# NVIDIA-Merlin/distributed-embeddings

Hardware: NVIDIA H100
Metric: DLRM global samples/sec (device-timed, max over ranks) (higher is better)
Workload: dtype bf16

## Files before the change

distributed_embeddings_b200/models/dlrm_fast.py:

```python
from __future__ import annotations

import os
from typing import Optional

import torch
from torch import nn

from ..ops import _native
from ..parallel.comm import CommContext
from ..parallel.fused import FusedEngine
from ..utils import nvtx
from ..utils.lr_schedule import LearningRateScheduler
from ..utils.metrics import BinnedAUC, auc_from_histogram
from .dense_optimizer import FlatDenseOptimizer, dense_optimizer_config
from .dlrm import DLRM

FUSED_UPDATE_MIN_ROWS = 20000


def _pad8(n: int) -> int:
  return (n + 7) // 8 * 8


def _fused_dgrad(L) -> bool:
  return L.in_f == L.in_pad and L.in_f <= 2048 and L.out_f % 8 == 0


def _dgrad_block_n(L) -> int:
  return 128 if L.out_f <= 256 else 0


class _Layer:

  def __init__(self, lin: nn.Linear, relu: bool):
    self.lin = lin
    self.relu = relu
    self.out_f, self.in_f = lin.weight.shape
    self.in_pad = _pad8(self.in_f)
    self.w_off = self.b_off = 0
    self.w_numel = self.out_f * self.in_pad
    self.b_numel = _pad8(self.out_f) if lin.bias is not None else 0


class DLRMTrainStep:

  def __init__(self, model: DLRM, lr: float = 24.0, embedding_optimizer: str = "sgd",
               scheduler: Optional[LearningRateScheduler] = None, use_cuda_graph: bool = True,
               embedding_optimizer_kwargs: Optional[dict] = None, overlap: bool = True,
               gemm: str = "cublas", eval_thresholds: int = 8000, dense_optimizer: str = "sgd",
               dense_optimizer_kwargs: Optional[dict] = None, fused_table_update: bool = True,
               fused_update_min_rows: int = FUSED_UPDATE_MIN_ROWS):
    if gemm not in ("cublas", "fused_dgrad", "tcgen05", "tcgen05_pair"):
      raise ValueError("gemm must be cublas | fused_dgrad | tcgen05 | tcgen05_pair")
    self.gemm = gemm
    self.dcn = getattr(model, "interaction", "dot") == "dcnv2"
    hots = getattr(model, "multi_hot_sizes", None)
    if self.dcn and gemm != "cublas":
      raise ValueError("the dcnv2 interaction runs its GEMMs on cuBLASLt: use gemm='cublas'")
    if not self.dcn and hots is not None and any(h != 1 for h in hots):
      raise ValueError("multi-hot features need the dcnv2 interaction in DLRMTrainStep")
    self.fused_table_update = bool(fused_table_update)
    self.fused_update_min_rows = int(fused_update_min_rows)
    self.dense_cfg = dense_optimizer_config(dense_optimizer, dense_optimizer_kwargs)
    self.model = model
    self.emb = model.embedding
    if self.emb.backend != "fused":
      raise ValueError("DLRMTrainStep needs the fused embedding back end")
    self.dev = self.emb.device
    self.ops = _native.require()
    self.world = self.emb.world_size
    self.ctx = CommContext.for_group(self.emb.group, self.dev)
    self.scheduler = scheduler
    self.use_cuda_graph = use_cuda_graph
    self.overlap = overlap
    self.emb.set_optimizer(embedding_optimizer, lr=lr, **(embedding_optimizer_kwargs or {}))
    if self.emb._engine is None:
      self.emb._engine = FusedEngine(self.emb)
    self.engine: FusedEngine = self.emb._engine
    self.n_emb = len(model.table_sizes)
    self.dim = model.embedding_dim
    self.hots = list(hots) if hots is not None else [1] * self.n_emb
    if self.dcn:
      st = self.emb.strategy
      if self.emb.dp_input and any(self.hots[i] != 1 for i in st.input_groups[2]):
        raise NotImplementedError("the dcnv2 step does not support multi-hot row-sliced inputs")
      if self.dim % 8 or any(l.V.out_features % 8 for l in model.cross_layers):
        raise ValueError("the dcnv2 step needs an embedding width and a cross rank that are "
                         "multiples of 8")
    sp_env = os.environ.get("DE_B200_STREAM_PUSH", "auto")
    self._stream_push = self.world > 1 and (sp_env == "1" or (sp_env == "auto" and self.world >= 4))
    self._push_stream = torch.cuda.Stream(device=self.dev) if self._stream_push else None
    self._push_ready = torch.cuda.Event() if self._stream_push else None

    lins_b = [m for m in model.bottom_mlp.net if isinstance(m, nn.Linear)]
    lins_t = [m for m in model.top_mlp.net if isinstance(m, nn.Linear)]
    self.bottom = [_Layer(l, True) for l in lins_b]
    self.top = [_Layer(l, True) for l in lins_t[:-1]]
    self.head = _Layer(lins_t[-1], False)
    if self.head.out_f != 1:
      raise ValueError("the top MLP must end in a single logit")
    self.cross = [(_Layer(c.V, False), _Layer(c.W, False)) for c in model.cross_layers] \
        if self.dcn else []
    layers = self.bottom + [L for pair in self.cross for L in pair] + self.top + [self.head]
    self._dp_slots = []
    pos = 0
    if len(self.emb.dp_layers):
      if embedding_optimizer.lower() != self.dense_cfg["kind"]:
        if embedding_optimizer.lower().startswith("rowwise_"):
          raise ValueError(
              f"replicated tables in the fast step are updated by the dense optimizer kernel, "
              f"which has no row-wise form: embedding_optimizer={embedding_optimizer!r} needs "
              f"data_parallel_threshold=None (no replicated tables)")
        if embedding_optimizer.lower() == "ftrl":
          raise ValueError(
              "replicated tables in the fast step are updated by the dense optimizer kernel, "
              "which has no FTRL: a dense FTRL step would set every row the step does not touch "
              "to the closed form of its z.  embedding_optimizer='ftrl' needs "
              "data_parallel_threshold=None (no replicated tables)")
        raise ValueError("replicated tables in the fast step are updated by the dense optimizer "
                         "kernel: use the same embedding_optimizer and dense_optimizer ('sgd', "
                         "'adagrad' or 'adam') or data_parallel_threshold=None")
      for layer in self.emb.dp_layers:
        w = layer.embeddings
        self._dp_slots.append((pos, tuple(w.shape)))
        pos += _pad8(w.numel())
    for L in layers:
      L.w_off = pos
      pos += L.w_numel
      L.b_off = pos
      pos += L.b_numel
    self.n_flat = pos
    dev = self.dev
    self.p32 = torch.zeros(pos, dtype=torch.float32, device=dev)
    self.p16 = torch.zeros(pos, dtype=torch.bfloat16, device=dev)
    if self.world > 1:
      self.gsym = self.ctx.alloc_multicast(pos * 4, "dense_grads") or \
          self.ctx.alloc(pos * 4, "dense_grads")
      self.allreduce_kind = "nvls_multimem" if getattr(self.gsym, "mc_ptr", 0) else "p2p"
      self.g32 = self.gsym.view(torch.float32, (pos,))
    else:
      self.gsym = None
      self.allreduce_kind = "none"
      self.g32 = torch.zeros(pos, dtype=torch.float32, device=dev)
    with torch.no_grad():
      dp_targets = []
      for layer, (off, shape) in zip(self.emb.dp_layers, self._dp_slots):
        n = shape[0] * shape[1]
        view = self.p32[off:off + n].view(shape)
        view.copy_(layer.embeddings.data)
        layer.embeddings.data = view
        dp_targets.append(self.g32[off:off + n].view(shape))
      if self._dp_slots:
        self.engine.set_dp_grad_targets(dp_targets)
        self.engine._tables_dirty = True
        self.engine._key = None
      for L in layers:
        wv = self.p32[L.w_off:L.w_off + L.w_numel].view(L.out_f, L.in_pad)
        wv[:, :L.in_f].copy_(L.lin.weight)
        L.lin.weight.data = wv[:, :L.in_f]
        if L.lin.bias is not None:
          bv = self.p32[L.b_off:L.b_off + L.out_f]
          bv.copy_(L.lin.bias)
          L.lin.bias.data = bv
        L.w16 = self.p16[L.w_off:L.w_off + L.w_numel].view(L.out_f, L.in_pad)
        L.b16 = self.p16[L.b_off:L.b_off + L.out_f]
        L.gw = self.g32[L.w_off:L.w_off + L.w_numel].view(L.out_f, L.in_pad)
        L.gb = self.g32[L.b_off:L.b_off + L.b_numel]
        L.w16T = torch.empty(L.in_pad, L.out_f, dtype=torch.bfloat16, device=dev)
      self.p16.copy_(self.p32)
      self._refresh_transposes()
    self.dense_opt = FlatDenseOptimizer(self.dense_cfg, self.p32)
    self.lr_t = torch.full((1,), float(lr), dtype=torch.float32, device=dev)
    self.engine.share_lr(self.lr_t)
    self.lr = float(lr)
    self.loss = torch.zeros(1, dtype=torch.float32, device=dev)
    self._batch = None
    self._graph = None
    self._side = torch.cuda.Stream(device=dev) if overlap else None
    self._wgrad_overlap = os.environ.get("DE_B200_WGRAD_STREAM", "auto")
    self._wstream = torch.cuda.Stream(device=dev) if overlap else None
    ar_env = os.environ.get("DE_B200_AR_OVERLAP", "auto")
    ar_on = ar_env == "1" or (ar_env == "auto" and self.world >= 4)
    self._ar_stream = torch.cuda.Stream(device=dev) if (overlap and self.world > 1 and ar_on) \
        else None
    self.eval_auc = BinnedAUC(eval_thresholds, device=dev)
    self._eval_loss = torch.zeros(1, dtype=torch.float64, device=dev)
    self._eval_count = torch.zeros(1, dtype=torch.int64, device=dev)
    self._eval_graph = None

  def _refresh_transposes(self):
    for L in self.bottom[1:] + self.top[1:]:
      if _fused_dgrad(L):
        L.w16T.copy_(L.w16.t())

  def _linear_fwd(self, L, x):
    if self.gemm in ("tcgen05", "tcgen05_pair"):
      pair = self.gemm == "tcgen05_pair" and L.out_f >= 256
      self.ops.gemm_tn_bias_act(x, L.w16, L.b16, L.y, True, 512 if pair else 0)
    else:
      torch._addmm_activation(L.b16, x, L.w16.t(), out=L.y)
    return L.y

  def _wgrad(self, L, x):
    use = self._wstream is not None and (
        self._wgrad_overlap == "1" or
        (self._wgrad_overlap == "auto" and (self._batch or 0) >= 49152))
    if not use:
      torch.mm(L.dy.t(), x, out_dtype=torch.float32, out=L.gw)
      return
    self._w_used = True
    self._wstream.wait_stream(torch.cuda.current_stream())
    with torch.cuda.stream(self._wstream):
      torch.mm(L.dy.t(), x, out_dtype=torch.float32, out=L.gw)

  def _dgrad_relu(self, L, x_below, dx, gb_below):
    if _fused_dgrad(L):
      self.ops.gemm_dgrad_relu_bias(L.dy, L.w16T, x_below, dx, gb_below, _dgrad_block_n(L))
    else:
      torch.mm(L.dy, L.w16, out=dx)
      self.ops.relu_bwd_bias(dx, x_below, gb_below)

  def _alloc(self, b: int):
    dev, bf = self.dev, torch.bfloat16
    if self.dcn:
      self._alloc_dcn(b)
    else:
      if self._stream_push:
        self.engine.enable_streamed_push(max(1024, -(-b // 16)))
      self.engine.prepare(b, [1] * self.n_emb, ids64=False)
      self.cat_stage = self.engine.in_flat[:self.n_emb * b].view(self.n_emb, b)
    self.num_in = torch.zeros(b, self.bottom[0].in_f, dtype=torch.float32, device=dev)
    self.lab_in = torch.zeros(b, dtype=torch.float32, device=dev)
    self.x0 = torch.zeros(b, self.bottom[0].in_pad, dtype=bf, device=dev)
    for L in self.bottom + self.top:
      L.y = torch.empty(b, L.out_f, dtype=bf, device=dev)
      L.dy = torch.empty(b, L.out_f, dtype=bf, device=dev)
    if not self.dcn:
      self.z = torch.zeros(b, self.top[0].in_pad, dtype=bf, device=dev)
      self.dz = torch.empty(b, self.top[0].in_pad, dtype=bf, device=dev)
    self._batch = b
    self._graph = None
    self._eval_graph = None
    self._n_valid = torch.zeros(1, dtype=torch.int64, device=dev)
    self._probs = torch.zeros(b, dtype=torch.float32, device=dev)
    self._stage = [(torch.zeros_like(self.cat_stage), torch.zeros_like(self.num_in),
                    torch.zeros_like(self.lab_in)) for _ in range(2)]
    self._slot_dev = torch.zeros(1, dtype=torch.int32, device=dev)
    self._slot_host = torch.tensor([[0], [1]], dtype=torch.int32).pin_memory()
    self._h2d_done = [torch.cuda.Event(), torch.cuda.Event()]
    self._consumed = [torch.cuda.Event(), torch.cuda.Event()]
    self._prefetched = 0
    self._consumed_n = 0
    self._use_stage = False

  def _alloc_dcn(self, b: int):
    dev, bf = self.dev, torch.bfloat16
    eng = self.engine
    D = self.model.cross_dim
    eng.set_out_row_stride(D)
    eng.prepare(b, self.hots, ids64=False)
    if eng.out_needs_reduce:
      raise NotImplementedError("the dcnv2 step does not support multi-hot row-sliced inputs")
    self.cat_stage = eng.in_flat[:sum(self.hots) * b]
    self.emb_cols = eng.total_width
    L = len(self.cross)
    self.xs = [eng.out_full] + [torch.empty(b, D, dtype=bf, device=dev) for _ in range(L)]
    self.ss = [torch.empty(b, D, dtype=bf, device=dev) for _ in range(L)]
    self.us = [torch.empty(b, V.out_f, dtype=bf, device=dev) for V, _ in self.cross]
    self.dX = [torch.empty(b, D, dtype=bf, device=dev) for _ in range(L + 1)]
    self.g = torch.empty(b, D, dtype=bf, device=dev)
    self.du = torch.empty(b, max(V.out_f for V, _ in self.cross), dtype=bf, device=dev)

  def _select_stage(self):
    a, b_ = self._stage
    self.ops.select_copy([a[0], a[1], a[2]], [b_[0], b_[1], b_[2]],
                         [self.cat_stage, self.num_in, self.lab_in], self._slot_dev)

  def _forward(self, train: bool = True):
    ops = self.ops
    eng = self.engine
    if self._side is not None:
      self._side.wait_stream(torch.cuda.current_stream())
      with torch.cuda.stream(self._side):
        eng.launch_forward(train)
    ops.cast_pad(self.num_in, self.x0)
    x = self.x0
    for L in self.bottom:
      x = self._linear_fwd(L, x)
    if self._side is not None:
      torch.cuda.current_stream().wait_stream(self._side)
    else:
      eng.launch_forward(train)
    if eng.out_needs_reduce:
      eng.wait_output()
      ops.interact_fwd(x, eng.out, self.n_emb, self.z, [])
    else:
      ops.interact_fwd(x, eng.out, self.n_emb, self.z, eng.sync_out_wait())
    x = self.z
    for L in self.top:
      x = self._linear_fwd(L, x)

  def _forward_dcn(self, train: bool = True):
    ops, eng = self.ops, self.engine
    if self._side is not None:
      self._side.wait_stream(torch.cuda.current_stream())
      with torch.cuda.stream(self._side):
        eng.launch_forward(train)
    ops.cast_pad(self.num_in, self.x0)
    x = self.x0
    for L in self.bottom:
      x = self._linear_fwd(L, x)
    x0 = self.xs[0]
    ops.copy_cast_2d(x, x0.data_ptr() + self.emb_cols * x0.element_size(), x0.stride(0), 1, 1.0)
    if self._side is not None:
      torch.cuda.current_stream().wait_stream(self._side)
    else:
      eng.launch_forward(train)
    eng.wait_output()
    x = x0
    for l, (V, W) in enumerate(self.cross):
      u, s_ = self.us[l], self.ss[l]
      torch.mm(x, V.w16.t(), out=u)
      torch.addmm(W.b16, u, W.w16.t(), out=s_)
      ops.cross_fwd(x0, s_, x, self.xs[l + 1])
      x = self.xs[l + 1]
    for L in self.top:
      x = self._linear_fwd(L, x)

  def _backward_dcn(self):
    ops, eng = self.ops, self.engine
    b = self._batch
    last = self.top[-1]
    self.loss.zero_()
    H = self.head
    ops.head_loss(last.y, H.w16.view(-1), H.b16, self.lab_in, 1.0 / b, last.dy,
                  H.gw.view(-1), H.gb, last.gb, self.loss, None)
    nL = len(self.cross)
    for i in range(len(self.top) - 1, -1, -1):
      L = self.top[i]
      x = self.top[i - 1].y if i > 0 else self.xs[nL]
      self._wgrad(L, x)
      if i > 0:
        self._dgrad_relu(L, x, self.top[i - 1].dy, self.top[i - 1].gb)
      else:
        torch.mm(L.dy, L.w16, out=self.dX[nL])
    self._allreduce_top_early()
    x0 = self.xs[0]
    for l in range(nL - 1, -1, -1):
      V, W = self.cross[l]
      dy = self.dX[l + 1]
      du = self.du[:, :V.out_f]
      ops.cross_bwd(dy, x0, self.g, W.gb)
      torch.mm(self.g.t(), self.us[l], out_dtype=torch.float32, out=W.gw)
      torch.mm(self.g, W.w16, out=du)
      torch.mm(du.t(), self.xs[l], out_dtype=torch.float32, out=V.gw)
      torch.addmm(dy, du, V.w16, out=self.dX[l])
    hb = self.bottom[-1]
    ops.cross_dx0(self.dX[0], self.dX[1:], self.ss, self.g, hb.dy)
    if eng.routes_all is not None:
      ops.push_grad(eng.routes_all, len(eng.routes_all_np), self.g[:, :self.emb_cols], eng.act,
                    1.0, eng.sync_grad_signal())
    self._backward_tail(None, False)

  def _allreduce_top_early(self):
    if self._ar_stream is not None:
      ar = self._ar_stream
      ar.wait_stream(torch.cuda.current_stream())
      if getattr(self, "_w_used", False):
        ar.wait_stream(self._wstream)
      off = self.top[0].w_off
      with torch.cuda.stream(ar):
        self.ctx.allreduce_(self.gsym, self.n_flat - off, torch.float32, scale=1.0 / self.world,
                            byte_offset=off * 4, max_blocks=32)

  def _backward(self):
    ops, eng = self.ops, self.engine
    b = self._batch
    last = self.top[-1]
    self.loss.zero_()
    H = self.head
    ops.head_loss(last.y, H.w16.view(-1), H.b16, self.lab_in, 1.0 / b, last.dy,
                  H.gw.view(-1), H.gb, last.gb, self.loss, None)
    for i in range(len(self.top) - 1, -1, -1):
      L = self.top[i]
      x = self.top[i - 1].y if i > 0 else self.z
      dx = self.top[i - 1].dy if i > 0 else self.dz
      self._wgrad(L, x)
      if i > 0:
        self._dgrad_relu(L, x, dx, self.top[i - 1].gb)
      else:
        torch.mm(L.dy, L.w16, out=dx)
    self._allreduce_top_early()
    hb = self.bottom[-1]
    pushed = eng.streamed_push
    applied = None
    if pushed:
      eng.push_counters.zero_()
      self._push_ready.record(torch.cuda.current_stream())
      ops.interact_bwd(hb.y, eng.out, self.n_emb, self.dz, hb.dy, 0, 0, 1.0, eng.routes_stage,
                       len(eng.routes_stage_np), [], eng.push_counters, eng.push_chunk_rows)
      self._push_stream.wait_event(self._push_ready)
      with torch.cuda.stream(self._push_stream):
        eng.launch_streamed_push()
    else:
      applied = eng.producer_update(self.dim, self.fused_update_min_rows) \
          if self.fused_table_update else None
      ops.interact_bwd(hb.y, eng.out, self.n_emb, self.dz, hb.dy, 0, 0, 1.0, eng.routes_all,
                       len(eng.routes_all_np), eng.sync_grad_signal(), None, 0,
                       *(applied.interact_args() if applied else ()))
    self._backward_tail(applied, pushed)

  def _backward_tail(self, applied, pushed: bool):
    ops, eng = self.ops, self.engine
    hb = self.bottom[-1]
    if self._side is not None:
      self._side.wait_stream(torch.cuda.current_stream())
      if pushed:
        self._side.wait_stream(self._push_stream)
      with torch.cuda.stream(self._side):
        eng.backward_inplace(applied)
    else:
      if pushed:
        torch.cuda.current_stream().wait_stream(self._push_stream)
      eng.backward_inplace(applied)
    ops.relu_bwd_bias(hb.dy, hb.y, hb.gb)
    for i in range(len(self.bottom) - 1, -1, -1):
      L = self.bottom[i]
      x = self.bottom[i - 1].y if i > 0 else self.x0
      self._wgrad(L, x)
      if i > 0:
        self._dgrad_relu(L, x, self.bottom[i - 1].dy, self.bottom[i - 1].gb)
    if self._dp_slots and self._side is not None:
      torch.cuda.current_stream().wait_stream(self._side)
    if getattr(self, "_w_used", False):
      torch.cuda.current_stream().wait_stream(self._wstream)
      self._w_used = False
    if self.world > 1:
      if self._ar_stream is not None:
        ar = self._ar_stream
        ar.wait_stream(torch.cuda.current_stream())
        with torch.cuda.stream(ar):
          self.ctx.allreduce_(self.gsym, self.top[0].w_off, torch.float32, scale=1.0 / self.world)
        torch.cuda.current_stream().wait_stream(ar)
      else:
        self.ctx.allreduce_(self.gsym, self.n_flat, torch.float32, scale=1.0 / self.world)
    self.dense_opt.apply(ops, self.p16, self.g32, self.lr_t)
    self._refresh_transposes()
    if self._side is not None:
      torch.cuda.current_stream().wait_stream(self._side)

  def _step_impl(self):
    with nvtx.range("dlrm_forward"):
      if self._use_stage:
        self._select_stage()
      self._forward_dcn() if self.dcn else self._forward()
    with nvtx.range("dlrm_backward_update"):
      self._backward_dcn() if self.dcn else self._backward()

  def set_lr(self, lr: float):
    self.lr = float(lr)
    self.lr_t.fill_(self.lr)
    if self.emb._fused_optimizer is not None:
      self.emb._fused_optimizer["lr"] = self.lr

  def load_batch(self, numerical, categorical, labels):
    b = int(numerical.shape[0])
    if b != self._batch:
      self._alloc(b)
    self.num_in.copy_(numerical, non_blocking=True)
    self.lab_in.copy_(labels.reshape(-1), non_blocking=True)
    if isinstance(categorical, (list, tuple)):
      for v, c in zip(self.engine.in_views, categorical):
        v.copy_(c.reshape(v.shape), non_blocking=True)
    elif self.dcn:
      self.cat_stage.copy_(categorical.reshape(-1), non_blocking=True)
    else:
      self.cat_stage.copy_(categorical, non_blocking=True)

  def prefetch(self, numerical, categorical, labels):
    b = int(numerical.shape[0])
    if b != self._batch:
      self._alloc(b)
    if not self._use_stage:
      self._use_stage = True
      self._graph = None
      self._copy_stream = torch.cuda.Stream(device=self.dev)
    slot = self._prefetched & 1
    cs = self._copy_stream
    if self._prefetched >= 2:
      cs.wait_event(self._consumed[slot])
    with torch.cuda.stream(cs):
      st = self._stage[slot]
      st[0].copy_(categorical.reshape(-1) if self.dcn else categorical, non_blocking=True)
      st[1].copy_(numerical, non_blocking=True)
      st[2].copy_(labels.reshape(-1), non_blocking=True)
      self._h2d_done[slot].record(cs)
    self._prefetched += 1

  def run_prefetched(self) -> torch.Tensor:
    assert self._consumed_n < self._prefetched, "call prefetch() first"
    slot = self._consumed_n & 1
    main = torch.cuda.current_stream()
    main.wait_event(self._h2d_done[slot])
    self._slot_dev.copy_(self._slot_host[slot], non_blocking=True)
    loss = self.run()
    self._consumed[slot].record(main)
    self._consumed_n += 1
    return loss

  def run(self) -> torch.Tensor:
    if self.scheduler is not None:
      self.set_lr(self.scheduler.step())
    if not self.use_cuda_graph:
      self._step_impl()
      return self.loss
    if self._graph is None:
      self.lr_t.zero_()
      self.engine.dry_updates(True)
      dense_snap = self.dense_opt.snapshot()
      s = torch.cuda.Stream(device=self.dev)
      s.wait_stream(torch.cuda.current_stream())
      with torch.cuda.stream(s):
        for _ in range(2):
          self._step_impl()
      torch.cuda.current_stream().wait_stream(s)
      torch.cuda.synchronize()
      self.engine.dry_updates(False)
      self.dense_opt.restore(dense_snap)
      g = torch.cuda.CUDAGraph()
      with torch.cuda.graph(g):
        self._step_impl()
      self._graph = g
      self.set_lr(self.lr)
    self._graph.replay()
    return self.loss

  def step(self, numerical, categorical, labels) -> torch.Tensor:
    self.load_batch(numerical, categorical, labels)
    return self.run()

  def dense_optimizer_state(self) -> dict:
    return self.dense_opt.state_dict(self.model)

  def load_dense_optimizer_state(self, state: dict):
    self.dense_opt.load_state_dict(self.model, state)

  def _eval_impl(self):
    with nvtx.range("dlrm_eval"):
      self._forward_dcn(False) if self.dcn else self._forward(False)
      H = self.head
      self.ops.head_eval(self.top[-1].y, H.w16.view(-1), H.b16, self.lab_in, self._n_valid,
                         self._probs, self.eval_auc.hist, self._eval_loss, self._eval_count)

  def _eval_ready(self):
    if self._batch is None:
      raise RuntimeError("evaluation runs in chunks of the training batch: load or run a "
                         "training batch first")
    if self.engine.out_needs_reduce:
      raise NotImplementedError("evaluation does not support multi-hot row-sliced inputs")
    if not self.use_cuda_graph or self._eval_graph is not None:
      return
    self._n_valid.zero_()
    s = torch.cuda.Stream(device=self.dev)
    s.wait_stream(torch.cuda.current_stream())
    with torch.cuda.stream(s):
      self._eval_impl()
    torch.cuda.current_stream().wait_stream(s)
    torch.cuda.synchronize()
    g = torch.cuda.CUDAGraph()
    with torch.cuda.graph(g):
      self._eval_impl()
    self._eval_graph = g

  def _eval_chunks(self, numerical, categorical, labels, out=None):
    n = int(numerical.shape[0])
    if n < 1:
      raise ValueError("evaluation needs at least one sample")
    self._eval_ready()
    b = self._batch
    lab = labels.reshape(-1) if labels is not None else None
    if self.dcn:
      cats = None
    elif isinstance(categorical, (list, tuple)):
      cats = [c.reshape(-1) for c in categorical]
    else:
      cats = None
    for s in range(0, n, b):
      m = min(b, n - s)
      self.num_in[:m].copy_(numerical[s:s + m], non_blocking=True)
      if self.dcn:
        for v, c in zip(self.engine.in_views, categorical):
          v[:m].copy_(c[s:s + m].reshape(m, -1), non_blocking=True)
          if m < b:
            v[m:].zero_()
        if m < b:
          self.num_in[m:].zero_()
      elif cats is None:
        self.cat_stage[:, :m].copy_(categorical[:, s:s + m], non_blocking=True)
      else:
        for f, c in enumerate(cats):
          self.cat_stage[f, :m].copy_(c[s:s + m], non_blocking=True)
      if m < b and not self.dcn:
        self.num_in[m:].zero_()
        self.cat_stage[:, m:].zero_()
      if lab is not None:
        self.lab_in[:m].copy_(lab[s:s + m], non_blocking=True)
      self._n_valid.fill_(m if lab is not None else 0)
      if self.use_cuda_graph:
        self._eval_graph.replay()
      else:
        self._eval_impl()
      if out is not None:
        out[s:s + m].copy_(self._probs[:m])

  def evaluate(self, numerical, categorical, labels):
    self._eval_chunks(numerical, categorical, labels)

  def predict(self, numerical, categorical) -> torch.Tensor:
    out = torch.empty(int(numerical.shape[0]), dtype=torch.float32, device=self.dev)
    self._eval_chunks(numerical, categorical, None, out)
    return out

  def eval_metrics(self, reset: bool = True) -> dict:
    hist = self.eval_auc.hist.view(-1)
    packed = torch.cat([hist.double(), self._eval_loss, self._eval_count.double()])
    if self.world > 1:
      import torch.distributed as dist
      dist.all_reduce(packed, group=self.emb.group)
    packed = packed.cpu()
    nb = hist.numel()
    res = auc_from_histogram(packed[:nb].round().long().view(2, -1))
    loss, count = float(packed[nb]), int(round(float(packed[nb + 1])))
    if reset:
      self.eval_auc.reset()
      self._eval_loss.zero_()
      self._eval_count.zero_()
    return {"auc": res.auc, "tie_bound": res.tie_bound,
            "log_loss": loss / count if count else float("nan"), "samples": count}
```

distributed_embeddings_b200/ops/csrc/bindings.cpp:

```cpp
#include <ATen/cuda/CUDAContext.h>
#include <c10/cuda/CUDAGuard.h>
#include <c10/cuda/CUDAStream.h>
#include <cuda_runtime.h>
#include <torch/library.h>
#include <torch/torch.h>

#include <cstdlib>
#include <cstring>
#include <mutex>
#include <string>
#include <unordered_map>
#include <vector>

#include "de_b200.h"

namespace {

using at::Tensor;

#define DE_CUDA_CHECK(expr)                                                              \
  do {                                                                                   \
    cudaError_t _e = (expr);                                                             \
    TORCH_CHECK(_e == cudaSuccess, "CUDA error in " #expr ": ", cudaGetErrorString(_e)); \
  } while (0)

cudaStream_t cur_stream() { return at::cuda::getCurrentCUDAStream().stream(); }

int sm_count() {
  static int cached = -1;
  if (cached < 0) cached = at::cuda::getCurrentDeviceProperties()->multiProcessorCount;
  return cached;
}

de::PeerPtrs to_peers(at::IntArrayRef ptrs) {
  TORCH_CHECK(ptrs.size() <= de::kMaxPeers, "at most ", de::kMaxPeers, " peers are supported");
  de::PeerPtrs p;
  std::memset(&p, 0, sizeof(p));
  for (size_t i = 0; i < ptrs.size(); ++i) p.p[i] = reinterpret_cast<void*>(ptrs[i]);
  return p;
}

void check_launch() {
  cudaError_t e = cudaGetLastError();
  TORCH_CHECK(e == cudaSuccess, "kernel launch failed: ", cudaGetErrorString(e));
}

struct SyncCtx {
  de::PeerPtrs flags;
  uint32_t* state;
  int* error_flag;
  unsigned long long timeout;
  int rank, world;
};
std::vector<SyncCtx>& sync_ctxs() {
  static std::vector<SyncCtx> v;
  return v;
}
std::mutex& sync_mutex() {
  static std::mutex m;
  return m;
}

int64_t sync_ctx_create(at::IntArrayRef flag_ptrs, Tensor state, int64_t rank, int64_t world,
                        int64_t timeout_cycles, int64_t error_ptr) {
  TORCH_CHECK(state.is_cuda() && state.scalar_type() == at::kInt && state.is_contiguous() &&
                  state.numel() >= de::kSyncStateWords,
              "sync state must be an int32 CUDA tensor of >= ", de::kSyncStateWords, " words");
  SyncCtx c;
  c.flags = to_peers(flag_ptrs);
  c.state = reinterpret_cast<uint32_t*>(state.data_ptr<int>());
  c.error_flag = reinterpret_cast<int*>(error_ptr);
  c.timeout = static_cast<unsigned long long>(timeout_cycles);
  c.rank = static_cast<int>(rank);
  c.world = static_cast<int>(world);
  std::lock_guard<std::mutex> lock(sync_mutex());
  sync_ctxs().push_back(c);
  return static_cast<int64_t>(sync_ctxs().size()) - 1;
}

de::SyncArgs to_sync(at::IntArrayRef spec) {
  de::SyncArgs a = de::no_sync();
  if (spec.size() == 0) return a;
  TORCH_CHECK(spec.size() == 5, "sync spec = {handle, wait_ch, wait_abs_ch, signal_ch, slot}");
  SyncCtx c;
  {
    std::lock_guard<std::mutex> lock(sync_mutex());
    TORCH_CHECK(spec[0] >= 0 && spec[0] < static_cast<int64_t>(sync_ctxs().size()),
                "unknown sync context");
    c = sync_ctxs()[spec[0]];
  }
  for (int i = 1; i <= 3; ++i)
    TORCH_CHECK(spec[i] >= -1 && spec[i] < de::kSyncChannels, "sync channel out of range");
  TORCH_CHECK(spec[4] >= 0 && spec[4] < 2 * de::kSyncChannels, "sync counter slot out of range");
  a.flags = c.flags;
  a.state = c.state;
  a.error_flag = c.error_flag;
  a.timeout = c.timeout;
  a.rank = c.rank;
  a.world = c.world;
  a.wait_ch = static_cast<int32_t>(spec[1]);
  a.wait_abs_ch = static_cast<int32_t>(spec[2]);
  a.signal_ch = static_cast<int32_t>(spec[3]);
  a.counter_slot = static_cast<int32_t>(spec[4]);
  return a;
}

int dtype_code(at::ScalarType t) {
  if (t == at::kFloat) return 0;
  if (t == at::kBFloat16) return 1;
  if (t == at::kHalf) return 2;
  TORCH_CHECK(false, "activations / gradients must be fp32, bf16 or fp16");
  return -1;
}

void sync_only(at::IntArrayRef sync) {
  de::launch_sync_only(to_sync(sync), cur_stream());
  check_launch();
}

std::vector<int64_t> struct_sizes() {
  return {static_cast<int64_t>(sizeof(de::InputDesc)), static_cast<int64_t>(sizeof(de::TableDesc)),
          static_cast<int64_t>(de::kMaxPeers), static_cast<int64_t>(sizeof(de::GradRoute)),
          static_cast<int64_t>(de::kSyncStateWords),
          static_cast<int64_t>(sizeof(de::CacheRemap))};
}

void lookup_fwd(const Tensor& descs, int64_t n_inputs, int64_t batch, int64_t src_batch,
                int64_t dst_batch, int64_t dst_stride, at::IntArrayRef src_ptrs,
                at::IntArrayRef dst_ptrs, int64_t rot, bool ids64, int64_t act_dtype, bool vec4,
                at::IntArrayRef sync, int64_t tile_samples, int64_t table_dtype, bool vec8) {
  TORCH_CHECK(descs.is_cuda(), "descs must live on the GPU");
  TORCH_CHECK(table_dtype >= 0 && table_dtype <= 2, "table_dtype: 0 fp32, 1 bf16, 2 fp16");
  c10::cuda::CUDAGuard guard(descs.device());
  de::launch_lookup_fwd(reinterpret_cast<const de::InputDesc*>(descs.data_ptr()),
                        static_cast<int>(n_inputs), batch, src_batch, dst_batch, dst_stride,
                        to_peers(src_ptrs), to_peers(dst_ptrs), static_cast<int>(rot), ids64,
                        static_cast<int>(act_dtype), vec4, sm_count(), cur_stream(),
                        to_sync(sync), static_cast<int>(tile_samples),
                        static_cast<int>(table_dtype), vec8);
  check_launch();
}

void scatter_add_bwd(const Tensor& descs, int64_t n_inputs, int64_t batch, int64_t src_batch,
                     int64_t grad_batch, int64_t grad_stride, at::IntArrayRef src_ptrs,
                     at::IntArrayRef grad_ptrs, int64_t rot, double scale, int64_t scale_ptr,
                     bool ids64, int64_t act_dtype, bool vec4, bool vec8, at::IntArrayRef sync,
                     bool staged) {
  TORCH_CHECK(descs.is_cuda(), "descs must live on the GPU");
  c10::cuda::CUDAGuard guard(descs.device());
  de::launch_scatter_add_bwd(reinterpret_cast<const de::InputDesc*>(descs.data_ptr()),
                             static_cast<int>(n_inputs), batch, src_batch, grad_batch, grad_stride,
                             to_peers(src_ptrs), to_peers(grad_ptrs), static_cast<int>(rot),
                             static_cast<float>(scale), reinterpret_cast<const float*>(scale_ptr),
                             ids64, static_cast<int>(act_dtype), vec4, sm_count(), cur_stream(),
                             vec8, to_sync(sync), staged);
  check_launch();
}

int bit_length(int64_t v) {
  int b = 0;
  while (v > 0) {
    ++b;
    v >>= 1;
  }
  return b < 1 ? 1 : b;
}

bool use_own_sort() {
  static const bool own = [] {
    const char* v = std::getenv("DE_B200_SORT");
    return !(v != nullptr && std::string(v) == "cub");
  }();
  return own;
}

std::tuple<Tensor, Tensor> radix_sort_pairs(const Tensor& keys, const Tensor& items,
                                            int64_t end_bit) {
  TORCH_CHECK(keys.is_cuda() && keys.scalar_type() == at::kLong && keys.is_contiguous());
  TORCH_CHECK(items.is_cuda() && items.scalar_type() == at::kInt && items.is_contiguous() &&
              items.numel() == keys.numel());
  c10::cuda::CUDAGuard guard(keys.device());
  const int64_t n = keys.numel();
  TORCH_CHECK(n < (int64_t(1) << 31), "own radix sort: too many items");
  Tensor ka = keys.clone(), ia = items.clone();
  Tensor kb = at::empty_like(ka), ib = at::empty_like(ia);
  if (n == 0) return {ka, ia};
  Tensor temp = at::empty({static_cast<int64_t>(de::radix_sort_temp_bytes(n))},
                          at::TensorOptions().device(keys.device()).dtype(at::kByte));
  int where = de::radix_sort_pairs(temp.data_ptr(), ka.data_ptr<int64_t>(),
                                   reinterpret_cast<uint32_t*>(ia.data_ptr<int>()),
                                   kb.data_ptr<int64_t>(),
                                   reinterpret_cast<uint32_t*>(ib.data_ptr<int>()), n,
                                   static_cast<int>(end_bit), cur_stream());
  check_launch();
  if (where == 0) return {ka, ia};
  return {kb, ib};
}

std::tuple<Tensor, Tensor> radix_sort_pairs32(const Tensor& keys, const Tensor& items,
                                              int64_t end_bit) {
  TORCH_CHECK(keys.is_cuda() && keys.scalar_type() == at::kInt && keys.is_contiguous());
  TORCH_CHECK(items.is_cuda() && items.scalar_type() == at::kInt && items.is_contiguous() &&
              items.numel() == keys.numel());
  c10::cuda::CUDAGuard guard(keys.device());
  const int64_t n = keys.numel();
  TORCH_CHECK(n < (int64_t(1) << 31), "own radix sort: too many items");
  Tensor ka = keys.clone(), ia = items.clone();
  Tensor kb = at::empty_like(ka), ib = at::empty_like(ia);
  Tensor out = at::empty({n}, keys.options().dtype(at::kLong));
  if (n == 0) return {out, ia};
  Tensor temp = at::empty({static_cast<int64_t>(de::radix_sort_temp_bytes(n))},
                          at::TensorOptions().device(keys.device()).dtype(at::kByte));
  int where = de::radix_sort_pairs32(
      temp.data_ptr(), reinterpret_cast<uint32_t*>(ka.data_ptr<int>()),
      reinterpret_cast<uint32_t*>(ia.data_ptr<int>()),
      reinterpret_cast<uint32_t*>(kb.data_ptr<int>()),
      reinterpret_cast<uint32_t*>(ib.data_ptr<int>()), out.data_ptr<int64_t>(), n,
      static_cast<int>(end_bit), cur_stream());
  check_launch();
  return {out, where == 0 ? ia : ib};
}

std::tuple<Tensor, Tensor> head_segments(const Tensor& sorted_keys) {
  TORCH_CHECK(sorted_keys.is_cuda() && sorted_keys.scalar_type() == at::kLong &&
              sorted_keys.is_contiguous());
  c10::cuda::CUDAGuard guard(sorted_keys.device());
  const int64_t n = sorted_keys.numel();
  auto i64 = at::TensorOptions().device(sorted_keys.device()).dtype(at::kLong);
  Tensor seg_start = at::empty({n + 1}, i64);
  Tensor n_unique = at::zeros({1}, i64);
  if (n == 0) return {seg_start, n_unique};
  Tensor temp = at::empty({static_cast<int64_t>(de::head_segments_temp_bytes(n))},
                          at::TensorOptions().device(sorted_keys.device()).dtype(at::kByte));
  de::head_segments(temp.data_ptr(), sorted_keys.data_ptr<int64_t>(), n,
                    seg_start.data_ptr<int64_t>(), n_unique.data_ptr<int64_t>(), cur_stream());
  check_launch();
  return {seg_start, n_unique};
}

std::tuple<Tensor, Tensor, Tensor, Tensor> sort_items(const Tensor& descs, const Tensor& tables,
                                                      int64_t n_tables, int64_t n_inputs,
                                                      int64_t batch, int64_t src_batch,
                                                      at::IntArrayRef src_ptrs, bool ids64,
                                                      int64_t n_items, int64_t total_rows,
                                                      bool prefill_sentinel) {
  TORCH_CHECK(descs.is_cuda() && tables.is_cuda());
  TORCH_CHECK(n_inputs * batch < (int64_t(1) << 32),
              "sorted update: n_inputs * batch = ", n_inputs * batch, " does not fit 32-bit items");
  c10::cuda::CUDAGuard guard(descs.device());
  auto stream = cur_stream();
  auto i64 = at::TensorOptions().device(descs.device()).dtype(at::kLong);
  auto i32 = at::TensorOptions().device(descs.device()).dtype(at::kInt);
  Tensor keys = prefill_sentinel ? at::full({n_items}, total_rows, i64) : at::empty({n_items}, i64);
  Tensor keys_sorted = at::empty({n_items}, i64);
  Tensor items = at::empty({n_items}, i32), items_sorted = at::empty({n_items}, i32);
  Tensor seg_start = at::empty({n_items + 1}, i64);
  Tensor n_unique = at::zeros({1}, i64);
  if (n_items == 0) return {keys_sorted, items_sorted, seg_start, n_unique};
  if (use_own_sort() && total_rows < (int64_t(1) << 32) - 1) {
    TORCH_CHECK(n_items < (int64_t(1) << 31), "own radix sort: too many items");
    Tensor k32a = prefill_sentinel
                      ? at::full({n_items}, static_cast<int64_t>(static_cast<int32_t>(
                                                static_cast<uint32_t>(total_rows))), i32)
                      : at::empty({n_items}, i32);
    Tensor k32b = at::empty({n_items}, i32);
    de::launch_build_keys(reinterpret_cast<const de::InputDesc*>(descs.data_ptr()),
                          reinterpret_cast<const de::TableDesc*>(tables.data_ptr()),
                          static_cast<int>(n_tables), static_cast<int>(n_inputs), batch,
                          src_batch, to_peers(src_ptrs), ids64, k32a.data_ptr(),
                          reinterpret_cast<uint32_t*>(items.data_ptr<int>()), sm_count(), stream,
                          true);
    check_launch();
    size_t sort_bytes = de::radix_sort_temp_bytes(n_items);
    size_t head_bytes = de::head_segments_temp_bytes(n_items);
    Tensor temp = at::empty({static_cast<int64_t>(std::max(sort_bytes, head_bytes))},
                            at::TensorOptions().device(descs.device()).dtype(at::kByte));
    int where = de::radix_sort_pairs32(
        temp.data_ptr(), reinterpret_cast<uint32_t*>(k32a.data_ptr<int>()),
        reinterpret_cast<uint32_t*>(items.data_ptr<int>()),
        reinterpret_cast<uint32_t*>(k32b.data_ptr<int>()),
        reinterpret_cast<uint32_t*>(items_sorted.data_ptr<int>()),
        keys_sorted.data_ptr<int64_t>(), n_items, bit_length(total_rows), stream);
    if (where == 0) std::swap(items, items_sorted);
    de::head_segments(temp.data_ptr(), keys_sorted.data_ptr<int64_t>(), n_items,
                      seg_start.data_ptr<int64_t>(), n_unique.data_ptr<int64_t>(), stream);
    check_launch();
    return {keys_sorted, items_sorted, seg_start, n_unique};
  }
  de::launch_build_keys(reinterpret_cast<const de::InputDesc*>(descs.data_ptr()),
                        reinterpret_cast<const de::TableDesc*>(tables.data_ptr()),
                        static_cast<int>(n_tables), static_cast<int>(n_inputs), batch, src_batch,
                        to_peers(src_ptrs), ids64, keys.data_ptr<int64_t>(),
                        reinterpret_cast<uint32_t*>(items.data_ptr<int>()), sm_count(), stream);
  check_launch();
  if (use_own_sort()) {
    TORCH_CHECK(n_items < (int64_t(1) << 31), "own radix sort: too many items");
    size_t sort_bytes = de::radix_sort_temp_bytes(n_items);
    size_t head_bytes = de::head_segments_temp_bytes(n_items);
    Tensor temp = at::empty({static_cast<int64_t>(std::max(sort_bytes, head_bytes))},
                            at::TensorOptions().device(descs.device()).dtype(at::kByte));
    int where = de::radix_sort_pairs(temp.data_ptr(), keys.data_ptr<int64_t>(),
                                     reinterpret_cast<uint32_t*>(items.data_ptr<int>()),
                                     keys_sorted.data_ptr<int64_t>(),
                                     reinterpret_cast<uint32_t*>(items_sorted.data_ptr<int>()),
                                     n_items, bit_length(total_rows), stream);
    if (where == 0) {
      std::swap(keys, keys_sorted);
      std::swap(items, items_sorted);
    }
    de::head_segments(temp.data_ptr(), keys_sorted.data_ptr<int64_t>(), n_items,
                      seg_start.data_ptr<int64_t>(), n_unique.data_ptr<int64_t>(), stream);
    check_launch();
    return {keys_sorted, items_sorted, seg_start, n_unique};
  }
  size_t sort_bytes = de::sort_pairs_temp_bytes(n_items);
  size_t uniq_bytes = de::unique_temp_bytes(n_items);
  Tensor temp = at::empty({static_cast<int64_t>(std::max(sort_bytes, uniq_bytes)) + 16},
                          at::TensorOptions().device(descs.device()).dtype(at::kByte));
  de::sort_pairs(temp.data_ptr(), sort_bytes, keys.data_ptr<int64_t>(),
                 keys_sorted.data_ptr<int64_t>(),
                 reinterpret_cast<const uint32_t*>(items.data_ptr<int>()),
                 reinterpret_cast<uint32_t*>(items_sorted.data_ptr<int>()), n_items,
                 bit_length(total_rows), stream);
  de::unique_segments(temp.data_ptr(), uniq_bytes, keys_sorted.data_ptr<int64_t>(), n_items,
                      seg_start.data_ptr<int64_t>(), n_unique.data_ptr<int64_t>(), stream);
  check_launch();
  return {keys_sorted, items_sorted, seg_start, n_unique};
}

void segment_update(const Tensor& descs, const Tensor& tables, int64_t n_tables, int64_t batch,
                    int64_t grad_batch, int64_t grad_stride, at::IntArrayRef grad_ptrs,
                    const Tensor& sorted_keys, const Tensor& sorted_items, const Tensor& seg_start,
                    const Tensor& n_unique, int64_t opt_kind, double lr, double eps, double beta1,
                    double beta2, double bias1, double bias2, double grad_scale,
                    double weight_decay, int64_t lr_ptr, const c10::optional<Tensor>& emit_keys,
                    const c10::optional<Tensor>& emit_rows, int64_t max_width, int64_t act_dtype,
                    bool vec4, const c10::optional<Tensor>& scratch, int64_t step_ptr,
                    int64_t table_dtype, int64_t state_dtype, double lr_power = -0.5,
                    double l1 = 0.0, double l2 = 0.0, double l2_shrinkage = 0.0,
                    double ftrl_beta = 0.0) {
  c10::cuda::CUDAGuard guard(descs.device());
  TORCH_CHECK(table_dtype >= 0 && table_dtype <= 2, "table_dtype: 0 fp32, 1 bf16, 2 fp16");
  TORCH_CHECK(state_dtype == 0 || state_dtype == 1, "state_dtype: 0 fp32, 1 bf16");
  de::OptimizerArgs opt;
  opt.kind = static_cast<int32_t>(opt_kind);
  opt.lr = static_cast<float>(lr);
  opt.eps = static_cast<float>(eps);
  opt.beta1 = static_cast<float>(beta1);
  opt.beta2 = static_cast<float>(beta2);
  opt.bias1 = static_cast<float>(bias1);
  opt.bias2 = static_cast<float>(bias2);
  opt.grad_scale = static_cast<float>(grad_scale);
  opt.weight_decay = static_cast<float>(weight_decay);
  opt.lr_ptr = reinterpret_cast<const float*>(lr_ptr);
  opt.step_ptr = reinterpret_cast<const float*>(step_ptr);
  opt.lr_power = static_cast<float>(lr_power);
  opt.l1 = static_cast<float>(l1);
  opt.l2 = static_cast<float>(l2);
  opt.l2_shrinkage = static_cast<float>(l2_shrinkage);
  opt.ftrl_beta = static_cast<float>(ftrl_beta);
  if (opt.kind == de::kOptEmit) TORCH_CHECK(emit_keys.has_value() && emit_rows.has_value());
  if (scratch.has_value() && vec4 && max_width <= 128 && opt.kind != de::kOptEmit) {
    const int64_t n_items = sorted_keys.numel();
    const int64_t sw = (max_width + 3) / 4 * 4;
    TORCH_CHECK(scratch->scalar_type() == at::kFloat && scratch->is_contiguous() &&
                    scratch->numel() >= ((n_items + 31) / 32) * sw,
                "scratch too small for the balanced update");
    bool ok = de::launch_balanced_update(
        reinterpret_cast<const de::InputDesc*>(descs.data_ptr()),
        reinterpret_cast<const de::TableDesc*>(tables.data_ptr()), static_cast<int>(n_tables),
        batch, grad_batch, grad_stride, to_peers(grad_ptrs), sorted_keys.data_ptr<int64_t>(),
        reinterpret_cast<const uint32_t*>(sorted_items.data_ptr<int>()), n_items,
        seg_start.data_ptr<int64_t>(), n_unique.data_ptr<int64_t>(), opt,
        scratch->data_ptr<float>(), static_cast<int>(sw), static_cast<int>(max_width),
        static_cast<int>(act_dtype), sm_count(), cur_stream(), static_cast<int>(table_dtype),
        static_cast<int>(state_dtype));
    TORCH_CHECK(ok, "balanced update launch failed");
    check_launch();
    return;
  }
  de::launch_segment_update(
      reinterpret_cast<const de::InputDesc*>(descs.data_ptr()),
      reinterpret_cast<const de::TableDesc*>(tables.data_ptr()), static_cast<int>(n_tables), batch,
      grad_batch, grad_stride, to_peers(grad_ptrs), sorted_keys.data_ptr<int64_t>(),
      reinterpret_cast<const uint32_t*>(sorted_items.data_ptr<int>()),
      seg_start.data_ptr<int64_t>(), n_unique.data_ptr<int64_t>(), sorted_keys.numel(), opt,
      emit_keys.has_value() ? emit_keys->data_ptr<int64_t>() : nullptr,
      emit_rows.has_value() ? emit_rows->data_ptr<float>() : nullptr, static_cast<int>(max_width),
      static_cast<int>(act_dtype), vec4, sm_count(), cur_stream(), static_cast<int>(table_dtype),
      static_cast<int>(state_dtype));
  check_launch();
}

Tensor upload_bytes(const void* host, size_t bytes, const at::Device& dev) {
  Tensor t = at::empty({static_cast<int64_t>(bytes)},
                       at::TensorOptions().device(dev).dtype(at::kByte));
  DE_CUDA_CHECK(cudaMemcpyAsync(t.data_ptr(), host, bytes, cudaMemcpyHostToDevice, cur_stream()));
  return t;
}

de::InputDesc single_desc(const void* table, const Tensor& values,
                          const c10::optional<Tensor>& offsets, int64_t hotness, int64_t rows,
                          int64_t width, int64_t combiner) {
  de::InputDesc d;
  std::memset(&d, 0, sizeof(d));
  d.table = table;
  d.ids = values.data_ptr();
  d.offsets = offsets.has_value() ? offsets->data_ptr<int64_t>() : nullptr;
  d.sub_rows = rows;
  d.width = static_cast<int32_t>(width);
  d.hotness = offsets.has_value() ? 0 : static_cast<int32_t>(hotness);
  d.combiner = static_cast<int32_t>(combiner);
  return d;
}

void check_ids(const Tensor& values, const c10::optional<Tensor>& offsets) {
  TORCH_CHECK(values.is_cuda() && values.is_contiguous(), "ids must be a contiguous CUDA tensor");
  TORCH_CHECK(values.scalar_type() == at::kInt || values.scalar_type() == at::kLong,
              "ids must be int32 or int64");
  if (offsets.has_value())
    TORCH_CHECK(offsets->is_cuda() && offsets->scalar_type() == at::kLong &&
                    offsets->is_contiguous(),
                "row_splits must be a contiguous int64 CUDA tensor");
}

Tensor embedding_lookup_fwd(const Tensor& param, const Tensor& values,
                            const c10::optional<Tensor>& offsets, int64_t hotness, int64_t batch,
                            int64_t combiner, bool out_bf16) {
  const auto pt = param.scalar_type();
  TORCH_CHECK(param.is_cuda() && param.dim() == 2 &&
                  (pt == at::kFloat || pt == at::kBFloat16 || pt == at::kHalf) &&
                  param.is_contiguous(),
              "param must be a contiguous fp32, bf16 or fp16 [rows, width] CUDA tensor");
  check_ids(values, offsets);
  c10::cuda::CUDAGuard guard(param.device());
  const int64_t width = param.size(1);
  const int tdt = dtype_code(pt);
  Tensor out = at::empty({batch, width}, param.options().dtype(out_bf16 ? at::kBFloat16 : pt));
  if (batch == 0) return out;
  de::InputDesc d = single_desc(param.data_ptr(), values, offsets, hotness, param.size(0), width,
                                combiner);
  Tensor dd = upload_bytes(&d, sizeof(d), param.device());
  de::PeerPtrs src, dst;
  std::memset(&src, 0, sizeof(src));
  std::memset(&dst, 0, sizeof(dst));
  dst.p[0] = out.data_ptr();
  const int64_t avg_hot = std::max<int64_t>(1, values.numel() / std::max<int64_t>(batch, 1));
  int64_t lanes_per_row = 1;
  while (lanes_per_row < (width + 3) / 4 && lanes_per_row < 32) lanes_per_row *= 2;
  const int64_t ts = std::max<int64_t>(32 / lanes_per_row, std::min<int64_t>(32, 64 / avg_hot));
  const uintptr_t base = reinterpret_cast<uintptr_t>(param.data_ptr());
  const bool vec4 = width % 4 == 0 && base % (4 * param.element_size()) == 0;
  de::launch_lookup_fwd(reinterpret_cast<const de::InputDesc*>(dd.data_ptr()), 1, batch, batch,
                        batch, width, src, dst, 0, values.scalar_type() == at::kLong,
                        out_bf16 ? 1 : tdt, vec4, sm_count(), cur_stream(), de::no_sync(),
                        static_cast<int>(std::max<int64_t>(1, ts)), tdt,
                        width % 8 == 0 && base % 16 == 0);
  check_launch();
  return out;
}

void embedding_scatter_add(Tensor dst, const Tensor& values, const c10::optional<Tensor>& offsets,
                           int64_t hotness, int64_t batch, int64_t combiner, const Tensor& grad,
                           double scale) {
  TORCH_CHECK(dst.is_cuda() && dst.dim() == 2 && dst.scalar_type() == at::kFloat &&
              dst.is_contiguous());
  TORCH_CHECK(grad.is_cuda() && grad.dim() == 2 && grad.stride(1) == 1);
  check_ids(values, offsets);
  if (batch == 0) return;
  c10::cuda::CUDAGuard guard(dst.device());
  const int64_t width = dst.size(1);
  de::InputDesc d = single_desc(dst.data_ptr(), values, offsets, hotness, dst.size(0), width,
                                combiner);
  Tensor dd = upload_bytes(&d, sizeof(d), dst.device());
  de::PeerPtrs src, gp;
  std::memset(&src, 0, sizeof(src));
  std::memset(&gp, 0, sizeof(gp));
  gp.p[0] = grad.data_ptr();
  const int gdt = dtype_code(grad.scalar_type());
  const int64_t gstride = grad.stride(0);
  const bool vec4 = (width % 4 == 0) && (gstride % 4 == 0) &&
                    (reinterpret_cast<uintptr_t>(grad.data_ptr()) % 16 == 0) &&
                    (reinterpret_cast<uintptr_t>(dst.data_ptr()) % 16 == 0);
  de::launch_scatter_add_bwd(reinterpret_cast<const de::InputDesc*>(dd.data_ptr()), 1, batch,
                             batch, batch, gstride, src, gp, 0, static_cast<float>(scale), nullptr,
                             values.scalar_type() == at::kLong, gdt, vec4, sm_count(),
                             cur_stream(), false, de::no_sync());
  check_launch();
}

std::tuple<Tensor, Tensor> embedding_lookup_grad(const Tensor& values,
                                                 const c10::optional<Tensor>& offsets,
                                                 int64_t hotness, int64_t batch, int64_t combiner,
                                                 const Tensor& grad, int64_t num_rows) {
  TORCH_CHECK(grad.is_cuda() && grad.dim() == 2 && grad.stride(1) == 1);
  check_ids(values, offsets);
  c10::cuda::CUDAGuard guard(grad.device());
  const int64_t width = grad.size(1);
  const int64_t n_items = values.numel();
  auto f32 = grad.options().dtype(at::kFloat);
  auto i64 = grad.options().dtype(at::kLong);
  if (n_items == 0) return {at::empty({0}, i64), at::empty({0, width}, f32)};
  de::InputDesc d = single_desc(nullptr, values, offsets, hotness, num_rows, width, combiner);
  de::TableDesc t;
  std::memset(&t, 0, sizeof(t));
  t.rows = num_rows;
  t.width = static_cast<int32_t>(width);
  Tensor dd = upload_bytes(&d, sizeof(d), grad.device());
  Tensor td = upload_bytes(&t, sizeof(t), grad.device());
  auto sorted = sort_items(dd, td, 1, 1, batch, batch, {}, values.scalar_type() == at::kLong,
                           n_items, num_rows, false);
  Tensor emit_keys = at::empty({n_items}, i64);
  Tensor emit_rows = at::empty({n_items, width}, f32);
  const int gdt = dtype_code(grad.scalar_type());
  const int64_t gstride = grad.stride(0);
  const bool vec4 = (width % 4 == 0) && (gstride % 4 == 0) &&
                    (reinterpret_cast<uintptr_t>(grad.data_ptr()) % 16 == 0);
  std::vector<int64_t> gp = {reinterpret_cast<int64_t>(grad.data_ptr())};
  segment_update(dd, td, 1, batch, batch, gstride, gp, std::get<0>(sorted), std::get<1>(sorted),
                 std::get<2>(sorted), std::get<3>(sorted), de::kOptEmit, 0, 0, 0, 0, 1, 1, 1.0, 0, 0,
                 emit_keys, emit_rows, width, gdt, vec4, c10::nullopt, 0, 0, 0);
  int64_t n_unique = std::get<3>(sorted).item<int64_t>();
  if (n_unique > 0) {
    int64_t last = emit_keys.narrow(0, n_unique - 1, 1).item<int64_t>();
    if (last >= num_rows) --n_unique;
  }
  return {emit_keys.narrow(0, 0, n_unique), emit_rows.narrow(0, 0, n_unique)};
}

Tensor row_to_split(const Tensor& indices, int64_t num_rows) {
  TORCH_CHECK(indices.is_cuda() && indices.dim() == 2 && indices.size(1) == 2 &&
                  indices.scalar_type() == at::kLong && indices.is_contiguous(),
              "indices must be a contiguous int64 [nnz, 2] CUDA tensor");
  c10::cuda::CUDAGuard guard(indices.device());
  Tensor splits = at::empty({num_rows + 1}, indices.options());
  de::launch_row_to_split(indices.data_ptr<int64_t>(), indices.size(0), num_rows,
                          splits.data_ptr<int64_t>(), cur_stream());
  check_launch();
  return splits;
}

void hash_init(Tensor table) {
  TORCH_CHECK(table.is_cuda() && table.scalar_type() == at::kLong && table.is_contiguous());
  c10::cuda::CUDAGuard guard(table.device());
  de::launch_hash_init(table.data_ptr<int64_t>(), table.numel() / 2, cur_stream());
  check_launch();
}

Tensor integer_lookup(Tensor table, Tensor count, Tensor next_index, const Tensor& keys,
                      int64_t capacity) {
  TORCH_CHECK(table.is_cuda() && count.is_cuda() && next_index.is_cuda() && keys.is_cuda());
  TORCH_CHECK(table.scalar_type() == at::kLong && keys.scalar_type() == at::kLong &&
              next_index.scalar_type() == at::kLong && count.scalar_type() == at::kInt);
  c10::cuda::CUDAGuard guard(table.device());
  Tensor k = keys.contiguous();
  Tensor out = at::empty_like(k);
  de::launch_integer_lookup(table.data_ptr<int64_t>(), table.numel() / 2,
                            reinterpret_cast<uint32_t*>(count.data_ptr<int>()),
                            next_index.data_ptr<int64_t>(), k.data_ptr<int64_t>(), k.numel(),
                            capacity, out.data_ptr<int64_t>(), cur_stream());
  check_launch();
  return out;
}

void barrier(at::IntArrayRef flag_ptrs, Tensor epoch, int64_t rank, int64_t world, int64_t channel,
             int64_t timeout_cycles, int64_t error_ptr) {
  c10::cuda::CUDAGuard guard(epoch.device());
  de::launch_barrier(to_peers(flag_ptrs), reinterpret_cast<uint32_t*>(epoch.data_ptr<int>()),
                     static_cast<int>(rank), static_cast<int>(world), static_cast<int>(channel),
                     static_cast<unsigned long long>(timeout_cycles),
                     reinterpret_cast<int*>(error_ptr), cur_stream());
  check_launch();
}

void allreduce(at::IntArrayRef buf_ptrs, at::IntArrayRef flag_ptrs, Tensor epoch, int64_t rank,
               int64_t world, int64_t n_elems, double scale, bool bf16, int64_t channel,
               int64_t timeout_cycles, int64_t error_ptr, int64_t mc_ptr, int64_t max_blocks) {
  c10::cuda::CUDAGuard guard(epoch.device());
  if (mc_ptr != 0) {
    de::launch_allreduce_multimem(reinterpret_cast<void*>(mc_ptr), to_peers(flag_ptrs),
                                  reinterpret_cast<uint32_t*>(epoch.data_ptr<int>()),
                                  static_cast<int>(rank), static_cast<int>(world), n_elems,
                                  static_cast<float>(scale), bf16, static_cast<int>(channel),
                                  static_cast<unsigned long long>(timeout_cycles),
                                  reinterpret_cast<int*>(error_ptr), sm_count(), cur_stream(),
                         static_cast<int>(max_blocks));
  } else {
    de::launch_allreduce(to_peers(buf_ptrs), to_peers(flag_ptrs),
                         reinterpret_cast<uint32_t*>(epoch.data_ptr<int>()),
                         static_cast<int>(rank), static_cast<int>(world), n_elems,
                         static_cast<float>(scale), bf16, static_cast<int>(channel),
                         static_cast<unsigned long long>(timeout_cycles),
                         reinterpret_cast<int*>(error_ptr), sm_count(), cur_stream(),
                         static_cast<int>(max_blocks));
  }
  check_launch();
}

void p2p_store_bench(const Tensor& src, int64_t dst_ptr, int64_t n_rows, int64_t row_bytes,
                     int64_t vec_bytes, int64_t dst_stride, int64_t unroll, int64_t blocks,
                     int64_t threads) {
  TORCH_CHECK(src.is_cuda() && src.is_contiguous() &&
              src.numel() * src.element_size() >= n_rows * row_bytes);
  TORCH_CHECK(row_bytes % vec_bytes == 0 && (vec_bytes == 4 || vec_bytes == 8 || vec_bytes == 16));
  TORCH_CHECK((row_bytes / vec_bytes >= 32 && (row_bytes / vec_bytes) % 32 == 0) ||
              32 % (row_bytes / vec_bytes) == 0);
  TORCH_CHECK(unroll >= 1 && unroll <= 8 && threads % 32 == 0 && threads <= 1024);
  c10::cuda::CUDAGuard guard(src.device());
  de::launch_p2p_store_bench(src.data_ptr(), reinterpret_cast<void*>(dst_ptr), n_rows,
                             static_cast<int>(row_bytes), static_cast<int>(vec_bytes), dst_stride,
                             static_cast<int>(unroll), static_cast<int>(blocks),
                             static_cast<int>(threads), cur_stream());
  check_launch();
}

void push_segments(const Tensor& segs, const Tensor& src, at::IntArrayRef dst_ptrs,
                   int64_t max_seg_elems, at::IntArrayRef sync) {
  TORCH_CHECK(segs.is_cuda() && segs.scalar_type() == at::kLong && segs.is_contiguous() &&
              segs.dim() == 2 && segs.size(1) == 4);
  TORCH_CHECK(src.is_cuda() && src.is_contiguous() &&
              (src.element_size() == 4 || src.element_size() == 8));
  c10::cuda::CUDAGuard guard(src.device());
  de::launch_push_segments(segs.data_ptr<int64_t>(), static_cast<int>(segs.size(0)),
                           src.data_ptr(), to_peers(dst_ptrs),
                           static_cast<int>(src.element_size()), max_seg_elems, sm_count(),
                           cur_stream(), to_sync(sync));
  check_launch();
}

void push_grad(const Tensor& routes, int64_t n_routes, const Tensor& src, int64_t dst_dtype,
               double scale, at::IntArrayRef sync) {
  TORCH_CHECK(routes.is_cuda() && routes.scalar_type() == at::kByte &&
              routes.numel() >= n_routes * static_cast<int64_t>(sizeof(de::GradRoute)));
  TORCH_CHECK(src.is_cuda() && src.dim() == 2 && src.stride(1) == 1);
  c10::cuda::CUDAGuard guard(src.device());
  de::launch_push_grad(reinterpret_cast<const de::GradRoute*>(routes.data_ptr()),
                       static_cast<int>(n_routes), src.data_ptr(), src.stride(0),
                       dtype_code(src.scalar_type()), static_cast<int>(dst_dtype), src.size(0),
                       static_cast<float>(scale), sm_count(), cur_stream(), to_sync(sync));
  check_launch();
}

void stream_push(at::IntArrayRef src_ptrs, at::IntArrayRef dst_ptrs, at::IntArrayRef row_bytes,
                 const Tensor& counters, int64_t chunk_rows, int64_t rows, int64_t blocks,
                 at::IntArrayRef sync) {
  TORCH_CHECK(src_ptrs.size() == dst_ptrs.size() && src_ptrs.size() == row_bytes.size() &&
              src_ptrs.size() <= de::kMaxPeers);
  TORCH_CHECK(counters.is_cuda() && counters.scalar_type() == at::kInt && chunk_rows > 0 &&
              counters.numel() >= (rows + chunk_rows - 1) / chunk_rows);
  de::PushPlan plan;
  std::memset(&plan, 0, sizeof(plan));
  plan.n = static_cast<int32_t>(src_ptrs.size());
  for (size_t i = 0; i < src_ptrs.size(); ++i) {
    TORCH_CHECK(row_bytes[i] % 16 == 0 && src_ptrs[i] % 16 == 0 && dst_ptrs[i] % 16 == 0,
                "streamed push needs 16-byte aligned rows");
    plan.src[i] = reinterpret_cast<const void*>(src_ptrs[i]);
    plan.dst[i] = reinterpret_cast<void*>(dst_ptrs[i]);
    plan.row_bytes[i] = row_bytes[i];
  }
  c10::cuda::CUDAGuard guard(counters.device());
  de::SyncArgs sa = to_sync(sync);
  de::launch_stream_push(plan, reinterpret_cast<const uint32_t*>(counters.data_ptr<int>()),
                         static_cast<int>(chunk_rows), rows, sa.timeout, sa.error_flag,
                         static_cast<int>(blocks), cur_stream(), sa);
  check_launch();
}

void rowslice_reduce(const Tensor& partial, int64_t out_ptr, int64_t out_stride,
                     int64_t out_dtype, const Tensor& cols) {
  TORCH_CHECK(partial.is_cuda() && partial.dim() == 3 && partial.scalar_type() == at::kFloat &&
              partial.is_contiguous());
  TORCH_CHECK(cols.is_cuda() && cols.scalar_type() == at::kInt && cols.is_contiguous() &&
              cols.dim() == 2 && cols.size(1) == 3);
  c10::cuda::CUDAGuard guard(partial.device());
  de::launch_rowslice_reduce(partial.data_ptr<float>(), static_cast<int>(partial.size(0)),
                             partial.size(1), partial.size(2), reinterpret_cast<void*>(out_ptr),
                             out_stride, static_cast<int>(out_dtype), cols.data_ptr<int>(),
                             static_cast<int>(cols.size(0)), cur_stream());
  check_launch();
}

void gather_segments(const Tensor& segs, at::IntArrayRef src_ptrs, Tensor dst,
                     int64_t max_seg_elems) {
  TORCH_CHECK(segs.is_cuda() && segs.scalar_type() == at::kLong && segs.is_contiguous());
  TORCH_CHECK(dst.is_cuda() && dst.is_contiguous());
  c10::cuda::CUDAGuard guard(dst.device());
  de::launch_gather_segments(segs.data_ptr<int64_t>(), static_cast<int>(segs.size(0)),
                             to_peers(src_ptrs), dst.data_ptr(),
                             static_cast<int>(dst.element_size()), max_seg_elems, cur_stream());
  check_launch();
}

void gather_ragged(const Tensor& segs, at::IntArrayRef val_ptrs, at::IntArrayRef split_ptrs,
                   Tensor dst_vals, Tensor goff, int64_t b, int64_t max_cap) {
  TORCH_CHECK(segs.is_cuda() && segs.scalar_type() == at::kLong && segs.is_contiguous());
  TORCH_CHECK(goff.is_cuda() && goff.scalar_type() == at::kLong && dst_vals.is_cuda());
  c10::cuda::CUDAGuard guard(dst_vals.device());
  de::launch_gather_ragged(segs.data_ptr<int64_t>(), static_cast<int>(segs.size(0)),
                           to_peers(val_ptrs), to_peers(split_ptrs), dst_vals.data_ptr(),
                           goff.data_ptr<int64_t>(), b, static_cast<int>(val_ptrs.size()),
                           static_cast<int>(dst_vals.element_size()), max_cap, cur_stream());
  check_launch();
}

void select_copy(at::TensorList src0, at::TensorList src1, at::TensorList dst,
                 const Tensor& slot_flag) {
  TORCH_CHECK(src0.size() == dst.size() && src1.size() == dst.size() && dst.size() <= 4);
  TORCH_CHECK(slot_flag.is_cuda() && slot_flag.scalar_type() == at::kInt);
  const void* s0[4];
  const void* s1[4];
  void* d[4];
  int64_t nb[4];
  for (size_t i = 0; i < dst.size(); ++i) {
    TORCH_CHECK(src0[i].is_contiguous() && src1[i].is_contiguous() && dst[i].is_contiguous());
    nb[i] = dst[i].numel() * dst[i].element_size();
    TORCH_CHECK(src0[i].numel() * src0[i].element_size() == nb[i] &&
                src1[i].numel() * src1[i].element_size() == nb[i] && nb[i] % 16 == 0,
                "select_copy segments must match and be multiples of 16 bytes");
    s0[i] = src0[i].data_ptr();
    s1[i] = src1[i].data_ptr();
    d[i] = dst[i].data_ptr();
  }
  c10::cuda::CUDAGuard guard(slot_flag.device());
  de::launch_select_copy(s0, s1, d, nb, static_cast<int>(dst.size()), slot_flag.data_ptr<int>(),
                         sm_count(), cur_stream());
  check_launch();
}

void copy_cast_2d(const Tensor& src, int64_t dst_ptr, int64_t dst_stride, int64_t dst_dtype,
                  double scale) {
  TORCH_CHECK(src.is_cuda() && src.dim() == 2 && src.stride(1) == 1);
  c10::cuda::CUDAGuard guard(src.device());
  de::launch_copy_cast_2d(src.data_ptr(), src.stride(0), reinterpret_cast<void*>(dst_ptr),
                          dst_stride, src.size(0), src.size(1), dtype_code(src.scalar_type()),
                          static_cast<int>(dst_dtype), static_cast<float>(scale), cur_stream());
  check_launch();
}

void check_bf16_2d(const Tensor& t, const char* name) {
  TORCH_CHECK(t.is_cuda() && t.dim() == 2 && t.scalar_type() == at::kBFloat16 && t.stride(1) == 1,
              name, " must be a 2-D bf16 CUDA tensor with unit inner stride");
}

void check_row_alignment(const Tensor& t, int64_t bytes, const char* name) {
  TORCH_CHECK((t.stride(0) * 2) % bytes == 0 &&
                  reinterpret_cast<uintptr_t>(t.data_ptr()) % static_cast<uintptr_t>(bytes) == 0,
              name, bytes == 16 ? " rows must start on 16-byte boundaries"
                                : " rows must start on 4-byte boundaries");
}

void interact_fwd(const Tensor& bottom, const Tensor& emb, int64_t n_emb, Tensor z,
                  at::IntArrayRef sync) {
  check_bf16_2d(bottom, "bottom");
  check_bf16_2d(emb, "emb");
  check_bf16_2d(z, "z");
  c10::cuda::CUDAGuard guard(bottom.device());
  const int64_t dim = bottom.size(1);
  TORCH_CHECK(emb.size(1) == n_emb * dim, "emb must be [batch, n_emb * dim]");
  TORCH_CHECK(emb.size(0) >= bottom.size(0) && z.size(0) >= bottom.size(0),
              "emb and z need a row per row of bottom");
  check_row_alignment(bottom, 16, "bottom");
  check_row_alignment(emb, 16, "emb");
  const int64_t need = (n_emb + 1) * n_emb / 2 + dim;
  TORCH_CHECK(z.size(1) >= need, "z is too narrow");
  bool ok = de::launch_interact_fwd(bottom.data_ptr(), bottom.stride(0), emb.data_ptr(),
                                    emb.stride(0), static_cast<int>(n_emb), static_cast<int>(dim),
                                    z.data_ptr(), z.stride(0), static_cast<int>(z.size(1)),
                                    bottom.size(0), sm_count(), cur_stream(), to_sync(sync));
  TORCH_CHECK(ok, "unsupported interaction shape (n_emb <= 31, dim in {16,32,64,128})");
  check_launch();
}

void interact_bwd(const Tensor& bottom, const Tensor& emb, int64_t n_emb, const Tensor& dz,
                  Tensor dbottom, int64_t demb_ptr, int64_t demb_stride, double emb_grad_scale,
                  const c10::optional<Tensor>& routes, int64_t n_routes, at::IntArrayRef sync,
                  const c10::optional<Tensor>& done_counters, int64_t chunk_rows,
                  const c10::optional<Tensor>& apply_descs, double apply_scale,
                  int64_t apply_scale_ptr, bool apply_ids64) {
  de::InteractApply apply{};
  if (apply_descs.has_value()) {
    const Tensor& a = *apply_descs;
    TORCH_CHECK(!a.is_cuda() && a.scalar_type() == at::kByte && a.is_contiguous(),
                "apply_descs must be a contiguous uint8 CPU tensor of InputDesc records");
    TORCH_CHECK(a.numel() == n_emb * static_cast<int64_t>(sizeof(de::InputDesc)),
                "apply_descs needs one InputDesc per embedding row");
    TORCH_CHECK(n_emb <= de::kMaxInteractApply, "apply_descs: at most 31 embedding rows");
    TORCH_CHECK(apply_scale_ptr % 4 == 0, "apply_scale_ptr must be 4-byte aligned");
    TORCH_CHECK(!done_counters.has_value(), "apply_descs cannot be combined with done_counters");
    const auto* d = reinterpret_cast<const de::InputDesc*>(a.data_ptr());
    for (int64_t f = 0; f < n_emb; ++f) {
      if (d[f].table == nullptr) continue;
      TORCH_CHECK(d[f].width == 128 && bottom.size(1) == 128,
                  "apply_descs: applied tables must be 128 wide, like the interaction");
      TORCH_CHECK(d[f].hotness == 1 && d[f].offsets == nullptr && d[f].ids != nullptr,
                  "apply_descs: applied inputs must be one-hot with direct ids");
      TORCH_CHECK(reinterpret_cast<uintptr_t>(d[f].table) % 16 == 0,
                  "apply_descs: tables must be 16-byte aligned");
      TORCH_CHECK(reinterpret_cast<uintptr_t>(d[f].ids) % (apply_ids64 ? 8 : 4) == 0,
                  "apply_descs: ids must be aligned to their element size");
      TORCH_CHECK(d[f].row_base >= 0 && d[f].sub_rows >= 0,
                  "apply_descs: row_base and sub_rows must not be negative");
      apply.table[f] = static_cast<float*>(const_cast<void*>(d[f].table));
      apply.ids[f] = d[f].ids;
      apply.row_base[f] = d[f].row_base;
      apply.sub_rows[f] = d[f].sub_rows;
      apply.id_shift[f] = d[f].id_shift;
      apply.mask |= 1u << f;
    }
    apply.scale = static_cast<float>(apply_scale);
    apply.scale_ptr = reinterpret_cast<const float*>(apply_scale_ptr);
    apply.ids64 = apply_ids64 ? 1 : 0;
  }
  check_bf16_2d(bottom, "bottom");
  check_bf16_2d(emb, "emb");
  check_bf16_2d(dz, "dz");
  check_bf16_2d(dbottom, "dbottom");
  if (routes.has_value()) {
    TORCH_CHECK(routes->is_cuda() && routes->scalar_type() == at::kByte &&
                routes->numel() >= n_routes * static_cast<int64_t>(sizeof(de::GradRoute)));
  } else {
    TORCH_CHECK(demb_ptr != 0, "interact_bwd needs an embedding-gradient buffer or routes");
  }
  const int64_t dim = bottom.size(1);
  const int64_t batch = bottom.size(0);
  TORCH_CHECK(emb.size(1) == n_emb * dim, "emb must be [batch, n_emb * dim]");
  TORCH_CHECK((n_emb + 1) * n_emb / 2 + dim <= dz.size(1), "dz is too narrow");
  TORCH_CHECK(dbottom.size(1) == dim, "dbottom must be [batch, dim]");
  TORCH_CHECK(emb.size(0) >= batch && dz.size(0) >= batch && dbottom.size(0) >= batch,
              "emb, dz and dbottom need a row per row of bottom");
  check_row_alignment(bottom, 16, "bottom");
  check_row_alignment(emb, 16, "emb");
  check_row_alignment(dbottom, 4, "dbottom");
  if (!routes.has_value())
    TORCH_CHECK(demb_stride % 2 == 0 && demb_ptr % 4 == 0,
                "embedding-gradient rows must start on 4-byte boundaries");
  if (done_counters.has_value()) {
    TORCH_CHECK(done_counters->is_cuda() && done_counters->scalar_type() == at::kInt &&
                    done_counters->is_contiguous(),
                "done_counters must be a contiguous int32 CUDA tensor");
    TORCH_CHECK(chunk_rows > 0, "chunk_rows must be positive with done_counters");
    TORCH_CHECK(done_counters->numel() >= (batch + chunk_rows - 1) / chunk_rows,
                "done_counters needs one counter per chunk of chunk_rows samples");
  }
  c10::cuda::CUDAGuard guard(bottom.device());
  bool ok = de::launch_interact_bwd(bottom.data_ptr(), bottom.stride(0), emb.data_ptr(),
                                    emb.stride(0), static_cast<int>(n_emb), static_cast<int>(dim),
                                    dz.data_ptr(), dz.stride(0), dbottom.data_ptr(),
                                    dbottom.stride(0), reinterpret_cast<void*>(demb_ptr),
                                    demb_stride, static_cast<float>(emb_grad_scale),
                                    bottom.size(0), sm_count(), cur_stream(),
                                    routes.has_value()
                                        ? reinterpret_cast<const de::GradRoute*>(routes->data_ptr())
                                        : nullptr,
                                    static_cast<int>(n_routes), to_sync(sync),
                                    done_counters.has_value()
                                        ? reinterpret_cast<uint32_t*>(done_counters->data_ptr<int>())
                                        : nullptr,
                                    static_cast<int>(chunk_rows),
                                    apply.mask != 0 ? &apply : nullptr);
  TORCH_CHECK(ok, "unsupported interaction shape (n_emb <= 31, dim in {32,64,128}; routed / "
                  "signalling launches need dim in {64,128} and 16-byte aligned rows)");
  check_launch();
}

void avgpool_fwd(const Tensor& x, int64_t n, Tensor out, int64_t stride) {
  check_bf16_2d(x, "x");
  check_bf16_2d(out, "out");
  const int64_t out_len = (n + stride - 1) / stride;
  TORCH_CHECK(x.size(1) >= n && out.size(1) >= out_len && out.size(0) == x.size(0));
  const int64_t pad = std::max<int64_t>(0, (out_len - 1) * stride + stride - n);
  c10::cuda::CUDAGuard guard(x.device());
  de::launch_avgpool_fwd(x.data_ptr(), x.stride(0), static_cast<int>(n), out.data_ptr(),
                         out.stride(0), static_cast<int>(out_len), static_cast<int>(stride),
                         static_cast<int>(pad / 2), x.size(0), cur_stream());
  check_launch();
}

void avgpool_bwd(const Tensor& dout, Tensor dx, int64_t n, int64_t stride) {
  check_bf16_2d(dout, "dout");
  check_bf16_2d(dx, "dx");
  const int64_t out_len = (n + stride - 1) / stride;
  TORCH_CHECK(dx.size(1) >= n && dout.size(1) >= out_len && dout.size(0) == dx.size(0));
  const int64_t pad = std::max<int64_t>(0, (out_len - 1) * stride + stride - n);
  c10::cuda::CUDAGuard guard(dx.device());
  de::launch_avgpool_bwd(dout.data_ptr(), dout.stride(0), static_cast<int>(out_len),
                         dx.data_ptr(), dx.stride(0), static_cast<int>(n),
                         static_cast<int>(stride), static_cast<int>(pad / 2), dx.size(0),
                         cur_stream());
  check_launch();
}

void relu_bwd_bias(Tensor dy, const Tensor& y, Tensor db) {
  check_bf16_2d(dy, "dy");
  check_bf16_2d(y, "y");
  TORCH_CHECK(dy.is_contiguous() && y.is_contiguous() && dy.size(1) % 8 == 0);
  TORCH_CHECK(y.sizes() == dy.sizes(), "y must have the shape of dy");
  TORCH_CHECK(dy.size(1) >= 8 && dy.size(1) <= 2048, "relu_bwd_bias supports 8..2048 columns");
  TORCH_CHECK(db.is_cuda() && db.scalar_type() == at::kFloat && db.numel() >= dy.size(1));
  c10::cuda::CUDAGuard guard(dy.device());
  de::launch_relu_bwd_bias(dy.data_ptr(), y.data_ptr(), db.data_ptr<float>(), dy.size(0),
                           static_cast<int>(dy.size(1)), cur_stream());
  check_launch();
}

void check_cross(const Tensor& t, const Tensor& ref, int64_t cols, const char* name) {
  TORCH_CHECK(t.is_cuda() && t.device() == ref.device(), name, " must be on the device of x0");
  TORCH_CHECK(t.dim() == 2 && t.scalar_type() == at::kBFloat16, name, " must be a 2-D bf16 tensor");
  TORCH_CHECK(t.is_contiguous(), name, " must be contiguous");
  TORCH_CHECK(t.size(0) == ref.size(0) && t.size(1) == cols, name, " has the wrong shape");
  TORCH_CHECK(cols % 8 == 0 && cols > 0, name, " must have a positive multiple of 8 columns");
  TORCH_CHECK((reinterpret_cast<uintptr_t>(t.data_ptr()) & 15) == 0, name,
              " must be 16-byte aligned");
}

void cross_fwd(const Tensor& x0, const Tensor& s, const Tensor& xl, Tensor out) {
  TORCH_CHECK(x0.dim() == 2, "x0 must be a 2-D bf16 tensor");
  const int64_t d = x0.size(1);
  check_cross(x0, x0, d, "x0");
  check_cross(s, x0, d, "s");
  check_cross(xl, x0, d, "xl");
  check_cross(out, x0, d, "out");
  c10::cuda::CUDAGuard guard(x0.device());
  de::launch_cross_fwd(x0.data_ptr(), s.data_ptr(), xl.data_ptr(), out.data_ptr(), x0.numel(),
                       sm_count(), cur_stream());
  check_launch();
}

void cross_bwd(const Tensor& dy, const Tensor& x0, Tensor g, Tensor db) {
  TORCH_CHECK(x0.dim() == 2, "x0 must be a 2-D bf16 tensor");
  const int64_t d = x0.size(1);
  check_cross(x0, x0, d, "x0");
  check_cross(dy, x0, d, "dy");
  check_cross(g, x0, d, "g");
  TORCH_CHECK(db.device() == x0.device() && db.scalar_type() == at::kFloat && db.is_contiguous(),
              "db must be a contiguous fp32 tensor on the device of x0");
  TORCH_CHECK(db.numel() == d, "db must hold one element per column");
  c10::cuda::CUDAGuard guard(x0.device());
  de::launch_cross_bwd(dy.data_ptr(), x0.data_ptr(), g.data_ptr(), db.data_ptr<float>(),
                       x0.size(0), static_cast<int>(d), cur_stream());
  check_launch();
}

void cross_dx0(const Tensor& d_chain, at::TensorList dy, at::TensorList s, Tensor dx0,
               Tensor d_bottom) {
  TORCH_CHECK(d_chain.dim() == 2, "d_chain must be a 2-D bf16 tensor");
  const int64_t d = d_chain.size(1);
  check_cross(d_chain, d_chain, d, "d_chain");
  check_cross(dx0, d_chain, d, "dx0");
  TORCH_CHECK(dy.size() == s.size(), "dy and s must have the same length");
  TORCH_CHECK(!dy.empty() && dy.size() <= static_cast<size_t>(de::kMaxCrossLayers),
              "cross_dx0 takes 1 to 8 layers");
  TORCH_CHECK(d_bottom.dim() == 2 && d_bottom.size(1) <= d,
              "d_bottom must be 2-D with at most the columns of d_chain");
  check_cross(d_bottom, d_chain, d_bottom.size(1), "d_bottom");
  de::CrossTerms terms{};
  for (size_t l = 0; l < dy.size(); ++l) {
    check_cross(dy[l], d_chain, d, "dy");
    check_cross(s[l], d_chain, d, "s");
    terms.dy[l] = dy[l].data_ptr();
    terms.s[l] = s[l].data_ptr();
  }
  terms.n = static_cast<int>(dy.size());
  c10::cuda::CUDAGuard guard(d_chain.device());
  de::launch_cross_dx0(d_chain.data_ptr(), terms, dx0.data_ptr(), d_bottom.data_ptr(),
                       d_chain.size(0), static_cast<int>(d),
                       static_cast<int>(d - d_bottom.size(1)), cur_stream());
  check_launch();
}

void head_loss(const Tensor& x, const Tensor& w, const Tensor& bias, const Tensor& labels,
               double inv_batch, Tensor dx, Tensor dw, Tensor db, Tensor dbias_prev,
               Tensor loss_sum, const c10::optional<Tensor>& logits) {
  check_bf16_2d(x, "x");
  TORCH_CHECK(x.is_contiguous() && dx.is_contiguous());
  TORCH_CHECK(w.scalar_type() == at::kBFloat16 && bias.scalar_type() == at::kBFloat16);
  TORCH_CHECK(labels.scalar_type() == at::kFloat && labels.is_contiguous());
  const int64_t batch = x.size(0), k = x.size(1);
  auto f32 = [](const Tensor& t, int64_t n, const char* name) {
    TORCH_CHECK(t.is_cuda() && t.scalar_type() == at::kFloat && t.is_contiguous() &&
                    t.numel() >= n,
                name, " must be a contiguous fp32 CUDA tensor with enough elements");
  };
  TORCH_CHECK(w.is_cuda() && w.is_contiguous() && w.numel() == k, "w must hold K elements");
  TORCH_CHECK(bias.is_cuda() && bias.numel() >= 1, "bias must hold one element");
  TORCH_CHECK(labels.is_cuda() && labels.numel() == batch, "labels must hold one value per row");
  TORCH_CHECK(dx.is_cuda() && dx.scalar_type() == at::kBFloat16 && dx.sizes() == x.sizes(),
              "dx must be a bf16 tensor of the shape of x");
  f32(dw, k, "dw");
  f32(db, 1, "db");
  f32(dbias_prev, k, "dbias_prev");
  f32(loss_sum, 1, "loss_sum");
  if (logits.has_value()) f32(*logits, batch, "logits");
  c10::cuda::CUDAGuard guard(x.device());
  bool ok = de::launch_head_loss(x.data_ptr(), static_cast<int>(x.size(1)), w.data_ptr(),
                                 bias.data_ptr(), labels.data_ptr<float>(), x.size(0),
                                 static_cast<float>(inv_batch), dx.data_ptr(),
                                 dw.data_ptr<float>(), db.data_ptr<float>(),
                                 dbias_prev.data_ptr<float>(), loss_sum.data_ptr<float>(),
                                 logits.has_value() ? logits->data_ptr<float>() : nullptr,
                                 sm_count(), cur_stream());
  TORCH_CHECK(ok, "head_loss supports K in {64,128,256,512,1024}");
  check_launch();
}

void head_eval(const Tensor& x, const Tensor& w, const Tensor& bias, const Tensor& labels,
               const Tensor& n_valid, Tensor probs, Tensor hist, Tensor loss_sum, Tensor count) {
  check_bf16_2d(x, "x");
  TORCH_CHECK(x.is_contiguous(), "x must be contiguous");
  const int64_t batch = x.size(0), k = x.size(1);
  TORCH_CHECK(k == 64 || k == 128 || k == 256 || k == 512 || k == 1024,
              "head_eval supports K in {64,128,256,512,1024}");
  const auto dev = x.device();
  auto on_dev = [&](const Tensor& t, at::ScalarType dt, const char* name, const char* what) {
    TORCH_CHECK(t.device() == dev && t.scalar_type() == dt && t.is_contiguous(), name, what);
  };
  on_dev(w, at::kBFloat16, "w", " must be a contiguous bf16 tensor on the device of x");
  TORCH_CHECK(w.numel() == k, "w must hold K elements");
  on_dev(bias, at::kBFloat16, "bias", " must be a contiguous bf16 tensor on the device of x");
  TORCH_CHECK(bias.numel() >= 1, "bias must hold one element");
  on_dev(labels, at::kFloat, "labels", " must be a contiguous fp32 tensor on the device of x");
  TORCH_CHECK(labels.numel() == batch, "labels must hold one value per row");
  on_dev(n_valid, at::kLong, "n_valid", " must be an int64 tensor on the device of x");
  TORCH_CHECK(n_valid.numel() == 1, "n_valid must be one int64 word");
  on_dev(probs, at::kFloat, "probs", " must be a contiguous fp32 tensor on the device of x");
  TORCH_CHECK(probs.numel() == batch, "probs must hold one value per row");
  on_dev(hist, at::kLong, "hist", " must be a contiguous int64 tensor on the device of x");
  TORCH_CHECK(hist.dim() == 2 && hist.size(0) == 2 && hist.size(1) >= 1 &&
                  hist.size(1) <= (int64_t{1} << 24),
              "hist must be [2, T - 1] with 2 <= T <= 2^24 + 1");
  on_dev(loss_sum, at::kDouble, "loss_sum", " must be an fp64 tensor on the device of x");
  TORCH_CHECK(loss_sum.numel() == 1, "loss_sum must hold one element");
  on_dev(count, at::kLong, "count", " must be an int64 tensor on the device of x");
  TORCH_CHECK(count.numel() == 1, "count must hold one element");
  c10::cuda::CUDAGuard guard(dev);
  bool ok = de::launch_head_eval(x.data_ptr(), static_cast<int>(k), w.data_ptr(), bias.data_ptr(),
                                 labels.data_ptr<float>(), batch, n_valid.data_ptr<int64_t>(),
                                 probs.data_ptr<float>(), hist.data_ptr<int64_t>(),
                                 static_cast<int>(hist.size(1)), loss_sum.data_ptr<double>(),
                                 count.data_ptr<int64_t>(), sm_count(), cur_stream());
  TORCH_CHECK(ok, "head_eval supports K in {64,128,256,512,1024}");
  check_launch();
}

void dense_sgd(Tensor p32, Tensor p16, Tensor g32, const Tensor& lr, double grad_scale) {
  TORCH_CHECK(p32.is_cuda() && p32.scalar_type() == at::kFloat && g32.scalar_type() == at::kFloat &&
              p16.scalar_type() == at::kBFloat16 && lr.scalar_type() == at::kFloat);
  TORCH_CHECK(p32.numel() % 4 == 0 && p32.numel() == g32.numel() && p32.numel() == p16.numel());
  c10::cuda::CUDAGuard guard(p32.device());
  de::launch_sgd_update(p32.data_ptr<float>(), p16.data_ptr(), g32.data_ptr<float>(),
                        lr.data_ptr<float>(), static_cast<float>(grad_scale), p32.numel(),
                        sm_count(), cur_stream());
  check_launch();
}

void check_dense_opt(const Tensor& p32, const Tensor& p16, const Tensor& g32,
                     const std::vector<std::pair<const Tensor*, const char*>>& state,
                     const Tensor& lr, const Tensor* step) {
  TORCH_CHECK(p32.is_cuda(), "p32 must be a CUDA tensor");
  const auto dev = p32.device();
  const int64_t n = p32.numel();
  TORCH_CHECK(n % 4 == 0, "the flat buffers must hold a multiple of 4 elements");
  auto flat = [&](const Tensor& t, at::ScalarType dt, const char* name, const char* what) {
    TORCH_CHECK(t.device() == dev && t.scalar_type() == dt, name, what);
    TORCH_CHECK(t.is_contiguous(), name, " must be contiguous");
    TORCH_CHECK(t.numel() == n, name, " must have as many elements as p32");
    TORCH_CHECK((reinterpret_cast<uintptr_t>(t.data_ptr()) & 15) == 0, name,
                " must be 16-byte aligned");
  };
  flat(p32, at::kFloat, "p32", " must be an fp32 tensor");
  flat(p16, at::kBFloat16, "p16", " must be a bf16 tensor on the device of p32");
  flat(g32, at::kFloat, "g32", " must be an fp32 tensor on the device of p32");
  for (const auto& s : state)
    flat(*s.first, at::kFloat, s.second, " must be an fp32 tensor on the device of p32");
  auto word = [&](const Tensor& t, const char* name) {
    TORCH_CHECK(t.device() == dev && t.scalar_type() == at::kFloat && t.numel() == 1, name,
                " must be a one-element fp32 tensor on the device of p32");
  };
  word(lr, "lr");
  if (step != nullptr) word(*step, "step");
}

void dense_adagrad(Tensor p32, Tensor p16, Tensor g32, Tensor acc, const Tensor& lr, double eps) {
  check_dense_opt(p32, p16, g32, {{&acc, "acc"}}, lr, nullptr);
  c10::cuda::CUDAGuard guard(p32.device());
  de::launch_dense_opt(de::kOptAdagrad, p32.data_ptr<float>(), p16.data_ptr(),
                       g32.data_ptr<float>(), acc.data_ptr<float>(), nullptr,
                       lr.data_ptr<float>(), nullptr, 0.f, 0.f, static_cast<float>(eps),
                       p32.numel(), sm_count(), cur_stream());
  check_launch();
}

void dense_adam(Tensor p32, Tensor p16, Tensor g32, Tensor m, Tensor v, const Tensor& lr,
                const Tensor& step, double beta1, double beta2, double eps) {
  check_dense_opt(p32, p16, g32, {{&m, "m"}, {&v, "v"}}, lr, &step);
  c10::cuda::CUDAGuard guard(p32.device());
  de::launch_dense_opt(de::kOptAdam, p32.data_ptr<float>(), p16.data_ptr(),
                       g32.data_ptr<float>(), m.data_ptr<float>(), v.data_ptr<float>(),
                       lr.data_ptr<float>(), step.data_ptr<float>(), static_cast<float>(beta1),
                       static_cast<float>(beta2), static_cast<float>(eps), p32.numel(),
                       sm_count(), cur_stream());
  check_launch();
}

void cast_pad(const Tensor& src, Tensor dst) {
  TORCH_CHECK(src.is_cuda() && src.scalar_type() == at::kFloat && src.is_contiguous());
  TORCH_CHECK(dst.scalar_type() == at::kBFloat16 && dst.is_contiguous() &&
              dst.size(0) == src.size(0) && dst.size(1) >= src.size(1));
  c10::cuda::CUDAGuard guard(src.device());
  de::launch_cast_pad(src.data_ptr<float>(), static_cast<int>(src.size(1)), dst.data_ptr(),
                      static_cast<int>(dst.size(1)), src.size(0), cur_stream());
  check_launch();
}

void gemm_tn_bias_act(const Tensor& a, const Tensor& b, const c10::optional<Tensor>& bias,
                      Tensor out, bool relu, int64_t block_n) {
  check_bf16_2d(a, "a");
  check_bf16_2d(b, "b");
  check_bf16_2d(out, "out");
  TORCH_CHECK(a.size(1) == b.size(1) && out.size(0) == a.size(0) && out.size(1) == b.size(0),
              "shape mismatch");
  if (bias.has_value())
    TORCH_CHECK(bias->is_cuda() && bias->scalar_type() == at::kBFloat16 && bias->is_contiguous() &&
                bias->numel() == b.size(0));
  c10::cuda::CUDAGuard guard(a.device());
  bool ok = de::launch_gemm_tn_bias_act(
      a.data_ptr(), a.stride(0), b.data_ptr(), b.stride(0),
      bias.has_value() ? bias->data_ptr() : nullptr, out.data_ptr(), out.stride(0),
      static_cast<int>(a.size(0)), static_cast<int>(b.size(0)), static_cast<int>(a.size(1)), relu,
      static_cast<int>(block_n), sm_count(), cur_stream());
  TORCH_CHECK(ok, "gemm_tn_bias_act: unsupported shape/alignment or launch failure");
  check_launch();
}

void gemm_dgrad_relu_bias(const Tensor& dy, const Tensor& wt, const Tensor& act, Tensor dx,
                          Tensor colsum, int64_t block_n) {
  check_bf16_2d(dy, "dy");
  check_bf16_2d(wt, "wt");
  check_bf16_2d(act, "act");
  check_bf16_2d(dx, "dx");
  TORCH_CHECK(dy.size(1) == wt.size(1) && dx.size(0) == dy.size(0) && dx.size(1) == wt.size(0) &&
              act.size(0) == dx.size(0) && act.size(1) == dx.size(1), "shape mismatch");
  TORCH_CHECK(colsum.is_cuda() && colsum.scalar_type() == at::kFloat &&
              colsum.numel() >= dx.size(1));
  c10::cuda::CUDAGuard guard(dy.device());
  bool ok = de::launch_gemm_tn_fused(
      dy.data_ptr(), dy.stride(0), wt.data_ptr(), wt.stride(0), nullptr, dx.data_ptr(),
      dx.stride(0), static_cast<int>(dy.size(0)), static_cast<int>(wt.size(0)),
      static_cast<int>(dy.size(1)), 2, act.data_ptr(), act.stride(0), colsum.data_ptr<float>(),
      static_cast<int>(block_n), sm_count(), cur_stream());
  TORCH_CHECK(ok, "gemm_dgrad_relu_bias: unsupported shape/alignment or launch failure");
  check_launch();
}

Tensor symm_alloc(int64_t nbytes, int64_t device_index) {
  c10::cuda::CUDAGuard guard(static_cast<c10::DeviceIndex>(device_index));
  void* ptr = nullptr;
  const size_t padded = (static_cast<size_t>(nbytes) + 255) & ~static_cast<size_t>(255);
  DE_CUDA_CHECK(cudaMalloc(&ptr, padded));
  DE_CUDA_CHECK(cudaMemset(ptr, 0, padded));
  DE_CUDA_CHECK(cudaDeviceSynchronize());
  auto deleter = [](void* p) { cudaFree(p); };
  return at::from_blob(ptr, {static_cast<int64_t>(padded)}, deleter,
                       at::TensorOptions()
                           .device(at::Device(at::kCUDA, static_cast<c10::DeviceIndex>(device_index)))
                           .dtype(at::kByte));
}

Tensor ipc_get_handle(const Tensor& buf) {
  TORCH_CHECK(buf.is_cuda());
  cudaIpcMemHandle_t h;
  DE_CUDA_CHECK(cudaIpcGetMemHandle(&h, buf.data_ptr()));
  Tensor out = at::empty({static_cast<int64_t>(sizeof(h))}, at::TensorOptions().dtype(at::kByte));
  std::memcpy(out.data_ptr(), &h, sizeof(h));
  return out;
}

int64_t ipc_open(const Tensor& handle, int64_t device_index) {
  TORCH_CHECK(!handle.is_cuda() && handle.numel() == sizeof(cudaIpcMemHandle_t));
  c10::cuda::CUDAGuard guard(static_cast<c10::DeviceIndex>(device_index));
  cudaIpcMemHandle_t h;
  std::memcpy(&h, handle.data_ptr(), sizeof(h));
  void* ptr = nullptr;
  DE_CUDA_CHECK(cudaIpcOpenMemHandle(&ptr, h, cudaIpcMemLazyEnablePeerAccess));
  return reinterpret_cast<int64_t>(ptr);
}

void ipc_close(int64_t ptr, int64_t device_index) {
  c10::cuda::CUDAGuard guard(static_cast<c10::DeviceIndex>(device_index));
  cudaIpcCloseMemHandle(reinterpret_cast<void*>(ptr));
}

de::CacheTable to_cache(at::TensorList cache, at::IntArrayRef host, int64_t n_sets,
                        int64_t n_spill, int64_t rows) {
  TORCH_CHECK(cache.size() == 8, "offload cache: 8 tensors expected");
  TORCH_CHECK(host.size() == 3, "offload cache: 3 host pointers expected");
  TORCH_CHECK(n_sets >= 1 && n_sets < (int64_t(1) << 31) && n_spill >= 0 && rows >= 1 &&
                  rows < (int64_t(1) << 32) - 1,
              "offload cache: bad geometry (n_sets ", n_sets, ", n_spill ", n_spill, ", rows ",
              rows, ")");
  const int64_t slots = n_sets * 32 + n_spill;
  const Tensor& w = cache[0];
  TORCH_CHECK(w.is_cuda() && w.scalar_type() == at::kFloat && w.is_contiguous() && w.dim() == 2 &&
                  w.size(0) == slots && w.size(1) >= 1 && w.data_ptr() != nullptr,
              "offload cache: weight must be a contiguous fp32 CUDA tensor [", slots, ", width]");
  TORCH_CHECK(w.size(1) % 4 != 0 || (reinterpret_cast<uintptr_t>(w.data_ptr()) % 16 == 0 &&
                                     host[0] % 16 == 0),
              "offload cache: rows of width % 4 == 0 must be 16-byte aligned");
  TORCH_CHECK(host[0] != 0, "offload cache: host table pointer is null");
  de::CacheTable T{};
  T.weight = w.data_ptr<float>();
  T.host_weight = reinterpret_cast<float*>(host[0]);
  T.width = static_cast<int32_t>(w.size(1));
  float** cs[2] = {&T.state0, &T.state1};
  float** hs[2] = {&T.host_state0, &T.host_state1};
  int32_t* sw[2] = {&T.state0_width, &T.state1_width};
  for (int k = 0; k < 2; ++k) {
    const Tensor& s = cache[1 + k];
    if (s.numel() == 0) {
      TORCH_CHECK(host[1 + k] == 0, "offload cache: host state without a cache state");
      continue;
    }
    TORCH_CHECK(s.is_cuda() && s.scalar_type() == at::kFloat && s.is_contiguous() &&
                    s.size(0) == slots && (s.dim() == 1 || (s.dim() == 2 && s.size(1) == w.size(1))),
                "offload cache: state must be fp32 CUDA [slots] or [slots, width]");
    TORCH_CHECK(host[1 + k] != 0 && host[1 + k] % 16 == 0 &&
                    reinterpret_cast<uintptr_t>(s.data_ptr()) % 16 == 0,
                "offload cache: host state pointer is null or misaligned");
    *cs[k] = s.data_ptr<float>();
    *hs[k] = reinterpret_cast<float*>(host[1 + k]);
    *sw[k] = static_cast<int32_t>(s.dim() == 1 ? 1 : s.size(1));
  }
  auto check_i = [&](const Tensor& t, at::ScalarType ty, int64_t n, const char* what) {
    TORCH_CHECK(t.is_cuda() && t.scalar_type() == ty && t.is_contiguous() && t.numel() == n &&
                    t.device() == w.device(),
                "offload cache: ", what, " must be a contiguous CUDA tensor of ", n, " elements");
  };
  check_i(cache[3], at::kLong, slots, "tags (int64)");
  check_i(cache[4], at::kInt, n_sets * 32, "ticks (int32)");
  check_i(cache[5], at::kInt, slots, "dirty (int32)");
  check_i(cache[6], at::kInt, 1, "tick_word (int32)");
  check_i(cache[7], at::kLong, 4, "stats (int64)");
  T.tags = cache[3].data_ptr<int64_t>();
  T.ticks = cache[4].data_ptr<int32_t>();
  T.dirty = cache[5].data_ptr<int32_t>();
  T.tick_word = cache[6].data_ptr<int32_t>();
  T.stats = cache[7].data_ptr<int64_t>();
  T.n_sets = n_sets;
  T.n_spill = n_spill;
  T.rows = rows;
  return T;
}

void offload_cache_pass(at::TensorList cache, at::IntArrayRef host, int64_t n_sets,
                        int64_t n_spill, int64_t rows, const Tensor& descs, const Tensor& tables,
                        int64_t n_inputs, int64_t batch, bool ids64, int64_t n_items,
                        bool prefill_sentinel, const Tensor& remap, int64_t n_remap,
                        int64_t max_remap_n, int64_t out_ptr, bool train) {
  de::CacheTable T = to_cache(cache, host, n_sets, n_spill, rows);
  TORCH_CHECK(n_items == n_spill && n_items >= 1,
              "offload cache: the spill region must hold every id of the step (", n_items,
              " ids, ", n_spill, " spill slots)");
  TORCH_CHECK(n_items < (int64_t(1) << 31), "offload cache: too many ids per step");
  TORCH_CHECK(descs.is_cuda() && tables.is_cuda() && remap.is_cuda() &&
                  descs.device() == cache[0].device() && remap.device() == cache[0].device(),
              "offload cache: descriptors must live on the cache's GPU");
  TORCH_CHECK(descs.numel() == n_inputs * static_cast<int64_t>(sizeof(de::InputDesc)) &&
                  tables.numel() == static_cast<int64_t>(sizeof(de::TableDesc)) &&
                  remap.numel() == n_remap * static_cast<int64_t>(sizeof(de::CacheRemap)) &&
                  n_inputs >= 1 && n_remap >= 1 && max_remap_n >= 0,
              "offload cache: descriptor array sizes do not match their counts");
  TORCH_CHECK(out_ptr != 0 && out_ptr % (ids64 ? 8 : 4) == 0, "offload cache: bad slot-id buffer");
  TORCH_CHECK(n_sets * 32 + n_spill < (ids64 ? (int64_t(1) << 62) : (int64_t(1) << 31)),
              "offload cache: slot ids do not fit the id type");
  c10::cuda::CUDAGuard guard(cache[0].device());
  auto stream = cur_stream();
  auto dev = cache[0].device();
  auto i64 = at::TensorOptions().device(dev).dtype(at::kLong);
  auto i32 = at::TensorOptions().device(dev).dtype(at::kInt);
  de::launch_cache_spill_writeback(T, sm_count(), stream);
  check_launch();
  auto sorted = sort_items(descs, tables, 1, n_inputs, batch, batch, {}, ids64, n_items, rows,
                           prefill_sentinel);
  const Tensor& keys = std::get<0>(sorted);
  const Tensor& seg_start = std::get<2>(sorted);
  const Tensor& n_unique = std::get<3>(sorted);
  Tensor uniq = at::empty({n_items}, i64), slot_of = at::empty({n_items}, i64);
  Tensor move = at::empty({n_items}, i64);
  Tensor set_a = at::empty({n_items}, i32), item_a = at::empty({n_items}, i32);
  Tensor set_b = at::empty({n_items}, i32), item_b = at::empty({n_items}, i32);
  Tensor set_sorted = at::empty({n_items}, i64);
  Tensor seg = at::empty({n_items + 1}, i64), n_seg = at::zeros({1}, i64);
  const size_t temp_bytes =
      std::max(de::radix_sort_temp_bytes(n_items), de::head_segments_temp_bytes(n_items));
  Tensor temp = at::empty({static_cast<int64_t>(temp_bytes)},
                          at::TensorOptions().device(dev).dtype(at::kByte));
  de::launch_cache_probe(T, keys.data_ptr<int64_t>(), seg_start.data_ptr<int64_t>(),
                         n_unique.data_ptr<int64_t>(), n_items, train, uniq.data_ptr<int64_t>(),
                         reinterpret_cast<uint32_t*>(set_a.data_ptr<int>()),
                         reinterpret_cast<uint32_t*>(item_a.data_ptr<int>()),
                         slot_of.data_ptr<int64_t>(), move.data_ptr<int64_t>(), sm_count(), stream);
  check_launch();
  int where = de::radix_sort_pairs32(
      temp.data_ptr(), reinterpret_cast<uint32_t*>(set_a.data_ptr<int>()),
      reinterpret_cast<uint32_t*>(item_a.data_ptr<int>()),
      reinterpret_cast<uint32_t*>(set_b.data_ptr<int>()),
      reinterpret_cast<uint32_t*>(item_b.data_ptr<int>()), set_sorted.data_ptr<int64_t>(), n_items,
      bit_length(n_sets), stream);
  const Tensor& u_sorted = where == 0 ? item_a : item_b;
  de::head_segments(temp.data_ptr(), set_sorted.data_ptr<int64_t>(), n_items,
                    seg.data_ptr<int64_t>(), n_seg.data_ptr<int64_t>(), stream);
  check_launch();
  de::launch_cache_assign(T, set_sorted.data_ptr<int64_t>(),
                          reinterpret_cast<const uint32_t*>(u_sorted.data_ptr<int>()),
                          seg.data_ptr<int64_t>(), n_seg.data_ptr<int64_t>(), n_items, train,
                          uniq.data_ptr<int64_t>(), slot_of.data_ptr<int64_t>(),
                          move.data_ptr<int64_t>(), sm_count(), stream);
  check_launch();
  de::launch_cache_fill(T, n_unique.data_ptr<int64_t>(), n_items, uniq.data_ptr<int64_t>(),
                        slot_of.data_ptr<int64_t>(), move.data_ptr<int64_t>(), sm_count(), stream);
  check_launch();
  de::launch_cache_remap(reinterpret_cast<const de::CacheRemap*>(remap.data_ptr()),
                         static_cast<int>(n_remap), max_remap_n, uniq.data_ptr<int64_t>(),
                         n_unique.data_ptr<int64_t>(), slot_of.data_ptr<int64_t>(), rows, ids64,
                         reinterpret_cast<void*>(out_ptr), sm_count(), stream);
  check_launch();
}

void offload_cache_flush(at::TensorList cache, at::IntArrayRef host, int64_t n_sets,
                         int64_t n_spill, int64_t rows) {
  de::CacheTable T = to_cache(cache, host, n_sets, n_spill, rows);
  c10::cuda::CUDAGuard guard(cache[0].device());
  de::launch_cache_flush(T, sm_count(), cur_stream());
  check_launch();
}

int64_t host_device_pointer(const Tensor& host) {
  TORCH_CHECK(!host.is_cuda());
  void* dptr = nullptr;
  DE_CUDA_CHECK(cudaHostGetDevicePointer(&dptr, host.data_ptr(), 0));
  return reinterpret_cast<int64_t>(dptr);
}

}

TORCH_LIBRARY(de_b200, m) {
  m.def("struct_sizes() -> int[]", &struct_sizes);
  m.def(
      "sync_ctx_create(int[] flag_ptrs, Tensor state, int rank, int world, int timeout_cycles, "
      "int error_ptr) -> int",
      &sync_ctx_create);
  m.def("sync_only(int[] sync) -> ()", &sync_only);
  m.def(
      "lookup_fwd(Tensor descs, int n_inputs, int batch, int src_batch, int dst_batch, "
      "int dst_stride, int[] src_ptrs, int[] dst_ptrs, int rot, bool ids64, int act_dtype, "
      "bool vec4, int[] sync, int tile_samples, int table_dtype=0, bool vec8=False) -> ()",
      &lookup_fwd);
  m.def(
      "scatter_add_bwd(Tensor descs, int n_inputs, int batch, int src_batch, int grad_batch, "
      "int grad_stride, int[] src_ptrs, int[] grad_ptrs, int rot, float scale, int scale_ptr, bool ids64, "
      "int act_dtype, bool vec4, bool vec8, int[] sync, bool staged) -> ()",
      &scatter_add_bwd);
  m.def(
      "sort_items(Tensor descs, Tensor tables, int n_tables, int n_inputs, int batch, "
      "int src_batch, int[] src_ptrs, bool ids64, int n_items, int total_rows, "
      "bool prefill_sentinel) -> "
      "(Tensor, Tensor, Tensor, Tensor)",
      &sort_items);
  m.def("radix_sort_pairs(Tensor keys, Tensor items, int end_bit) -> (Tensor, Tensor)",
        &radix_sort_pairs);
  m.def("radix_sort_pairs32(Tensor keys, Tensor items, int end_bit) -> (Tensor, Tensor)",
        &radix_sort_pairs32);
  m.def("head_segments(Tensor sorted_keys) -> (Tensor, Tensor)", &head_segments);
  m.def(
      "segment_update(Tensor descs, Tensor tables, int n_tables, int batch, int grad_batch, "
      "int grad_stride, int[] grad_ptrs, Tensor sorted_keys, Tensor sorted_items, "
      "Tensor seg_start, Tensor n_unique, int opt_kind, float lr, float eps, float beta1, "
      "float beta2, float bias1, float bias2, float grad_scale, float weight_decay, int lr_ptr, "
      "Tensor? emit_keys, Tensor? emit_rows, int max_width, int act_dtype, bool vec4, "
      "Tensor? scratch, int step_ptr, int table_dtype=0, int state_dtype=0, "
      "float lr_power=-0.5, float l1=0., float l2=0., float l2_shrinkage=0., "
      "float ftrl_beta=0.) -> ()",
      &segment_update);
  m.def(
      "embedding_lookup_fwd(Tensor param, Tensor values, Tensor? offsets, int hotness, int batch, "
      "int combiner, bool out_bf16) -> Tensor",
      &embedding_lookup_fwd);
  m.def(
      "embedding_scatter_add(Tensor(a!) dst, Tensor values, Tensor? offsets, int hotness, "
      "int batch, int combiner, Tensor grad, float scale) -> ()",
      &embedding_scatter_add);
  m.def(
      "embedding_lookup_grad(Tensor values, Tensor? offsets, int hotness, int batch, int combiner, "
      "Tensor grad, int num_rows) -> (Tensor, Tensor)",
      &embedding_lookup_grad);
  m.def("row_to_split(Tensor indices, int num_rows) -> Tensor", &row_to_split);
  m.def("hash_init(Tensor(a!) table) -> ()", &hash_init);
  m.def(
      "integer_lookup(Tensor(a!) table, Tensor(b!) count, Tensor(c!) next_index, Tensor keys, "
      "int capacity) -> Tensor",
      &integer_lookup);
  m.def(
      "barrier(int[] flag_ptrs, Tensor(a!) epoch, int rank, int world, int channel, "
      "int timeout_cycles, int error_ptr) -> ()",
      &barrier);
  m.def(
      "allreduce(int[] buf_ptrs, int[] flag_ptrs, Tensor(a!) epoch, int rank, int world, "
      "int n_elems, float scale, bool bf16, int channel, int timeout_cycles, "
      "int error_ptr, int mc_ptr, int max_blocks) -> ()",
      &allreduce);
  m.def("gather_segments(Tensor segs, int[] src_ptrs, Tensor(a!) dst, int max_seg_elems) -> ()",
        &gather_segments);
  m.def(
      "p2p_store_bench(Tensor src, int dst_ptr, int n_rows, int row_bytes, int vec_bytes, "
      "int dst_stride, int unroll, int blocks, int threads) -> ()",
      &p2p_store_bench);
  m.def(
      "push_segments(Tensor segs, Tensor src, int[] dst_ptrs, int max_seg_elems, int[] sync) -> ()",
      &push_segments);
  m.def(
      "push_grad(Tensor routes, int n_routes, Tensor src, int dst_dtype, float scale, int[] sync) "
      "-> ()",
      &push_grad);
  m.def(
      "stream_push(int[] src_ptrs, int[] dst_ptrs, int[] row_bytes, Tensor counters, "
      "int chunk_rows, int rows, int blocks, int[] sync) -> ()",
      &stream_push);
  m.def(
      "rowslice_reduce(Tensor partial, int out_ptr, int out_stride, int out_dtype, Tensor cols) "
      "-> ()",
      &rowslice_reduce);
  m.def(
      "gather_ragged(Tensor segs, int[] val_ptrs, int[] split_ptrs, Tensor(a!) dst_vals, "
      "Tensor(b!) goff, int b, int max_cap) -> ()",
      &gather_ragged);
  m.def("select_copy(Tensor[] src0, Tensor[] src1, Tensor(a!)[] dst, Tensor slot_flag) -> ()",
        &select_copy);
  m.def("copy_cast_2d(Tensor src, int dst_ptr, int dst_stride, int dst_dtype, float scale) -> ()",
        &copy_cast_2d);
  m.def("interact_fwd(Tensor bottom, Tensor emb, int n_emb, Tensor(a!) z, int[] sync) -> ()",
        &interact_fwd);
  m.def(
      "interact_bwd(Tensor bottom, Tensor emb, int n_emb, Tensor dz, Tensor(a!) dbottom, "
      "int demb_ptr, int demb_stride, float emb_grad_scale, Tensor? routes, int n_routes, "
      "int[] sync, Tensor? done_counters, int chunk_rows, Tensor? apply_descs=None, "
      "float apply_scale=0.0, int apply_scale_ptr=0, bool apply_ids64=False) -> ()",
      &interact_bwd);
  m.def("avgpool_fwd(Tensor x, int n, Tensor(a!) out, int stride) -> ()", &avgpool_fwd);
  m.def("avgpool_bwd(Tensor dout, Tensor(a!) dx, int n, int stride) -> ()", &avgpool_bwd);
  m.def("relu_bwd_bias(Tensor(a!) dy, Tensor y, Tensor(b!) db) -> ()", &relu_bwd_bias);
  m.def("cross_fwd(Tensor x0, Tensor s, Tensor xl, Tensor(a!) out) -> ()", &cross_fwd);
  m.def("cross_bwd(Tensor dy, Tensor x0, Tensor(a!) g, Tensor(b!) db) -> ()", &cross_bwd);
  m.def(
      "cross_dx0(Tensor d_chain, Tensor[] dy, Tensor[] s, Tensor(a!) dx0, Tensor(b!) d_bottom) "
      "-> ()",
      &cross_dx0);
  m.def(
      "head_loss(Tensor x, Tensor w, Tensor bias, Tensor labels, float inv_batch, Tensor(a!) dx, "
      "Tensor(b!) dw, Tensor(c!) db, Tensor(d!) dbias_prev, Tensor(e!) loss_sum, Tensor? logits) "
      "-> ()",
      &head_loss);
  m.def(
      "head_eval(Tensor x, Tensor w, Tensor bias, Tensor labels, Tensor n_valid, Tensor(a!) probs, "
      "Tensor(b!) hist, Tensor(c!) loss_sum, Tensor(d!) count) -> ()",
      &head_eval);
  m.def(
      "dense_sgd(Tensor(a!) p32, Tensor(b!) p16, Tensor(c!) g32, Tensor lr, float grad_scale) "
      "-> ()",
      &dense_sgd);
  m.def(
      "dense_adagrad(Tensor(a!) p32, Tensor(b!) p16, Tensor(c!) g32, Tensor(d!) acc, Tensor lr, "
      "float eps) -> ()",
      &dense_adagrad);
  m.def(
      "dense_adam(Tensor(a!) p32, Tensor(b!) p16, Tensor(c!) g32, Tensor(d!) m, Tensor(e!) v, "
      "Tensor lr, Tensor step, float beta1, float beta2, float eps) -> ()",
      &dense_adam);
  m.def("cast_pad(Tensor src, Tensor(a!) dst) -> ()", &cast_pad);
  m.def(
      "gemm_tn_bias_act(Tensor a, Tensor b, Tensor? bias, Tensor(a!) out, bool relu, int block_n) "
      "-> ()",
      &gemm_tn_bias_act);
  m.def(
      "gemm_dgrad_relu_bias(Tensor dy, Tensor wt, Tensor act, Tensor(a!) dx, Tensor(b!) colsum, "
      "int block_n) -> ()",
      &gemm_dgrad_relu_bias);
  m.def("symm_alloc(int nbytes, int device_index) -> Tensor", &symm_alloc);
  m.def("ipc_get_handle(Tensor buf) -> Tensor", &ipc_get_handle);
  m.def("ipc_open(Tensor handle, int device_index) -> int", &ipc_open);
  m.def("ipc_close(int ptr, int device_index) -> ()", &ipc_close);
  m.def("host_device_pointer(Tensor host) -> int", &host_device_pointer);
  m.def(
      "offload_cache_pass(Tensor[] cache, int[] host, int n_sets, int n_spill, int rows, "
      "Tensor descs, Tensor tables, int n_inputs, int batch, bool ids64, int n_items, "
      "bool prefill_sentinel, Tensor remap, int n_remap, int max_remap_n, int out_ptr, "
      "bool train) -> ()",
      &offload_cache_pass);
  m.def("offload_cache_flush(Tensor[] cache, int[] host, int n_sets, int n_spill, int rows) -> ()",
        &offload_cache_flush);
}
```

distributed_embeddings_b200/ops/csrc/de_b200.h:

```cpp
#pragma once
#include <cuda_runtime.h>
#include <stdint.h>

namespace de {

constexpr int kMaxPeers = 16;
constexpr int kGridCapSms = 132;

struct alignas(16) InputDesc {
  const void* table;
  const void* ids;
  const int64_t* offsets;
  int64_t ids_off;
  int64_t id_shift;
  int64_t sub_rows;
  int64_t row_base;
  int32_t width;
  int32_t hotness;
  int32_t dst_col;
  int32_t combiner;
  int32_t local_table;
  int32_t flags;
  int64_t item_off;
};

struct PeerPtrs {
  void* p[kMaxPeers];
};

constexpr int kSyncChannels = 16;
constexpr int kSyncStateWords = 64;
struct SyncArgs {
  PeerPtrs flags;
  uint32_t* state;
  int* error_flag;
  unsigned long long timeout;
  int32_t rank, world;
  int32_t wait_ch;
  int32_t wait_abs_ch;
  int32_t signal_ch;
  int32_t counter_slot;
};
inline SyncArgs no_sync() {
  SyncArgs s{};
  s.state = nullptr;
  s.wait_ch = s.wait_abs_ch = s.signal_ch = -1;
  return s;
}

struct alignas(16) GradRoute {
  void* dst;
  int64_t dst_stride;
  int32_t src_col;
  int32_t width;
  int32_t dst_col;
  int32_t pad;
};

enum OptimizerKind : int32_t {
  kOptSGD = 0,
  kOptAdagrad = 1,
  kOptRowwiseAdagrad = 2,
  kOptAdam = 3,
  kOptEmit = 4,
  kOptRowwiseAdam = 5,
  kOptFtrl = 6,
};

struct alignas(16) TableDesc {
  void* weight;
  void* state0;
  void* state1;
  int64_t rows;
  int64_t key_base;
  int32_t width;
  int32_t pad;
};

struct OptimizerArgs {
  int32_t kind;
  float lr;
  float eps;
  float beta1, beta2;
  float bias1, bias2;
  float grad_scale;
  float weight_decay;
  const float* lr_ptr;
  const float* step_ptr;
  float lr_power;
  float l1, l2;
  float l2_shrinkage;
  float ftrl_beta;
};

void launch_lookup_fwd(const InputDesc* descs, int n_inputs, int64_t batch, int64_t src_batch,
                       int64_t dst_batch, int64_t dst_stride, const PeerPtrs& src,
                       const PeerPtrs& dst, int rot, bool ids64, int act_dtype, bool vec4,
                       int sm_count, cudaStream_t stream, const SyncArgs& sync,
                       int tile_samples = 32, int table_dtype = 0, bool vec8 = false);

void launch_scatter_add_bwd(const InputDesc* descs, int n_inputs, int64_t batch, int64_t src_batch,
                            int64_t grad_batch, int64_t grad_stride, const PeerPtrs& src,
                            const PeerPtrs& grad, int rot, float scale, const float* scale_ptr,
                            bool ids64, int act_dtype, bool vec4, int sm_count,
                            cudaStream_t stream, bool vec8, const SyncArgs& sync,
                            bool staged = false);

void launch_build_keys(const InputDesc* descs, const TableDesc* tables, int n_tables, int n_inputs,
                       int64_t batch, int64_t src_batch, const PeerPtrs& src, bool ids64, void* keys,
                       uint32_t* items, int sm_count, cudaStream_t stream, bool keys32 = false);
size_t sort_pairs_temp_bytes(int64_t n);
void sort_pairs(void* temp, size_t temp_bytes, const int64_t* keys_in, int64_t* keys_out,
                const uint32_t* items_in, uint32_t* items_out, int64_t n, int end_bit,
                cudaStream_t stream);
size_t unique_temp_bytes(int64_t n);
void unique_segments(void* temp, size_t temp_bytes, const int64_t* sorted_keys, int64_t n,
                     int64_t* seg_start, int64_t* n_unique, cudaStream_t stream);
size_t radix_sort_temp_bytes(int64_t n);
int radix_sort_pairs(void* temp, int64_t* keys_a, uint32_t* items_a, int64_t* keys_b,
                     uint32_t* items_b, int64_t n, int end_bit, cudaStream_t stream);
int radix_sort_pairs32(void* temp, uint32_t* keys_a, uint32_t* items_a, uint32_t* keys_b,
                       uint32_t* items_b, int64_t* keys_out64, int64_t n, int end_bit,
                       cudaStream_t stream);
size_t head_segments_temp_bytes(int64_t n);
void head_segments(void* temp, const int64_t* sorted_keys, int64_t n, int64_t* seg_start,
                   int64_t* n_unique, cudaStream_t stream);
void launch_segment_update(const InputDesc* descs, const TableDesc* tables, int n_tables,
                           int64_t batch, int64_t grad_batch, int64_t grad_stride,
                           const PeerPtrs& grad, const int64_t* sorted_keys,
                           const uint32_t* sorted_items, const int64_t* seg_start,
                           const int64_t* n_unique, int64_t n_items, const OptimizerArgs& opt,
                           int64_t* emit_keys, float* emit_rows, int max_width, int act_dtype,
                           bool vec4, int sm_count, cudaStream_t stream, int table_dtype = 0,
                           int state_dtype = 0);

bool launch_balanced_update(const InputDesc* descs, const TableDesc* tables, int n_tables,
                            int64_t batch, int64_t grad_batch, int64_t grad_stride,
                            const PeerPtrs& grad, const int64_t* sorted_keys,
                            const uint32_t* sorted_items, int64_t n_items,
                            const int64_t* seg_start, const int64_t* n_unique,
                            const OptimizerArgs& opt, float* scratch, int scratch_width,
                            int max_width, int act_dtype, int sm_count, cudaStream_t stream,
                            int table_dtype = 0, int state_dtype = 0);

struct CacheTable {
  float* weight;
  float* state0;
  float* state1;
  float* host_weight;
  float* host_state0;
  float* host_state1;
  int64_t* tags;
  int32_t* ticks;
  int32_t* dirty;
  int32_t* tick_word;
  int64_t* stats;
  int64_t n_sets;
  int64_t n_spill;
  int64_t rows;
  int32_t width;
  int32_t state0_width;
  int32_t state1_width;
  int32_t pad;
};
struct alignas(16) CacheRemap {
  const void* ids;
  int64_t n;
  int64_t id_shift;
  int64_t sub_rows;
  int64_t row_base;
  int64_t out_off;
};
void launch_cache_spill_writeback(const CacheTable& T, int sm_count, cudaStream_t stream);
void launch_cache_probe(const CacheTable& T, const int64_t* sorted_keys, const int64_t* seg_start,
                        const int64_t* n_unique, int64_t cap, bool train, int64_t* uniq,
                        uint32_t* miss_set, uint32_t* miss_item, int64_t* slot_of, int64_t* move,
                        int sm_count, cudaStream_t stream);
void launch_cache_assign(const CacheTable& T, const int64_t* set_sorted, const uint32_t* u_sorted,
                         const int64_t* seg, const int64_t* n_seg, int64_t cap, bool train,
                         const int64_t* uniq, int64_t* slot_of, int64_t* move, int sm_count,
                         cudaStream_t stream);
void launch_cache_fill(const CacheTable& T, const int64_t* n_unique, int64_t cap,
                       const int64_t* uniq, const int64_t* slot_of, const int64_t* move,
                       int sm_count, cudaStream_t stream);
void launch_cache_remap(const CacheRemap* inputs, int n_inputs, int64_t max_n,
                        const int64_t* uniq, const int64_t* n_unique, const int64_t* slot_of,
                        int64_t rows, bool ids64, void* out, int sm_count, cudaStream_t stream);
void launch_cache_flush(const CacheTable& T, int sm_count, cudaStream_t stream);

void launch_row_to_split(const int64_t* coo_indices, int64_t nnz, int64_t num_rows,
                         int64_t* row_splits, cudaStream_t stream);
void launch_hash_init(int64_t* table, int64_t n_slots, cudaStream_t stream);
void launch_integer_lookup(int64_t* table, int64_t n_slots, uint32_t* counts, int64_t* next_index,
                           const int64_t* keys, int64_t n, int64_t capacity, int64_t* out,
                           cudaStream_t stream);

void launch_barrier(const PeerPtrs& flags, uint32_t* epoch, int rank, int world, int channel,
                    unsigned long long timeout_cycles, int* error_flag, cudaStream_t stream);
void launch_allreduce(const PeerPtrs& bufs, const PeerPtrs& flags, uint32_t* epoch, int rank,
                      int world, int64_t n_elems, float scale, bool bf16, int channel,
                      unsigned long long timeout_cycles, int* error_flag, int sm_count,
                      cudaStream_t stream, int max_blocks = 0);
void launch_allreduce_multimem(void* mc_ptr, const PeerPtrs& flags, uint32_t* epoch, int rank,
                               int world, int64_t n_elems, float scale, bool bf16, int channel,
                               unsigned long long timeout_cycles, int* error_flag, int sm_count,
                               cudaStream_t stream, int max_blocks = 0);
void launch_p2p_store_bench(const void* src, void* dst, int64_t n_rows, int row_bytes,
                            int vec_bytes, int64_t dst_stride, int unroll, int blocks, int threads,
                            cudaStream_t stream);
void launch_sync_only(const SyncArgs& sync, cudaStream_t stream);
void launch_push_segments(const int64_t* segs, int n_seg, const void* src, const PeerPtrs& dst,
                          int elem_bytes, int64_t max_seg_elems, int sm_count,
                          cudaStream_t stream, const SyncArgs& sync);
void launch_push_grad(const GradRoute* routes, int n_routes, const void* src, int64_t src_stride,
                      int src_dtype, int dst_dtype, int64_t rows, float scale, int sm_count,
                      cudaStream_t stream, const SyncArgs& sync);
struct PushPlan {
  const void* src[kMaxPeers];
  void* dst[kMaxPeers];
  int64_t row_bytes[kMaxPeers];
  int32_t n;
};
void launch_stream_push(const PushPlan& plan, const uint32_t* counters, int chunk_rows,
                        int64_t rows, unsigned long long timeout, int* error_flag, int blocks,
                        cudaStream_t stream, const SyncArgs& sync);
void launch_rowslice_reduce(const float* partial, int world, int64_t rows, int64_t part_stride,
                            void* out, int64_t out_stride, int out_dtype, const int32_t* cols,
                            int n_cols, cudaStream_t stream);
void launch_gather_segments(const int64_t* segs, int n_seg, const PeerPtrs& src, void* dst,
                            int elem_bytes, int64_t max_seg_elems, cudaStream_t stream);
void launch_gather_ragged(const int64_t* segs, int n_seg, const PeerPtrs& src_vals,
                          const PeerPtrs& src_splits, void* dst_vals, int64_t* goff, int64_t b,
                          int world, int elem_bytes, int64_t max_cap, cudaStream_t stream);
void launch_select_copy(const void* const* src0, const void* const* src1, void* const* dst,
                        const int64_t* nbytes, int count, const int* slot_flag, int sm_count,
                        cudaStream_t stream);
void launch_copy_cast_2d(const void* src, int64_t src_stride, void* dst, int64_t dst_stride,
                         int64_t rows, int64_t cols, int src_dtype, int dst_dtype, float scale,
                         cudaStream_t stream);

bool launch_interact_fwd(const void* bottom, int64_t bottom_stride, const void* emb,
                         int64_t emb_stride, int n_emb, int dim, void* z, int64_t z_stride,
                         int z_width, int64_t batch, int sm_count, cudaStream_t stream,
                         const SyncArgs& sync);
constexpr int kMaxInteractApply = 31;
struct InteractApply {
  float* table[kMaxInteractApply];
  const void* ids[kMaxInteractApply];
  int64_t row_base[kMaxInteractApply];
  int64_t sub_rows[kMaxInteractApply];
  int64_t id_shift[kMaxInteractApply];
  const float* scale_ptr;
  float scale;
  uint32_t mask;
  int32_t ids64;
};

bool launch_interact_bwd(const void* bottom, int64_t bottom_stride, const void* emb,
                         int64_t emb_stride, int n_emb, int dim, const void* dz,
                         int64_t dz_stride, void* dbottom, int64_t dbottom_stride, void* demb,
                         int64_t demb_stride, float emb_grad_scale, int64_t batch, int sm_count,
                         cudaStream_t stream, const GradRoute* routes, int n_routes,
                         const SyncArgs& sync, uint32_t* done_counters = nullptr,
                         int chunk_rows = 0, const InteractApply* apply = nullptr);
void launch_avgpool_fwd(const void* x, int64_t x_stride, int n, void* out, int64_t out_stride,
                        int out_len, int stride, int left, int64_t rows, cudaStream_t stream);
void launch_avgpool_bwd(const void* dout, int64_t dout_stride, int out_len, void* dx,
                        int64_t dx_stride, int n, int stride, int left, int64_t rows,
                        cudaStream_t stream);
void launch_relu_bwd_bias(void* dy, const void* y, float* db, int64_t rows, int cols,
                          cudaStream_t stream);
constexpr int kMaxCrossLayers = 8;
struct CrossTerms {
  const void* dy[kMaxCrossLayers];
  const void* s[kMaxCrossLayers];
  int n;
};
void launch_cross_fwd(const void* x0, const void* s, const void* xl, void* out, int64_t n,
                      int sm_count, cudaStream_t stream);
void launch_cross_bwd(const void* dy, const void* x0, void* g, float* db, int64_t rows, int cols,
                      cudaStream_t stream);
void launch_cross_dx0(const void* d_chain, const CrossTerms& terms, void* dx0, void* d_bottom,
                      int64_t rows, int cols, int emb_cols, cudaStream_t stream);
bool launch_head_loss(const void* x, int K, const void* w, const void* bias, const float* labels,
                      int64_t batch, float inv_batch, void* dx, float* dw, float* db,
                      float* dbias_prev, float* loss_sum, float* logits_out, int sm_count,
                      cudaStream_t stream);
bool launch_head_eval(const void* x, int K, const void* w, const void* bias, const float* labels,
                      int64_t batch, const int64_t* n_valid, float* probs, int64_t* hist, int nb,
                      double* loss_sum, int64_t* count, int sm_count, cudaStream_t stream);
void launch_sgd_update(float* p32, void* p16, float* g32, const float* lr_ptr, float grad_scale,
                       int64_t n, int sm_count, cudaStream_t stream);
bool launch_dense_opt(int kind, float* p32, void* p16, float* g32, float* s0, float* s1,
                      const float* lr_ptr, const float* step_ptr, float beta1, float beta2,
                      float eps, int64_t n, int sm_count, cudaStream_t stream);
void launch_cast_pad(const float* src, int src_cols, void* dst, int dst_cols, int64_t rows,
                     cudaStream_t stream);

bool launch_gemm_tn_fused(const void* A, int64_t lda, const void* B, int64_t ldb, const void* bias,
                          void* C, int64_t ldc, int M, int N, int K, int epi, const void* act,
                          int64_t ldact, float* colsum, int block_n, int sm_count,
                          cudaStream_t stream);
bool launch_gemm_tn_bias_act(const void* A, int64_t lda, const void* B, int64_t ldb,
                             const void* bias, void* C, int64_t ldc, int M, int N, int K,
                             bool relu, int block_n, int sm_count, cudaStream_t stream);

}
```

distributed_embeddings_b200/ops/csrc/gemm_wgmma.cu:

```cuda
#include <cuda.h>
#include <cuda_bf16.h>
#include <cuda_runtime.h>
#include <stdint.h>

#include <atomic>
#include <mutex>

#include "de_b200.h"

namespace de {

namespace {

using bf16 = __nv_bfloat16;

constexpr int BLOCK_M = 128;
constexpr int BLOCK_K = 64;
constexpr int WGMMA_N = 128;
constexpr int WGMMA_K = 16;
constexpr int kGemmThreads = 384;
constexpr int kMaxColsum = 2048;

__device__ __forceinline__ uint32_t smem_addr(const void* p) {
  return static_cast<uint32_t>(__cvta_generic_to_shared(p));
}
__device__ __forceinline__ void mbar_init(uint64_t* bar, uint32_t count) {
  asm volatile("mbarrier.init.shared::cta.b64 [%0], %1;" ::"r"(smem_addr(bar)), "r"(count));
}
__device__ __forceinline__ void mbar_expect_tx(uint64_t* bar, uint32_t bytes) {
  asm volatile("mbarrier.arrive.expect_tx.shared::cta.b64 _, [%0], %1;" ::"r"(smem_addr(bar)),
               "r"(bytes)
               : "memory");
}
__device__ __forceinline__ void mbar_arrive(uint64_t* bar) {
  asm volatile("mbarrier.arrive.shared::cta.b64 _, [%0];" ::"r"(smem_addr(bar)) : "memory");
}
__device__ __forceinline__ void mbar_wait(uint64_t* bar, uint32_t parity) {
  uint32_t done;
  do {
    asm volatile(
        "{\n"
        ".reg .pred p;\n"
        "mbarrier.try_wait.parity.shared::cta.b64 p, [%1], %2;\n"
        "selp.u32 %0, 1, 0, p;\n"
        "}\n"
        : "=r"(done)
        : "r"(smem_addr(bar)), "r"(parity)
        : "memory");
  } while (!done);
}
__device__ __forceinline__ void mbar_wait_cluster(uint64_t* bar, uint32_t parity) {
  uint32_t done;
  do {
    asm volatile(
        "{\n"
        ".reg .pred p;\n"
        "mbarrier.try_wait.parity.acquire.cluster.shared::cta.b64 p, [%1], %2;\n"
        "selp.u32 %0, 1, 0, p;\n"
        "}\n"
        : "=r"(done)
        : "r"(smem_addr(bar)), "r"(parity)
        : "memory");
  } while (!done);
}
__device__ __forceinline__ void fence_barrier_init() {
  asm volatile("fence.mbarrier_init.release.cluster;" ::: "memory");
}
__device__ __forceinline__ void fence_proxy_async() {
  asm volatile("fence.proxy.async.shared::cta;" ::: "memory");
}
__device__ __forceinline__ void tma_load_2d(void* smem_dst, const CUtensorMap* map, uint64_t* bar,
                                            int c0, int c1) {
  asm volatile(
      "cp.async.bulk.tensor.2d.shared::cluster.global.mbarrier::complete_tx::bytes [%0], [%1, "
      "{%3, %4}], [%2];" ::"r"(smem_addr(smem_dst)),
      "l"(map), "r"(smem_addr(bar)), "r"(c0), "r"(c1)
      : "memory");
}
__device__ __forceinline__ void tma_load_2d_multicast(void* smem_dst, const CUtensorMap* map,
                                                      uint64_t* bar, int c0, int c1,
                                                      uint16_t cta_mask) {
  asm volatile(
      "cp.async.bulk.tensor.2d.shared::cluster.global.mbarrier::complete_tx::bytes.multicast::"
      "cluster [%0], [%1, {%3, %4}], [%2], %5;" ::"r"(smem_addr(smem_dst)),
      "l"(map), "r"(smem_addr(bar)), "r"(c0), "r"(c1), "h"(cta_mask)
      : "memory");
}
__device__ __forceinline__ void tma_prefetch_desc(const CUtensorMap* map) {
  asm volatile("prefetch.tensormap [%0];" ::"l"(map) : "memory");
}
__device__ __forceinline__ void cp_async_16(void* smem_dst, const void* src, uint32_t src_bytes) {
  asm volatile("cp.async.cg.shared.global [%0], [%1], 16, %2;" ::"r"(smem_addr(smem_dst)),
               "l"(src), "r"(src_bytes)
               : "memory");
}
__device__ __forceinline__ void cp_async_commit() {
  asm volatile("cp.async.commit_group;" ::: "memory");
}
__device__ __forceinline__ void cp_async_wait_all() {
  asm volatile("cp.async.wait_group 0;" ::: "memory");
}
__device__ __forceinline__ uint32_t lds_b32(uint32_t a) {
  uint32_t v;
  asm volatile("ld.shared.b32 %0, [%1];" : "=r"(v) : "r"(a) : "memory");
  return v;
}
__device__ __forceinline__ void sts_b32(uint32_t a, uint32_t v) {
  asm volatile("st.shared.b32 [%0], %1;" ::"r"(a), "r"(v) : "memory");
}
__device__ __forceinline__ uint4 lds_b128(uint32_t a) {
  uint4 v;
  asm volatile("ld.shared.v4.b32 {%0, %1, %2, %3}, [%4];"
               : "=r"(v.x), "=r"(v.y), "=r"(v.z), "=r"(v.w)
               : "r"(a)
               : "memory");
  return v;
}
__device__ __forceinline__ void red_add_f32(float* gmem, float v) {
  asm volatile("red.global.add.f32 [%0], %1;" ::"l"(gmem), "f"(v) : "memory");
}
__device__ __forceinline__ void warpgroup_bar_sync(int cw) {
  asm volatile("bar.sync %0, 128;" ::"r"(2 + cw) : "memory");
}

__device__ __forceinline__ void wgmma_fence() {
  asm volatile("wgmma.fence.sync.aligned;" ::: "memory");
}
__device__ __forceinline__ void wgmma_commit() {
  asm volatile("wgmma.commit_group.sync.aligned;" ::: "memory");
}
template <int N>
__device__ __forceinline__ void wgmma_wait() {
  asm volatile("wgmma.wait_group.sync.aligned %0;" ::"n"(N) : "memory");
}
__device__ __forceinline__ void wgmma_m64n128k16(float (&d)[64], uint64_t desc_a, uint64_t desc_b,
                                                 uint32_t accumulate) {
  asm volatile(
      "{\n"
      ".reg .pred p;\n"
      "setp.ne.b32 p, %66, 0;\n"
      "wgmma.mma_async.sync.aligned.m64n128k16.f32.bf16.bf16 "
      "{%0,%1,%2,%3,%4,%5,%6,%7,%8,%9,%10,%11,%12,%13,%14,%15,%16,%17,%18,%19,%20,%21,%22,%23,%24,"
      "%25,%26,%27,%28,%29,%30,%31,%32,%33,%34,%35,%36,%37,%38,%39,%40,%41,%42,%43,%44,%45,%46,%47,"
      "%48,%49,%50,%51,%52,%53,%54,%55,%56,%57,%58,%59,%60,%61,%62,%63}, "
      "%64, %65, p, 1, 1, 0, 0;\n"
      "}\n"
      : "+f"(d[0]), "+f"(d[1]), "+f"(d[2]), "+f"(d[3]), "+f"(d[4]), "+f"(d[5]), "+f"(d[6]),
        "+f"(d[7]), "+f"(d[8]), "+f"(d[9]), "+f"(d[10]), "+f"(d[11]), "+f"(d[12]), "+f"(d[13]),
        "+f"(d[14]), "+f"(d[15]), "+f"(d[16]), "+f"(d[17]), "+f"(d[18]), "+f"(d[19]), "+f"(d[20]),
        "+f"(d[21]), "+f"(d[22]), "+f"(d[23]), "+f"(d[24]), "+f"(d[25]), "+f"(d[26]), "+f"(d[27]),
        "+f"(d[28]), "+f"(d[29]), "+f"(d[30]), "+f"(d[31]), "+f"(d[32]), "+f"(d[33]), "+f"(d[34]),
        "+f"(d[35]), "+f"(d[36]), "+f"(d[37]), "+f"(d[38]), "+f"(d[39]), "+f"(d[40]), "+f"(d[41]),
        "+f"(d[42]), "+f"(d[43]), "+f"(d[44]), "+f"(d[45]), "+f"(d[46]), "+f"(d[47]), "+f"(d[48]),
        "+f"(d[49]), "+f"(d[50]), "+f"(d[51]), "+f"(d[52]), "+f"(d[53]), "+f"(d[54]), "+f"(d[55]),
        "+f"(d[56]), "+f"(d[57]), "+f"(d[58]), "+f"(d[59]), "+f"(d[60]), "+f"(d[61]), "+f"(d[62]),
        "+f"(d[63])
      : "l"(desc_a), "l"(desc_b), "r"(accumulate)
      : "memory");
}

__device__ __forceinline__ uint64_t make_sw128_kmajor_desc(uint32_t smem_byte_addr) {
  uint64_t d = 0;
  d |= static_cast<uint64_t>((smem_byte_addr & 0x3FFFF) >> 4);
  d |= static_cast<uint64_t>(1) << 16;
  d |= static_cast<uint64_t>(1024 >> 4) << 32;
  d |= static_cast<uint64_t>(1) << 62;
  return d;
}

template <int BLOCK_N, int STAGES, int EPI = 0>
struct SmemLayout {
  static constexpr int kABytes = BLOCK_M * BLOCK_K * 2;
  static constexpr int kBBytes = BLOCK_N * BLOCK_K * 2;
  static constexpr int kStageBytes = kABytes + kBBytes;
  static constexpr int kActRowBytes = BLOCK_N * 2 + 16;
  static constexpr int kActWgBytes = 64 * kActRowBytes;
  static constexpr int kActOffset = STAGES * kStageBytes;
  static constexpr int kColsumOffset = kActOffset + (EPI == 2 ? 2 * kActWgBytes : 0);
  static constexpr int kBarOffset = kColsumOffset + kMaxColsum * 4;
  static_assert(8 * BLOCK_N <= kMaxColsum, "per-warp column sums exceed their region");
  static constexpr int kNumBars = 2 * STAGES;
  static constexpr int kTileOffset = kBarOffset + kNumBars * 8;
  static constexpr int kTotal = kTileOffset + STAGES * 4;
};

constexpr int kSchedSlots = 256;
__device__ unsigned int g_tile_sched[kSchedSlots][2];

template <int BLOCK_N, int STAGES, int EPI, bool CLUSTER>
__device__ __forceinline__ void consumer_tile(uint8_t* smem, uint64_t* full_bar, uint64_t* empty_bar,
                                              int& stage, uint32_t& phase, int m0, int n0,
                                              int num_kb, int cw, const bf16* __restrict__ bias,
                                              bf16* __restrict__ C, int64_t ldc, int M, int N,
                                              const bf16* __restrict__ act, int64_t ldact,
                                              float* colsum, float (&acc)[BLOCK_N / WGMMA_N][64]) {
  using L = SmemLayout<BLOCK_N, STAGES, EPI>;
  constexpr int NB = BLOCK_N / WGMMA_N;
  const int lane = threadIdx.x & 31, warp_in_wg = (threadIdx.x >> 5) & 3;
  const bool releaser = warp_in_wg == 0 && lane == 0;
  const int row0 = m0 + cw * 64 + warp_in_wg * 16 + (lane >> 2);
  uint8_t* s_act = smem + L::kActOffset + cw * L::kActWgBytes;
  const uint32_t s_act_a = smem_addr(s_act);
  const uint32_t s_part_a = smem_addr(smem + L::kColsumOffset) + cw * 4 * BLOCK_N * 4;
  constexpr int kRowChunks = BLOCK_N / 8;
  const int wt = threadIdx.x & 127;
  if constexpr (EPI == 2) {
    warpgroup_bar_sync(cw);
#pragma unroll 4
    for (int c = wt; c < 64 * kRowChunks; c += 128) {
      const int r = c / kRowChunks, cc = c % kRowChunks;
      const int row = m0 + cw * 64 + r, col = n0 + cc * 8;
      const bool ok = row < M && col < N;
      cp_async_16(s_act + r * L::kActRowBytes + cc * 16,
                  act + (ok ? static_cast<int64_t>(row) * ldact + col : 0), ok ? 16u : 0u);
    }
    cp_async_commit();
  }
  int prev_stage = -1;
  for (int kb = 0; kb < num_kb; ++kb) {
    mbar_wait(&full_bar[stage], phase);
    const uint32_t sa = smem_addr(smem + stage * L::kStageBytes) + cw * 64 * 128;
    const uint32_t sb = smem_addr(smem + stage * L::kStageBytes + L::kABytes);
    wgmma_fence();
#pragma unroll
    for (int k = 0; k < BLOCK_K / WGMMA_K; ++k) {
      const uint64_t da = make_sw128_kmajor_desc(sa + k * WGMMA_K * 2);
#pragma unroll
      for (int nb = 0; nb < NB; ++nb) {
        const uint64_t db = make_sw128_kmajor_desc(sb + nb * WGMMA_N * 128 + k * WGMMA_K * 2);
        wgmma_m64n128k16(acc[nb], da, db, (kb | k) != 0 ? 1u : 0u);
      }
    }
    wgmma_commit();
    wgmma_wait<1>();
    if (prev_stage >= 0 && releaser) {
      if (CLUSTER) {
        for (uint32_t r = 0; r < 2; ++r) {
          const uint32_t a = smem_addr(&empty_bar[prev_stage]);
          uint32_t remote;
          asm volatile("mapa.shared::cluster.u32 %0, %1, %2;" : "=r"(remote) : "r"(a), "r"(r));
          asm volatile("mbarrier.arrive.release.cluster.shared::cluster.b64 _, [%0];" ::"r"(remote)
                       : "memory");
        }
      } else {
        mbar_arrive(&empty_bar[prev_stage]);
      }
    }
    prev_stage = stage;
    if (++stage == STAGES) {
      stage = 0;
      phase ^= 1;
    }
  }
  wgmma_wait<0>();
  if (prev_stage >= 0 && releaser) {
    if (CLUSTER) {
      for (uint32_t r = 0; r < 2; ++r) {
        const uint32_t a = smem_addr(&empty_bar[prev_stage]);
        uint32_t remote;
        asm volatile("mapa.shared::cluster.u32 %0, %1, %2;" : "=r"(remote) : "r"(a), "r"(r));
        asm volatile("mbarrier.arrive.release.cluster.shared::cluster.b64 _, [%0];" ::"r"(remote)
                     : "memory");
      }
    } else {
      mbar_arrive(&empty_bar[prev_stage]);
    }
  }

  if constexpr (EPI == 2) {
    cp_async_wait_all();
    warpgroup_bar_sync(cw);
  }
#pragma unroll
  for (int nb = 0; nb < NB; ++nb) {
#pragma unroll
    for (int j = 0; j < WGMMA_N / 8; ++j) {
      const int col = n0 + nb * WGMMA_N + j * 8 + (lane & 3) * 2;
      const bool col_ok = col < N;
      float b0 = 0.f, b1 = 0.f;
      if (EPI != 2 && bias != nullptr && col_ok) {
        const float2 bb = __bfloat1622float2(*reinterpret_cast<const __nv_bfloat162*>(bias + col));
        b0 = bb.x;
        b1 = bb.y;
      }
      float cs0 = 0.f, cs1 = 0.f;
#pragma unroll
      for (int i = 0; i < 2; ++i) {
        const int row = row0 + 8 * i;
        float v0 = acc[nb][4 * j + 2 * i], v1 = acc[nb][4 * j + 2 * i + 1];
        if constexpr (EPI == 2) {
          const uint32_t sp = s_act_a + (row - m0 - cw * 64) * L::kActRowBytes + (col - n0) * 2;
          const uint32_t a = lds_b32(sp);
          v0 = __uint_as_float(a << 16) > 0.f ? v0 : 0.f;
          v1 = __uint_as_float(a & 0xffff0000u) > 0.f ? v1 : 0.f;
          cs0 += v0;
          cs1 += v1;
          const __nv_bfloat162 r = __floats2bfloat162_rn(v0, v1);
          sts_b32(sp, *reinterpret_cast<const uint32_t*>(&r));
        } else {
          v0 += b0;
          v1 += b1;
          if (EPI == 1) {
            v0 = fmaxf(v0, 0.f);
            v1 = fmaxf(v1, 0.f);
          }
          if (row < M && col_ok)
            *reinterpret_cast<__nv_bfloat162*>(C + static_cast<int64_t>(row) * ldc + col) =
                __floats2bfloat162_rn(v0, v1);
        }
      }
      if (EPI == 2) {
#pragma unroll
        for (int sft = 4; sft < 32; sft <<= 1) {
          cs0 += __shfl_xor_sync(0xffffffffu, cs0, sft);
          cs1 += __shfl_xor_sync(0xffffffffu, cs1, sft);
        }
        if (lane < 4) {
          const uint32_t sp = s_part_a + (warp_in_wg * BLOCK_N + col - n0) * 4;
          sts_b32(sp, __float_as_uint(cs0));
          sts_b32(sp + 4, __float_as_uint(cs1));
        }
      }
    }
  }
  if constexpr (EPI == 2) {
    warpgroup_bar_sync(cw);
    for (int c = wt; c < BLOCK_N; c += 128) {
      const uint32_t sp = s_part_a + c * 4;
      const float v = __uint_as_float(lds_b32(sp)) + __uint_as_float(lds_b32(sp + BLOCK_N * 4)) +
                      __uint_as_float(lds_b32(sp + 2 * BLOCK_N * 4)) +
                      __uint_as_float(lds_b32(sp + 3 * BLOCK_N * 4));
      if (n0 + c < N && v != 0.f) red_add_f32(colsum + n0 + c, v);
    }
#pragma unroll 4
    for (int c = wt; c < 64 * kRowChunks; c += 128) {
      const int r = c / kRowChunks, cc = c % kRowChunks;
      const int row = m0 + cw * 64 + r, col = n0 + cc * 8;
      if (row < M && col < N)
        *reinterpret_cast<uint4*>(C + static_cast<int64_t>(row) * ldc + col) =
            lds_b128(s_act_a + r * L::kActRowBytes + cc * 16);
    }
  }
}

template <int BLOCK_N, int STAGES, int EPI>
__global__ void __launch_bounds__(kGemmThreads, 1)
gemm_tn_fused_kernel(const __grid_constant__ CUtensorMap tma_a,
                     const __grid_constant__ CUtensorMap tma_b, const bf16* __restrict__ bias,
                     bf16* __restrict__ C, int64_t ldc, int M, int N, int K,
                     const bf16* __restrict__ act, int64_t ldact, float* __restrict__ colsum,
                     int sched_slot) {
  using L = SmemLayout<BLOCK_N, STAGES, EPI>;
  extern __shared__ uint8_t smem_raw[];
  uint8_t* smem = reinterpret_cast<uint8_t*>(
      (reinterpret_cast<uintptr_t>(smem_raw) + 1023) & ~static_cast<uintptr_t>(1023));
  uint64_t* full_bar = reinterpret_cast<uint64_t*>(smem + L::kBarOffset);
  uint64_t* empty_bar = full_bar + STAGES;
  volatile int* s_tile = reinterpret_cast<int*>(smem + L::kTileOffset);

  const int wg = threadIdx.x >> 7;
  const int num_kb = (K + BLOCK_K - 1) / BLOCK_K;
  const int tiles_n = (N + BLOCK_N - 1) / BLOCK_N;
  const int tiles_m = (M + BLOCK_M - 1) / BLOCK_M;
  const int num_tiles = tiles_n * tiles_m;

  if (threadIdx.x == 0) {
    tma_prefetch_desc(&tma_a);
    tma_prefetch_desc(&tma_b);
    for (int s = 0; s < STAGES; ++s) {
      mbar_init(&full_bar[s], 1);
      mbar_init(&empty_bar[s], 2);
    }
    fence_barrier_init();
    fence_proxy_async();
  }
  __syncthreads();

  if (wg == 0) {
    if (threadIdx.x == 0) {
      unsigned int* sched = g_tile_sched[sched_slot];
      int stage = 0;
      uint32_t phase = 0;
      for (int tile = blockIdx.x;;) {
        const int next = static_cast<int>(gridDim.x + atomicAdd(&sched[0], 1u));
        const bool done = tile >= num_tiles;
        const int m0 = (tile / tiles_n) * BLOCK_M, n0 = (tile % tiles_n) * BLOCK_N;
        for (int kb = 0; kb < num_kb; ++kb) {
          mbar_wait(&empty_bar[stage], phase ^ 1);
          if (kb == 0) s_tile[stage] = done ? -1 : tile;
          if (done) {
            mbar_arrive(&full_bar[stage]);
            break;
          }
          uint8_t* sa = smem + stage * L::kStageBytes;
          uint8_t* sb = sa + L::kABytes;
          mbar_expect_tx(&full_bar[stage], L::kStageBytes);
          tma_load_2d(sa, &tma_a, &full_bar[stage], kb * BLOCK_K, m0);
          tma_load_2d(sb, &tma_b, &full_bar[stage], kb * BLOCK_K, n0);
          if (++stage == STAGES) {
            stage = 0;
            phase ^= 1;
          }
        }
        if (done) break;
        tile = next;
      }
      __threadfence();
      if (atomicAdd(&sched[1], 1u) == gridDim.x - 1) {
        __threadfence();
        atomicExch(&sched[0], 0u);
        atomicExch(&sched[1], 0u);
      }
    }
  } else {
    const int cw = wg - 1;
    float acc[BLOCK_N / WGMMA_N][64];
#pragma unroll
    for (int nb = 0; nb < BLOCK_N / WGMMA_N; ++nb)
#pragma unroll
      for (int r = 0; r < 64; ++r) acc[nb][r] = 0.f;
    int stage = 0;
    uint32_t phase = 0;
    for (;;) {
      mbar_wait(&full_bar[stage], phase);
      const int tile = s_tile[stage];
      if (tile < 0) break;
      const int m0 = (tile / tiles_n) * BLOCK_M, n0 = (tile % tiles_n) * BLOCK_N;
      consumer_tile<BLOCK_N, STAGES, EPI, false>(smem, full_bar, empty_bar, stage, phase, m0, n0,
                                                 num_kb, cw, bias, C, ldc, M, N, act, ldact,
                                                 colsum, acc);
    }
  }
}

__device__ __forceinline__ uint32_t cluster_ctarank() {
  uint32_t r;
  asm volatile("mov.u32 %0, %%cluster_ctarank;" : "=r"(r));
  return r;
}
__device__ __forceinline__ void cluster_sync_all() {
  asm volatile("barrier.cluster.arrive.release.aligned;" ::: "memory");
  asm volatile("barrier.cluster.wait.acquire.aligned;" ::: "memory");
}

template <int BLOCK_N, int STAGES, int EPI>
__global__ void __cluster_dims__(2, 1, 1) __launch_bounds__(kGemmThreads, 1)
gemm_tn_pair_kernel(const __grid_constant__ CUtensorMap tma_a,
                    const __grid_constant__ CUtensorMap tma_b, const bf16* __restrict__ bias,
                    bf16* __restrict__ C, int64_t ldc, int M, int N, int K) {
  using L = SmemLayout<BLOCK_N, STAGES>;
  constexpr int kHalfB = L::kBBytes / 2;
  extern __shared__ uint8_t smem_raw[];
  uint8_t* smem = reinterpret_cast<uint8_t*>(
      (reinterpret_cast<uintptr_t>(smem_raw) + 1023) & ~static_cast<uintptr_t>(1023));
  uint64_t* full_bar = reinterpret_cast<uint64_t*>(smem + L::kBarOffset);
  uint64_t* empty_bar = full_bar + STAGES;

  const int wg = threadIdx.x >> 7;
  const uint32_t cta_rank = cluster_ctarank();
  const int pair = blockIdx.x >> 1, num_pairs = gridDim.x >> 1;
  const int num_kb = (K + BLOCK_K - 1) / BLOCK_K;
  const int tiles_n = (N + BLOCK_N - 1) / BLOCK_N;
  const int tiles_m = (M + 2 * BLOCK_M - 1) / (2 * BLOCK_M);
  const int num_tiles = tiles_n * tiles_m;

  if (threadIdx.x == 0) {
    tma_prefetch_desc(&tma_a);
    tma_prefetch_desc(&tma_b);
    for (int s = 0; s < STAGES; ++s) {
      mbar_init(&full_bar[s], 1);
      mbar_init(&empty_bar[s], 4);
    }
    fence_barrier_init();
    fence_proxy_async();
  }
  __syncthreads();
  cluster_sync_all();

  if (wg == 0) {
    if (threadIdx.x == 0) {
      int stage = 0;
      uint32_t phase = 0;
      for (int tile = pair; tile < num_tiles; tile += num_pairs) {
        const int m0 = (tile / tiles_n) * (2 * BLOCK_M) + static_cast<int>(cta_rank) * BLOCK_M;
        const int n0 = (tile % tiles_n) * BLOCK_N + static_cast<int>(cta_rank) * (BLOCK_N / 2);
        for (int kb = 0; kb < num_kb; ++kb) {
          mbar_wait_cluster(&empty_bar[stage], phase ^ 1);
          uint8_t* sa = smem + stage * L::kStageBytes;
          uint8_t* sb = sa + L::kABytes + cta_rank * kHalfB;
          mbar_expect_tx(&full_bar[stage], L::kStageBytes);
          tma_load_2d(sa, &tma_a, &full_bar[stage], kb * BLOCK_K, m0);
          tma_load_2d_multicast(sb, &tma_b, &full_bar[stage], kb * BLOCK_K, n0, 0x3);
          if (++stage == STAGES) {
            stage = 0;
            phase ^= 1;
          }
        }
      }
    }
  } else {
    const int cw = wg - 1;
    float acc[BLOCK_N / WGMMA_N][64];
#pragma unroll
    for (int nb = 0; nb < BLOCK_N / WGMMA_N; ++nb)
#pragma unroll
      for (int r = 0; r < 64; ++r) acc[nb][r] = 0.f;
    int stage = 0;
    uint32_t phase = 0;
    for (int tile = pair; tile < num_tiles; tile += num_pairs) {
      const int m0 = (tile / tiles_n) * (2 * BLOCK_M) + static_cast<int>(cta_rank) * BLOCK_M;
      const int n0 = (tile % tiles_n) * BLOCK_N;
      consumer_tile<BLOCK_N, STAGES, EPI, true>(smem, full_bar, empty_bar, stage, phase, m0, n0,
                                                num_kb, cw, bias, C, ldc, M, N, nullptr, 0,
                                                nullptr, acc);
    }
  }
  __syncthreads();
  cluster_sync_all();
}

using EncodeFn = CUresult (*)(CUtensorMap*, CUtensorMapDataType, cuuint32_t, void*,
                              const cuuint64_t*, const cuuint64_t*, const cuuint32_t*,
                              const cuuint32_t*, CUtensorMapInterleave, CUtensorMapSwizzle,
                              CUtensorMapL2promotion, CUtensorMapFloatOOBfill);

EncodeFn get_encode_fn() {
  static EncodeFn fn = nullptr;
  static std::once_flag once;
  std::call_once(once, [] {
    void* p = nullptr;
    cudaDriverEntryPointQueryResult q;
    if (cudaGetDriverEntryPoint("cuTensorMapEncodeTiled", &p, cudaEnableDefault, &q) ==
            cudaSuccess &&
        q == cudaDriverEntryPointSuccess)
      fn = reinterpret_cast<EncodeFn>(p);
  });
  return fn;
}

bool make_tensor_map(CUtensorMap* map, const void* ptr, int64_t rows, int64_t cols,
                     int64_t row_stride_elems, int box_rows) {
  EncodeFn fn = get_encode_fn();
  if (fn == nullptr) return false;
  cuuint64_t gdim[2] = {static_cast<cuuint64_t>(cols), static_cast<cuuint64_t>(rows)};
  cuuint64_t gstride[1] = {static_cast<cuuint64_t>(row_stride_elems) * 2};
  cuuint32_t box[2] = {static_cast<cuuint32_t>(BLOCK_K), static_cast<cuuint32_t>(box_rows)};
  cuuint32_t estr[2] = {1, 1};
  CUresult r = fn(map, CU_TENSOR_MAP_DATA_TYPE_BFLOAT16, 2, const_cast<void*>(ptr), gdim, gstride,
                  box, estr, CU_TENSOR_MAP_INTERLEAVE_NONE, CU_TENSOR_MAP_SWIZZLE_128B,
                  CU_TENSOR_MAP_L2_PROMOTION_L2_256B, CU_TENSOR_MAP_FLOAT_OOB_FILL_NONE);
  return r == CUDA_SUCCESS;
}

int next_sched_slot() {
  static std::atomic<unsigned int> seq{0};
  return static_cast<int>(seq.fetch_add(1, std::memory_order_relaxed) % kSchedSlots);
}

template <int BLOCK_N, int STAGES, int EPI>
bool launch_one(const CUtensorMap& ta, const CUtensorMap& tb, const void* bias, void* C,
                int64_t ldc, int M, int N, int K, const void* act, int64_t ldact, float* colsum,
                int sm_count, cudaStream_t stream) {
  using L = SmemLayout<BLOCK_N, STAGES, EPI>;
  const size_t smem = L::kTotal + 1024;
  static_assert(L::kTotal + 1024 <= 227 * 1024, "exceeds the 227 KB of shared memory per block");
  const int tiles = ((N + BLOCK_N - 1) / BLOCK_N) * ((M + BLOCK_M - 1) / BLOCK_M);
  dim3 grid(tiles < sm_count ? tiles : sm_count);
  cudaFuncSetAttribute(gemm_tn_fused_kernel<BLOCK_N, STAGES, EPI>,
                       cudaFuncAttributeMaxDynamicSharedMemorySize, static_cast<int>(smem));
  gemm_tn_fused_kernel<BLOCK_N, STAGES, EPI><<<grid, kGemmThreads, smem, stream>>>(
      ta, tb, reinterpret_cast<const bf16*>(bias), reinterpret_cast<bf16*>(C), ldc, M, N, K,
      reinterpret_cast<const bf16*>(act), ldact, colsum, next_sched_slot());
  return cudaGetLastError() == cudaSuccess;
}

template <int BLOCK_N, int STAGES>
bool launch_cfg(const CUtensorMap& ta, const CUtensorMap& tb, const void* bias, void* C,
                int64_t ldc, int M, int N, int K, int epi, const void* act, int64_t ldact,
                float* colsum, int sm_count, cudaStream_t stream) {
  if (epi == 0)
    return launch_one<BLOCK_N, STAGES, 0>(ta, tb, bias, C, ldc, M, N, K, act, ldact, colsum,
                                          sm_count, stream);
  if (epi == 1)
    return launch_one<BLOCK_N, STAGES, 1>(ta, tb, bias, C, ldc, M, N, K, act, ldact, colsum,
                                          sm_count, stream);
  return launch_one<BLOCK_N, STAGES - 1, 2>(ta, tb, bias, C, ldc, M, N, K, act, ldact, colsum,
                                            sm_count, stream);
}

}

bool launch_gemm_tn_fused(const void* A, int64_t lda, const void* B, int64_t ldb, const void* bias,
                          void* C, int64_t ldc, int M, int N, int K, int epi, const void* act,
                          int64_t ldact, float* colsum, int block_n, int sm_count,
                          cudaStream_t stream) {
  if (M <= 0 || N <= 0 || K <= 0) return true;
  if ((lda % 8) || (ldb % 8) || (ldc % 8) || (N % 8)) return false;
  if ((reinterpret_cast<uintptr_t>(A) | reinterpret_cast<uintptr_t>(B) |
       reinterpret_cast<uintptr_t>(C)) & 15)
    return false;
  if (epi == 2 && (act == nullptr || colsum == nullptr || N > kMaxColsum || (ldact % 8) ||
                   (reinterpret_cast<uintptr_t>(act) & 15)))
    return false;
  const int bn = (block_n == 128 || block_n == 256) ? block_n : (N >= 256 ? 256 : 128);
  alignas(64) CUtensorMap ta, tb;
  if (!make_tensor_map(&ta, A, M, K, lda, BLOCK_M)) return false;
  if (!make_tensor_map(&tb, B, N, K, ldb, bn)) return false;
  if (bn == 256)
    return launch_cfg<256, 4>(ta, tb, bias, C, ldc, M, N, K, epi, act, ldact, colsum, sm_count,
                              stream);
  return launch_cfg<128, 6>(ta, tb, bias, C, ldc, M, N, K, epi, act, ldact, colsum, sm_count,
                            stream);
}

namespace {
template <int EPI>
bool launch_pair(const CUtensorMap& ta, const CUtensorMap& tb, const void* bias, void* C,
                 int64_t ldc, int M, int N, int K, int sm_count, cudaStream_t stream) {
  constexpr int BN = 256, ST = 4;
  using L = SmemLayout<BN, ST>;
  const size_t smem = L::kTotal + 1024;
  const int tiles = ((N + BN - 1) / BN) * ((M + 2 * BLOCK_M - 1) / (2 * BLOCK_M));
  int pairs = sm_count / 2;
  if (tiles < pairs) pairs = tiles;
  if (pairs < 1) return false;
  cudaFuncSetAttribute(gemm_tn_pair_kernel<BN, ST, EPI>,
                       cudaFuncAttributeMaxDynamicSharedMemorySize, static_cast<int>(smem));
  gemm_tn_pair_kernel<BN, ST, EPI><<<dim3(2 * pairs), kGemmThreads, smem, stream>>>(
      ta, tb, reinterpret_cast<const bf16*>(bias), reinterpret_cast<bf16*>(C), ldc, M, N, K);
  return cudaGetLastError() == cudaSuccess;
}
}

bool launch_gemm_tn_pair(const void* A, int64_t lda, const void* B, int64_t ldb, const void* bias,
                         void* C, int64_t ldc, int M, int N, int K, bool relu, int sm_count,
                         cudaStream_t stream) {
  if (M <= 0 || N <= 0 || K <= 0) return true;
  if ((lda % 8) || (ldb % 8) || (ldc % 8) || (N % 8)) return false;
  if ((reinterpret_cast<uintptr_t>(A) | reinterpret_cast<uintptr_t>(B) |
       reinterpret_cast<uintptr_t>(C)) & 15)
    return false;
  alignas(64) CUtensorMap ta, tb;
  if (!make_tensor_map(&ta, A, M, K, lda, BLOCK_M)) return false;
  if (!make_tensor_map(&tb, B, N, K, ldb, 128)) return false;
  return relu ? launch_pair<1>(ta, tb, bias, C, ldc, M, N, K, sm_count, stream)
              : launch_pair<0>(ta, tb, bias, C, ldc, M, N, K, sm_count, stream);
}

bool launch_gemm_tn_bias_act(const void* A, int64_t lda, const void* B, int64_t ldb,
                             const void* bias, void* C, int64_t ldc, int M, int N, int K,
                             bool relu, int block_n, int sm_count, cudaStream_t stream) {
  if (block_n == 512)
    return launch_gemm_tn_pair(A, lda, B, ldb, bias, C, ldc, M, N, K, relu, sm_count, stream);
  return launch_gemm_tn_fused(A, lda, B, ldb, bias, C, ldc, M, N, K, relu ? 1 : 0, nullptr, 0,
                              nullptr, block_n, sm_count, stream);
}

}
```

Measured before the change: 19.01 million.

## Rewrite fused GEMM epilogue with TMA stores, TMA activation prefetch and fixed 128-wide tiles

Restructures the persistent wgmma GEMM kernel so the epilogue writes output tiles through shared memory with TMA bulk stores. In the dgrad-relu path, the producer warp now prefetches the activation tile by TMA into double-buffered smem, replacing consumer-issued cp.async loads. Block N is fixed at 128 with 4 stages, which drops the per-layer 256/128 selection. The aim is to overlap epilogue I/O with the next tile's mainloop and cut consumer-side global traffic, at the cost of fewer pipeline stages and losing the wider tile for large-N layers.

```diff
diff --git a/distributed_embeddings_b200/models/dlrm_fast.py b/distributed_embeddings_b200/models/dlrm_fast.py
--- a/distributed_embeddings_b200/models/dlrm_fast.py
+++ b/distributed_embeddings_b200/models/dlrm_fast.py
@@ -24,10 +24,6 @@
 
 def _fused_dgrad(L) -> bool:
   return L.in_f == L.in_pad and L.in_f <= 2048 and L.out_f % 8 == 0
-
-
-def _dgrad_block_n(L) -> int:
-  return 128 if L.out_f <= 256 else 0
 
 
 class _Layer:
@@ -215,7 +211,7 @@
 
   def _dgrad_relu(self, L, x_below, dx, gb_below):
     if _fused_dgrad(L):
-      self.ops.gemm_dgrad_relu_bias(L.dy, L.w16T, x_below, dx, gb_below, _dgrad_block_n(L))
+      self.ops.gemm_dgrad_relu_bias(L.dy, L.w16T, x_below, dx, gb_below, 0)
     else:
       torch.mm(L.dy, L.w16, out=dx)
       self.ops.relu_bwd_bias(dx, x_below, gb_below)
diff --git a/distributed_embeddings_b200/ops/csrc/bindings.cpp b/distributed_embeddings_b200/ops/csrc/bindings.cpp
--- a/distributed_embeddings_b200/ops/csrc/bindings.cpp
+++ b/distributed_embeddings_b200/ops/csrc/bindings.cpp
@@ -1147,7 +1147,7 @@
       dy.data_ptr(), dy.stride(0), wt.data_ptr(), wt.stride(0), nullptr, dx.data_ptr(),
       dx.stride(0), static_cast<int>(dy.size(0)), static_cast<int>(wt.size(0)),
       static_cast<int>(dy.size(1)), 2, act.data_ptr(), act.stride(0), colsum.data_ptr<float>(),
-      static_cast<int>(block_n), sm_count(), cur_stream());
+      sm_count(), cur_stream());
   TORCH_CHECK(ok, "gemm_dgrad_relu_bias: unsupported shape/alignment or launch failure");
   check_launch();
 }
diff --git a/distributed_embeddings_b200/ops/csrc/de_b200.h b/distributed_embeddings_b200/ops/csrc/de_b200.h
--- a/distributed_embeddings_b200/ops/csrc/de_b200.h
+++ b/distributed_embeddings_b200/ops/csrc/de_b200.h
@@ -299,8 +299,7 @@
 
 bool launch_gemm_tn_fused(const void* A, int64_t lda, const void* B, int64_t ldb, const void* bias,
                           void* C, int64_t ldc, int M, int N, int K, int epi, const void* act,
-                          int64_t ldact, float* colsum, int block_n, int sm_count,
-                          cudaStream_t stream);
+                          int64_t ldact, float* colsum, int sm_count, cudaStream_t stream);
 bool launch_gemm_tn_bias_act(const void* A, int64_t lda, const void* B, int64_t ldb,
                              const void* bias, void* C, int64_t ldc, int M, int N, int K,
                              bool relu, int block_n, int sm_count, cudaStream_t stream);
diff --git a/distributed_embeddings_b200/ops/csrc/gemm_wgmma.cu b/distributed_embeddings_b200/ops/csrc/gemm_wgmma.cu
--- a/distributed_embeddings_b200/ops/csrc/gemm_wgmma.cu
+++ b/distributed_embeddings_b200/ops/csrc/gemm_wgmma.cu
@@ -20,6 +20,10 @@
 constexpr int WGMMA_K = 16;
 constexpr int kGemmThreads = 384;
 constexpr int kMaxColsum = 2048;
+constexpr int BLOCK_N = 128;
+constexpr int kStages = 4;
+constexpr int kEpiBar = 2;
+constexpr int kTurnBar = 4;
 
 __device__ __forceinline__ uint32_t smem_addr(const void* p) {
   return static_cast<uint32_t>(__cvta_generic_to_shared(p));
@@ -89,16 +93,18 @@
 __device__ __forceinline__ void tma_prefetch_desc(const CUtensorMap* map) {
   asm volatile("prefetch.tensormap [%0];" ::"l"(map) : "memory");
 }
-__device__ __forceinline__ void cp_async_16(void* smem_dst, const void* src, uint32_t src_bytes) {
-  asm volatile("cp.async.cg.shared.global [%0], [%1], 16, %2;" ::"r"(smem_addr(smem_dst)),
-               "l"(src), "r"(src_bytes)
-               : "memory");
-}
-__device__ __forceinline__ void cp_async_commit() {
-  asm volatile("cp.async.commit_group;" ::: "memory");
-}
-__device__ __forceinline__ void cp_async_wait_all() {
-  asm volatile("cp.async.wait_group 0;" ::: "memory");
+__device__ __forceinline__ void tma_store_2d(const CUtensorMap* map, uint32_t smem_src, int c0,
+                                             int c1) {
+  asm volatile(
+      "cp.async.bulk.tensor.2d.global.shared::cta.bulk_group [%0, {%2, %3}], [%1];" ::"l"(map),
+      "r"(smem_src), "r"(c0), "r"(c1)
+      : "memory");
+}
+__device__ __forceinline__ void bulk_commit_group() {
+  asm volatile("cp.async.bulk.commit_group;" ::: "memory");
+}
+__device__ __forceinline__ void bulk_wait_group_read0() {
+  asm volatile("cp.async.bulk.wait_group.read 0;" ::: "memory");
 }
 __device__ __forceinline__ uint32_t lds_b32(uint32_t a) {
   uint32_t v;
@@ -108,19 +114,14 @@
 __device__ __forceinline__ void sts_b32(uint32_t a, uint32_t v) {
   asm volatile("st.shared.b32 [%0], %1;" ::"r"(a), "r"(v) : "memory");
 }
-__device__ __forceinline__ uint4 lds_b128(uint32_t a) {
-  uint4 v;
-  asm volatile("ld.shared.v4.b32 {%0, %1, %2, %3}, [%4];"
-               : "=r"(v.x), "=r"(v.y), "=r"(v.z), "=r"(v.w)
-               : "r"(a)
-               : "memory");
-  return v;
-}
 __device__ __forceinline__ void red_add_f32(float* gmem, float v) {
   asm volatile("red.global.add.f32 [%0], %1;" ::"l"(gmem), "f"(v) : "memory");
 }
-__device__ __forceinline__ void warpgroup_bar_sync(int cw) {
-  asm volatile("bar.sync %0, 128;" ::"r"(2 + cw) : "memory");
+__device__ __forceinline__ void named_bar_sync(int id, int threads) {
+  asm volatile("bar.sync %0, %1;" ::"r"(id), "r"(threads) : "memory");
+}
+__device__ __forceinline__ void named_bar_arrive(int id, int threads) {
+  asm volatile("bar.arrive %0, %1;" ::"r"(id), "r"(threads) : "memory");
 }
 
 __device__ __forceinline__ void wgmma_fence() {
@@ -168,195 +169,41 @@
   return d;
 }
 
-template <int BLOCK_N, int STAGES, int EPI = 0>
+template <int EPI>
 struct SmemLayout {
   static constexpr int kABytes = BLOCK_M * BLOCK_K * 2;
   static constexpr int kBBytes = BLOCK_N * BLOCK_K * 2;
   static constexpr int kStageBytes = kABytes + kBBytes;
-  static constexpr int kActRowBytes = BLOCK_N * 2 + 16;
-  static constexpr int kActWgBytes = 64 * kActRowBytes;
-  static constexpr int kActOffset = STAGES * kStageBytes;
-  static constexpr int kColsumOffset = kActOffset + (EPI == 2 ? 2 * kActWgBytes : 0);
-  static constexpr int kBarOffset = kColsumOffset + kMaxColsum * 4;
-  static_assert(8 * BLOCK_N <= kMaxColsum, "per-warp column sums exceed their region");
-  static constexpr int kNumBars = 2 * STAGES;
+  static constexpr int kOutBoxBytes = BLOCK_M * 128;
+  static constexpr int kOutBytes = 2 * kOutBoxBytes;
+  static constexpr int kOutOffset = kStages * kStageBytes;
+  static constexpr int kColsumOffset = kOutOffset + 2 * kOutBytes;
+  static constexpr int kBarOffset = kColsumOffset + (EPI == 2 ? 8 * BLOCK_N * 4 : 0);
+  static constexpr int kNumBars = 2 * kStages + 4;
   static constexpr int kTileOffset = kBarOffset + kNumBars * 8;
-  static constexpr int kTotal = kTileOffset + STAGES * 4;
+  static constexpr int kTotal = kTileOffset + kStages * 4 + 4;
 };
 
 constexpr int kSchedSlots = 256;
 __device__ unsigned int g_tile_sched[kSchedSlots][2];
 
-template <int BLOCK_N, int STAGES, int EPI, bool CLUSTER>
-__device__ __forceinline__ void consumer_tile(uint8_t* smem, uint64_t* full_bar, uint64_t* empty_bar,
-                                              int& stage, uint32_t& phase, int m0, int n0,
-                                              int num_kb, int cw, const bf16* __restrict__ bias,
-                                              bf16* __restrict__ C, int64_t ldc, int M, int N,
-                                              const bf16* __restrict__ act, int64_t ldact,
-                                              float* colsum, float (&acc)[BLOCK_N / WGMMA_N][64]) {
-  using L = SmemLayout<BLOCK_N, STAGES, EPI>;
-  constexpr int NB = BLOCK_N / WGMMA_N;
-  const int lane = threadIdx.x & 31, warp_in_wg = (threadIdx.x >> 5) & 3;
-  const bool releaser = warp_in_wg == 0 && lane == 0;
-  const int row0 = m0 + cw * 64 + warp_in_wg * 16 + (lane >> 2);
-  uint8_t* s_act = smem + L::kActOffset + cw * L::kActWgBytes;
-  const uint32_t s_act_a = smem_addr(s_act);
-  const uint32_t s_part_a = smem_addr(smem + L::kColsumOffset) + cw * 4 * BLOCK_N * 4;
-  constexpr int kRowChunks = BLOCK_N / 8;
-  const int wt = threadIdx.x & 127;
-  if constexpr (EPI == 2) {
-    warpgroup_bar_sync(cw);
-#pragma unroll 4
-    for (int c = wt; c < 64 * kRowChunks; c += 128) {
-      const int r = c / kRowChunks, cc = c % kRowChunks;
-      const int row = m0 + cw * 64 + r, col = n0 + cc * 8;
-      const bool ok = row < M && col < N;
-      cp_async_16(s_act + r * L::kActRowBytes + cc * 16,
-                  act + (ok ? static_cast<int64_t>(row) * ldact + col : 0), ok ? 16u : 0u);
-    }
-    cp_async_commit();
-  }
-  int prev_stage = -1;
-  for (int kb = 0; kb < num_kb; ++kb) {
-    mbar_wait(&full_bar[stage], phase);
-    const uint32_t sa = smem_addr(smem + stage * L::kStageBytes) + cw * 64 * 128;
-    const uint32_t sb = smem_addr(smem + stage * L::kStageBytes + L::kABytes);
-    wgmma_fence();
-#pragma unroll
-    for (int k = 0; k < BLOCK_K / WGMMA_K; ++k) {
-      const uint64_t da = make_sw128_kmajor_desc(sa + k * WGMMA_K * 2);
-#pragma unroll
-      for (int nb = 0; nb < NB; ++nb) {
-        const uint64_t db = make_sw128_kmajor_desc(sb + nb * WGMMA_N * 128 + k * WGMMA_K * 2);
-        wgmma_m64n128k16(acc[nb], da, db, (kb | k) != 0 ? 1u : 0u);
-      }
-    }
-    wgmma_commit();
-    wgmma_wait<1>();
-    if (prev_stage >= 0 && releaser) {
-      if (CLUSTER) {
-        for (uint32_t r = 0; r < 2; ++r) {
-          const uint32_t a = smem_addr(&empty_bar[prev_stage]);
-          uint32_t remote;
-          asm volatile("mapa.shared::cluster.u32 %0, %1, %2;" : "=r"(remote) : "r"(a), "r"(r));
-          asm volatile("mbarrier.arrive.release.cluster.shared::cluster.b64 _, [%0];" ::"r"(remote)
-                       : "memory");
-        }
-      } else {
-        mbar_arrive(&empty_bar[prev_stage]);
-      }
-    }
-    prev_stage = stage;
-    if (++stage == STAGES) {
-      stage = 0;
-      phase ^= 1;
-    }
-  }
-  wgmma_wait<0>();
-  if (prev_stage >= 0 && releaser) {
-    if (CLUSTER) {
-      for (uint32_t r = 0; r < 2; ++r) {
-        const uint32_t a = smem_addr(&empty_bar[prev_stage]);
-        uint32_t remote;
-        asm volatile("mapa.shared::cluster.u32 %0, %1, %2;" : "=r"(remote) : "r"(a), "r"(r));
-        asm volatile("mbarrier.arrive.release.cluster.shared::cluster.b64 _, [%0];" ::"r"(remote)
-                     : "memory");
-      }
-    } else {
-      mbar_arrive(&empty_bar[prev_stage]);
-    }
-  }
-
-  if constexpr (EPI == 2) {
-    cp_async_wait_all();
-    warpgroup_bar_sync(cw);
-  }
-#pragma unroll
-  for (int nb = 0; nb < NB; ++nb) {
-#pragma unroll
-    for (int j = 0; j < WGMMA_N / 8; ++j) {
-      const int col = n0 + nb * WGMMA_N + j * 8 + (lane & 3) * 2;
-      const bool col_ok = col < N;
-      float b0 = 0.f, b1 = 0.f;
-      if (EPI != 2 && bias != nullptr && col_ok) {
-        const float2 bb = __bfloat1622float2(*reinterpret_cast<const __nv_bfloat162*>(bias + col));
-        b0 = bb.x;
-        b1 = bb.y;
-      }
-      float cs0 = 0.f, cs1 = 0.f;
-#pragma unroll
-      for (int i = 0; i < 2; ++i) {
-        const int row = row0 + 8 * i;
-        float v0 = acc[nb][4 * j + 2 * i], v1 = acc[nb][4 * j + 2 * i + 1];
-        if constexpr (EPI == 2) {
-          const uint32_t sp = s_act_a + (row - m0 - cw * 64) * L::kActRowBytes + (col - n0) * 2;
-          const uint32_t a = lds_b32(sp);
-          v0 = __uint_as_float(a << 16) > 0.f ? v0 : 0.f;
-          v1 = __uint_as_float(a & 0xffff0000u) > 0.f ? v1 : 0.f;
-          cs0 += v0;
-          cs1 += v1;
-          const __nv_bfloat162 r = __floats2bfloat162_rn(v0, v1);
-          sts_b32(sp, *reinterpret_cast<const uint32_t*>(&r));
-        } else {
-          v0 += b0;
-          v1 += b1;
-          if (EPI == 1) {
-            v0 = fmaxf(v0, 0.f);
-            v1 = fmaxf(v1, 0.f);
-          }
-          if (row < M && col_ok)
-            *reinterpret_cast<__nv_bfloat162*>(C + static_cast<int64_t>(row) * ldc + col) =
-                __floats2bfloat162_rn(v0, v1);
-        }
-      }
-      if (EPI == 2) {
-#pragma unroll
-        for (int sft = 4; sft < 32; sft <<= 1) {
-          cs0 += __shfl_xor_sync(0xffffffffu, cs0, sft);
-          cs1 += __shfl_xor_sync(0xffffffffu, cs1, sft);
-        }
-        if (lane < 4) {
-          const uint32_t sp = s_part_a + (warp_in_wg * BLOCK_N + col - n0) * 4;
-          sts_b32(sp, __float_as_uint(cs0));
-          sts_b32(sp + 4, __float_as_uint(cs1));
-        }
-      }
-    }
-  }
-  if constexpr (EPI == 2) {
-    warpgroup_bar_sync(cw);
-    for (int c = wt; c < BLOCK_N; c += 128) {
-      const uint32_t sp = s_part_a + c * 4;
-      const float v = __uint_as_float(lds_b32(sp)) + __uint_as_float(lds_b32(sp + BLOCK_N * 4)) +
-                      __uint_as_float(lds_b32(sp + 2 * BLOCK_N * 4)) +
-                      __uint_as_float(lds_b32(sp + 3 * BLOCK_N * 4));
-      if (n0 + c < N && v != 0.f) red_add_f32(colsum + n0 + c, v);
-    }
-#pragma unroll 4
-    for (int c = wt; c < 64 * kRowChunks; c += 128) {
-      const int r = c / kRowChunks, cc = c % kRowChunks;
-      const int row = m0 + cw * 64 + r, col = n0 + cc * 8;
-      if (row < M && col < N)
-        *reinterpret_cast<uint4*>(C + static_cast<int64_t>(row) * ldc + col) =
-            lds_b128(s_act_a + r * L::kActRowBytes + cc * 16);
-    }
-  }
-}
-
-template <int BLOCK_N, int STAGES, int EPI>
+template <int EPI>
 __global__ void __launch_bounds__(kGemmThreads, 1)
 gemm_tn_fused_kernel(const __grid_constant__ CUtensorMap tma_a,
-                     const __grid_constant__ CUtensorMap tma_b, const bf16* __restrict__ bias,
-                     bf16* __restrict__ C, int64_t ldc, int M, int N, int K,
-                     const bf16* __restrict__ act, int64_t ldact, float* __restrict__ colsum,
-                     int sched_slot) {
-  using L = SmemLayout<BLOCK_N, STAGES, EPI>;
+                     const __grid_constant__ CUtensorMap tma_b,
+                     const __grid_constant__ CUtensorMap tma_c,
+                     const __grid_constant__ CUtensorMap tma_act, const bf16* __restrict__ bias,
+                     int M, int N, int K, float* __restrict__ colsum, int sched_slot) {
+  using L = SmemLayout<EPI>;
   extern __shared__ uint8_t smem_raw[];
   uint8_t* smem = reinterpret_cast<uint8_t*>(
       (reinterpret_cast<uintptr_t>(smem_raw) + 1023) & ~static_cast<uintptr_t>(1023));
   uint64_t* full_bar = reinterpret_cast<uint64_t*>(smem + L::kBarOffset);
-  uint64_t* empty_bar = full_bar + STAGES;
+  uint64_t* empty_bar = full_bar + kStages;
+  uint64_t* act_full = empty_bar + kStages;
+  uint64_t* act_empty = act_full + 2;
   volatile int* s_tile = reinterpret_cast<int*>(smem + L::kTileOffset);
+  volatile int* s_end = s_tile + kStages;
 
   const int wg = threadIdx.x >> 7;
   const int num_kb = (K + BLOCK_K - 1) / BLOCK_K;
@@ -367,10 +214,17 @@
   if (threadIdx.x == 0) {
     tma_prefetch_desc(&tma_a);
     tma_prefetch_desc(&tma_b);
-    for (int s = 0; s < STAGES; ++s) {
+    tma_prefetch_desc(&tma_c);
+    if (EPI == 2) tma_prefetch_desc(&tma_act);
+    for (int s = 0; s < kStages; ++s) {
       mbar_init(&full_bar[s], 1);
-      mbar_init(&empty_bar[s], 2);
-    }
+      mbar_init(&empty_bar[s], 1);
+    }
+    for (int c = 0; c < 2; ++c) {
+      mbar_init(&act_full[c], 1);
+      mbar_init(&act_empty[c], 1);
+    }
+    *s_end = 0;
     fence_barrier_init();
     fence_proxy_async();
   }
@@ -379,14 +233,14 @@
   if (wg == 0) {
     if (threadIdx.x == 0) {
       unsigned int* sched = g_tile_sched[sched_slot];
-      int stage = 0;
-      uint32_t phase = 0;
-      for (int tile = blockIdx.x;;) {
+      uint32_t pos = 0;
+      for (int tile = blockIdx.x, n_local = 0;; ++n_local) {
         const int next = static_cast<int>(gridDim.x + atomicAdd(&sched[0], 1u));
         const bool done = tile >= num_tiles;
         const int m0 = (tile / tiles_n) * BLOCK_M, n0 = (tile % tiles_n) * BLOCK_N;
-        for (int kb = 0; kb < num_kb; ++kb) {
-          mbar_wait(&empty_bar[stage], phase ^ 1);
+        for (int kb = 0; kb < num_kb; ++kb, ++pos) {
+          const uint32_t stage = pos % kStages;
+          mbar_wait(&empty_bar[stage], ((pos / kStages) & 1) ^ 1);
           if (kb == 0) s_tile[stage] = done ? -1 : tile;
           if (done) {
             mbar_arrive(&full_bar[stage]);
@@ -397,12 +251,17 @@
           mbar_expect_tx(&full_bar[stage], L::kStageBytes);
           tma_load_2d(sa, &tma_a, &full_bar[stage], kb * BLOCK_K, m0);
           tma_load_2d(sb, &tma_b, &full_bar[stage], kb * BLOCK_K, n0);
-          if (++stage == STAGES) {
-            stage = 0;
-            phase ^= 1;
-          }
         }
         if (done) break;
+        if constexpr (EPI == 2) {
+          const int c = n_local & 1;
+          const uint32_t uses = static_cast<uint32_t>(n_local >> 1);
+          mbar_wait(&act_empty[c], (uses & 1) ^ 1);
+          uint8_t* buf = smem + L::kOutOffset + c * L::kOutBytes;
+          mbar_expect_tx(&act_full[c], L::kOutBytes);
+          tma_load_2d(buf, &tma_act, &act_full[c], n0, m0);
+          tma_load_2d(buf + L::kOutBoxBytes, &tma_act, &act_full[c], n0 + 64, m0);
+        }
         tile = next;
       }
       __threadfence();
@@ -414,21 +273,117 @@
     }
   } else {
     const int cw = wg - 1;
-    float acc[BLOCK_N / WGMMA_N][64];
-#pragma unroll
-    for (int nb = 0; nb < BLOCK_N / WGMMA_N; ++nb)
-#pragma unroll
-      for (int r = 0; r < 64; ++r) acc[nb][r] = 0.f;
-    int stage = 0;
-    uint32_t phase = 0;
-    for (;;) {
-      mbar_wait(&full_bar[stage], phase);
-      const int tile = s_tile[stage];
-      if (tile < 0) break;
+    const int wt = threadIdx.x & 127, lane = wt & 31, warp = wt >> 5;
+    const uint32_t ring = smem_addr(smem);
+    const uint32_t buf = smem_addr(smem + L::kOutOffset + cw * L::kOutBytes);
+    const uint32_t s_part = smem_addr(smem + L::kColsumOffset) + cw * 4 * BLOCK_N * 4;
+    float acc[2][64];
+    uint32_t pos = cw == 0 ? 0u : static_cast<uint32_t>(num_kb);
+    for (uint32_t use = 0;; ++use) {
+      if (cw == 1 || use > 0) {
+        named_bar_sync(kTurnBar + cw, 256);
+        if (*s_end) break;
+      }
+      const uint32_t stage0 = pos % kStages;
+      mbar_wait(&full_bar[stage0], (pos / kStages) & 1);
+      const int tile = s_tile[stage0];
+      if (tile < 0) {
+        *s_end = 1;
+        named_bar_arrive(kTurnBar + (cw ^ 1), 256);
+        break;
+      }
       const int m0 = (tile / tiles_n) * BLOCK_M, n0 = (tile % tiles_n) * BLOCK_N;
-      consumer_tile<BLOCK_N, STAGES, EPI, false>(smem, full_bar, empty_bar, stage, phase, m0, n0,
-                                                 num_kb, cw, bias, C, ldc, M, N, act, ldact,
-                                                 colsum, acc);
+      for (int kb = 0; kb < num_kb; ++kb) {
+        const uint32_t p = pos + kb, stage = p % kStages;
+        mbar_wait(&full_bar[stage], (p / kStages) & 1);
+        const uint32_t sa = ring + stage * L::kStageBytes, sb = sa + L::kABytes;
+        wgmma_fence();
+#pragma unroll
+        for (int k = 0; k < BLOCK_K / WGMMA_K; ++k) {
+          const uint64_t db = make_sw128_kmajor_desc(sb + k * WGMMA_K * 2);
+#pragma unroll
+          for (int mb = 0; mb < 2; ++mb)
+            wgmma_m64n128k16(acc[mb], make_sw128_kmajor_desc(sa + mb * 64 * 128 + k * WGMMA_K * 2),
+                             db, (kb | k) != 0 ? 1u : 0u);
+        }
+        wgmma_commit();
+        wgmma_wait<1>();
+        if (kb > 0 && wt == 0) mbar_arrive(&empty_bar[(p - 1) % kStages]);
+      }
+      named_bar_arrive(kTurnBar + (cw ^ 1), 256);
+      wgmma_wait<0>();
+      if (wt == 0) mbar_arrive(&empty_bar[(pos + num_kb - 1) % kStages]);
+      pos += 2 * num_kb;
+
+      if constexpr (EPI == 2) mbar_wait(&act_full[cw], use & 1);
+#pragma unroll
+      for (int j = 0; j < BLOCK_N / 8; ++j) {
+        const int col = n0 + j * 8 + (lane & 3) * 2;
+        float b0 = 0.f, b1 = 0.f;
+        if (EPI != 2 && bias != nullptr && col < N) {
+          const float2 bb =
+              __bfloat1622float2(*reinterpret_cast<const __nv_bfloat162*>(bias + col));
+          b0 = bb.x;
+          b1 = bb.y;
+        }
+        float cs0 = 0.f, cs1 = 0.f;
+#pragma unroll
+        for (int mb = 0; mb < 2; ++mb) {
+#pragma unroll
+          for (int i = 0; i < 2; ++i) {
+            const int r = mb * 64 + warp * 16 + (lane >> 2) + 8 * i;
+            const uint32_t sp = buf + (j >> 3) * L::kOutBoxBytes + r * 128 +
+                                (((j & 7) ^ (lane >> 2)) << 4) + (lane & 3) * 4;
+            float v0 = acc[mb][4 * j + 2 * i], v1 = acc[mb][4 * j + 2 * i + 1];
+            if constexpr (EPI == 2) {
+              const uint32_t a = lds_b32(sp);
+              v0 = __uint_as_float(a << 16) > 0.f ? v0 : 0.f;
+              v1 = __uint_as_float(a & 0xffff0000u) > 0.f ? v1 : 0.f;
+              cs0 += v0;
+              cs1 += v1;
+            } else {
+              v0 += b0;
+              v1 += b1;
+              if (EPI == 1) {
+                v0 = fmaxf(v0, 0.f);
+                v1 = fmaxf(v1, 0.f);
+              }
+            }
+            const __nv_bfloat162 o = __floats2bfloat162_rn(v0, v1);
+            sts_b32(sp, *reinterpret_cast<const uint32_t*>(&o));
+          }
+        }
+        if constexpr (EPI == 2) {
+#pragma unroll
+          for (int sft = 4; sft < 32; sft <<= 1) {
+            cs0 += __shfl_xor_sync(0xffffffffu, cs0, sft);
+            cs1 += __shfl_xor_sync(0xffffffffu, cs1, sft);
+          }
+          if (lane < 4) {
+            const uint32_t sp = s_part + (warp * BLOCK_N + j * 8 + lane * 2) * 4;
+            sts_b32(sp, __float_as_uint(cs0));
+            sts_b32(sp + 4, __float_as_uint(cs1));
+          }
+        }
+      }
+      fence_proxy_async();
+      named_bar_sync(kEpiBar + cw, 128);
+      if (wt == 0) {
+        tma_store_2d(&tma_c, buf, n0, m0);
+        if (n0 + 64 < N) tma_store_2d(&tma_c, buf + L::kOutBoxBytes, n0 + 64, m0);
+        bulk_commit_group();
+      }
+      if constexpr (EPI == 2) {
+        const uint32_t sp = s_part + wt * 4;
+        const float v = __uint_as_float(lds_b32(sp)) + __uint_as_float(lds_b32(sp + BLOCK_N * 4)) +
+                        __uint_as_float(lds_b32(sp + 2 * BLOCK_N * 4)) +
+                        __uint_as_float(lds_b32(sp + 3 * BLOCK_N * 4));
+        if (n0 + wt < N && v != 0.f) red_add_f32(colsum + n0 + wt, v);
+      }
+      if (wt == 0) {
+        bulk_wait_group_read0();
+        if constexpr (EPI == 2) mbar_arrive(&act_empty[cw]);
+      }
     }
   }
 }
@@ -443,12 +398,99 @@
   asm volatile("barrier.cluster.wait.acquire.aligned;" ::: "memory");
 }
 
-template <int BLOCK_N, int STAGES, int EPI>
+constexpr int kPairN = 256;
+constexpr int kPairStages = 4;
+struct PairSmemLayout {
+  static constexpr int kABytes = BLOCK_M * BLOCK_K * 2;
+  static constexpr int kBBytes = kPairN * BLOCK_K * 2;
+  static constexpr int kStageBytes = kABytes + kBBytes;
+  static constexpr int kBarOffset = kPairStages * kStageBytes;
+  static constexpr int kTotal = kBarOffset + 2 * kPairStages * 8;
+};
+
+template <int EPI>
+__device__ __forceinline__ void pair_consumer_tile(uint8_t* smem, uint64_t* full_bar,
+                                                   uint64_t* empty_bar, int& stage,
+                                                   uint32_t& phase, int m0, int n0, int num_kb,
+                                                   int cw, const bf16* __restrict__ bias,
+                                                   bf16* __restrict__ C, int64_t ldc, int M, int N,
+                                                   float (&acc)[kPairN / WGMMA_N][64]) {
+  using L = PairSmemLayout;
+  constexpr int NB = kPairN / WGMMA_N;
+  const int lane = threadIdx.x & 31, warp_in_wg = (threadIdx.x >> 5) & 3;
+  const bool releaser = warp_in_wg == 0 && lane == 0;
+  auto release = [&](int s) {
+    for (uint32_t r = 0; r < 2; ++r) {
+      const uint32_t a = smem_addr(&empty_bar[s]);
+      uint32_t remote;
+      asm volatile("mapa.shared::cluster.u32 %0, %1, %2;" : "=r"(remote) : "r"(a), "r"(r));
+      asm volatile("mbarrier.arrive.release.cluster.shared::cluster.b64 _, [%0];" ::"r"(remote)
+                   : "memory");
+    }
+  };
+  const int row0 = m0 + cw * 64 + warp_in_wg * 16 + (lane >> 2);
+  int prev_stage = -1;
+  for (int kb = 0; kb < num_kb; ++kb) {
+    mbar_wait(&full_bar[stage], phase);
+    const uint32_t sa = smem_addr(smem + stage * L::kStageBytes) + cw * 64 * 128;
+    const uint32_t sb = smem_addr(smem + stage * L::kStageBytes + L::kABytes);
+    wgmma_fence();
+#pragma unroll
+    for (int k = 0; k < BLOCK_K / WGMMA_K; ++k) {
+      const uint64_t da = make_sw128_kmajor_desc(sa + k * WGMMA_K * 2);
+#pragma unroll
+      for (int nb = 0; nb < NB; ++nb) {
+        const uint64_t db = make_sw128_kmajor_desc(sb + nb * WGMMA_N * 128 + k * WGMMA_K * 2);
+        wgmma_m64n128k16(acc[nb], da, db, (kb | k) != 0 ? 1u : 0u);
+      }
+    }
+    wgmma_commit();
+    wgmma_wait<1>();
+    if (prev_stage >= 0 && releaser) release(prev_stage);
+    prev_stage = stage;
+    if (++stage == kPairStages) {
+      stage = 0;
+      phase ^= 1;
+    }
+  }
+  wgmma_wait<0>();
+  if (prev_stage >= 0 && releaser) release(prev_stage);
+
+#pragma unroll
+  for (int nb = 0; nb < NB; ++nb) {
+#pragma unroll
+    for (int j = 0; j < WGMMA_N / 8; ++j) {
+      const int col = n0 + nb * WGMMA_N + j * 8 + (lane & 3) * 2;
+      const bool col_ok = col < N;
+      float b0 = 0.f, b1 = 0.f;
+      if (bias != nullptr && col_ok) {
+        const float2 bb = __bfloat1622float2(*reinterpret_cast<const __nv_bfloat162*>(bias + col));
+        b0 = bb.x;
+        b1 = bb.y;
+      }
+#pragma unroll
+      for (int i = 0; i < 2; ++i) {
+        const int row = row0 + 8 * i;
+        float v0 = acc[nb][4 * j + 2 * i] + b0, v1 = acc[nb][4 * j + 2 * i + 1] + b1;
+        if (EPI == 1) {
+          v0 = fmaxf(v0, 0.f);
+          v1 = fmaxf(v1, 0.f);
+        }
+        if (row < M && col_ok)
+          *reinterpret_cast<__nv_bfloat162*>(C + static_cast<int64_t>(row) * ldc + col) =
+              __floats2bfloat162_rn(v0, v1);
+      }
+    }
+  }
+}
+
+template <int EPI>
 __global__ void __cluster_dims__(2, 1, 1) __launch_bounds__(kGemmThreads, 1)
 gemm_tn_pair_kernel(const __grid_constant__ CUtensorMap tma_a,
                     const __grid_constant__ CUtensorMap tma_b, const bf16* __restrict__ bias,
                     bf16* __restrict__ C, int64_t ldc, int M, int N, int K) {
-  using L = SmemLayout<BLOCK_N, STAGES>;
+  using L = PairSmemLayout;
+  constexpr int BN = kPairN, STAGES = kPairStages;
   constexpr int kHalfB = L::kBBytes / 2;
   extern __shared__ uint8_t smem_raw[];
   uint8_t* smem = reinterpret_cast<uint8_t*>(
@@ -460,7 +502,7 @@
   const uint32_t cta_rank = cluster_ctarank();
   const int pair = blockIdx.x >> 1, num_pairs = gridDim.x >> 1;
   const int num_kb = (K + BLOCK_K - 1) / BLOCK_K;
-  const int tiles_n = (N + BLOCK_N - 1) / BLOCK_N;
+  const int tiles_n = (N + BN - 1) / BN;
   const int tiles_m = (M + 2 * BLOCK_M - 1) / (2 * BLOCK_M);
   const int num_tiles = tiles_n * tiles_m;
 
@@ -483,7 +525,7 @@
       uint32_t phase = 0;
       for (int tile = pair; tile < num_tiles; tile += num_pairs) {
         const int m0 = (tile / tiles_n) * (2 * BLOCK_M) + static_cast<int>(cta_rank) * BLOCK_M;
-        const int n0 = (tile % tiles_n) * BLOCK_N + static_cast<int>(cta_rank) * (BLOCK_N / 2);
+        const int n0 = (tile % tiles_n) * BN + static_cast<int>(cta_rank) * (BN / 2);
         for (int kb = 0; kb < num_kb; ++kb) {
           mbar_wait_cluster(&empty_bar[stage], phase ^ 1);
           uint8_t* sa = smem + stage * L::kStageBytes;
@@ -500,19 +542,18 @@
     }
   } else {
     const int cw = wg - 1;
-    float acc[BLOCK_N / WGMMA_N][64];
-#pragma unroll
-    for (int nb = 0; nb < BLOCK_N / WGMMA_N; ++nb)
+    float acc[BN / WGMMA_N][64];
+#pragma unroll
+    for (int nb = 0; nb < BN / WGMMA_N; ++nb)
 #pragma unroll
       for (int r = 0; r < 64; ++r) acc[nb][r] = 0.f;
     int stage = 0;
     uint32_t phase = 0;
     for (int tile = pair; tile < num_tiles; tile += num_pairs) {
       const int m0 = (tile / tiles_n) * (2 * BLOCK_M) + static_cast<int>(cta_rank) * BLOCK_M;
-      const int n0 = (tile % tiles_n) * BLOCK_N;
-      consumer_tile<BLOCK_N, STAGES, EPI, true>(smem, full_bar, empty_bar, stage, phase, m0, n0,
-                                                num_kb, cw, bias, C, ldc, M, N, nullptr, 0,
-                                                nullptr, acc);
+      const int n0 = (tile % tiles_n) * BN;
+      pair_consumer_tile<EPI>(smem, full_bar, empty_bar, stage, phase, m0, n0, num_kb, cw, bias,
+                              C, ldc, M, N, acc);
     }
   }
   __syncthreads();
@@ -557,43 +598,27 @@
   return static_cast<int>(seq.fetch_add(1, std::memory_order_relaxed) % kSchedSlots);
 }
 
-template <int BLOCK_N, int STAGES, int EPI>
-bool launch_one(const CUtensorMap& ta, const CUtensorMap& tb, const void* bias, void* C,
-                int64_t ldc, int M, int N, int K, const void* act, int64_t ldact, float* colsum,
+template <int EPI>
+bool launch_one(const CUtensorMap& ta, const CUtensorMap& tb, const CUtensorMap& tc,
+                const CUtensorMap& tact, const void* bias, int M, int N, int K, float* colsum,
                 int sm_count, cudaStream_t stream) {
-  using L = SmemLayout<BLOCK_N, STAGES, EPI>;
+  using L = SmemLayout<EPI>;
   const size_t smem = L::kTotal + 1024;
   static_assert(L::kTotal + 1024 <= 227 * 1024, "exceeds the 227 KB of shared memory per block");
   const int tiles = ((N + BLOCK_N - 1) / BLOCK_N) * ((M + BLOCK_M - 1) / BLOCK_M);
   dim3 grid(tiles < sm_count ? tiles : sm_count);
-  cudaFuncSetAttribute(gemm_tn_fused_kernel<BLOCK_N, STAGES, EPI>,
-                       cudaFuncAttributeMaxDynamicSharedMemorySize, static_cast<int>(smem));
-  gemm_tn_fused_kernel<BLOCK_N, STAGES, EPI><<<grid, kGemmThreads, smem, stream>>>(
-      ta, tb, reinterpret_cast<const bf16*>(bias), reinterpret_cast<bf16*>(C), ldc, M, N, K,
-      reinterpret_cast<const bf16*>(act), ldact, colsum, next_sched_slot());
+  cudaFuncSetAttribute(gemm_tn_fused_kernel<EPI>, cudaFuncAttributeMaxDynamicSharedMemorySize,
+                       static_cast<int>(smem));
+  gemm_tn_fused_kernel<EPI><<<grid, kGemmThreads, smem, stream>>>(
+      ta, tb, tc, tact, reinterpret_cast<const bf16*>(bias), M, N, K, colsum, next_sched_slot());
   return cudaGetLastError() == cudaSuccess;
-}
-
-template <int BLOCK_N, int STAGES>
-bool launch_cfg(const CUtensorMap& ta, const CUtensorMap& tb, const void* bias, void* C,
-                int64_t ldc, int M, int N, int K, int epi, const void* act, int64_t ldact,
-                float* colsum, int sm_count, cudaStream_t stream) {
-  if (epi == 0)
-    return launch_one<BLOCK_N, STAGES, 0>(ta, tb, bias, C, ldc, M, N, K, act, ldact, colsum,
-                                          sm_count, stream);
-  if (epi == 1)
-    return launch_one<BLOCK_N, STAGES, 1>(ta, tb, bias, C, ldc, M, N, K, act, ldact, colsum,
-                                          sm_count, stream);
-  return launch_one<BLOCK_N, STAGES - 1, 2>(ta, tb, bias, C, ldc, M, N, K, act, ldact, colsum,
-                                            sm_count, stream);
 }
 
 }
 
 bool launch_gemm_tn_fused(const void* A, int64_t lda, const void* B, int64_t ldb, const void* bias,
                           void* C, int64_t ldc, int M, int N, int K, int epi, const void* act,
-                          int64_t ldact, float* colsum, int block_n, int sm_count,
-                          cudaStream_t stream) {
+                          int64_t ldact, float* colsum, int sm_count, cudaStream_t stream) {
   if (M <= 0 || N <= 0 || K <= 0) return true;
   if ((lda % 8) || (ldb % 8) || (ldc % 8) || (N % 8)) return false;
   if ((reinterpret_cast<uintptr_t>(A) | reinterpret_cast<uintptr_t>(B) |
@@ -602,31 +627,30 @@
   if (epi == 2 && (act == nullptr || colsum == nullptr || N > kMaxColsum || (ldact % 8) ||
                    (reinterpret_cast<uintptr_t>(act) & 15)))
     return false;
-  const int bn = (block_n == 128 || block_n == 256) ? block_n : (N >= 256 ? 256 : 128);
-  alignas(64) CUtensorMap ta, tb;
+  alignas(64) CUtensorMap ta, tb, tc, tact;
   if (!make_tensor_map(&ta, A, M, K, lda, BLOCK_M)) return false;
-  if (!make_tensor_map(&tb, B, N, K, ldb, bn)) return false;
-  if (bn == 256)
-    return launch_cfg<256, 4>(ta, tb, bias, C, ldc, M, N, K, epi, act, ldact, colsum, sm_count,
-                              stream);
-  return launch_cfg<128, 6>(ta, tb, bias, C, ldc, M, N, K, epi, act, ldact, colsum, sm_count,
-                            stream);
+  if (!make_tensor_map(&tb, B, N, K, ldb, BLOCK_N)) return false;
+  if (!make_tensor_map(&tc, C, M, N, ldc, BLOCK_M)) return false;
+  if (epi != 2)
+    return epi == 1 ? launch_one<1>(ta, tb, tc, tc, bias, M, N, K, nullptr, sm_count, stream)
+                    : launch_one<0>(ta, tb, tc, tc, bias, M, N, K, nullptr, sm_count, stream);
+  if (!make_tensor_map(&tact, act, M, N, ldact, BLOCK_M)) return false;
+  return launch_one<2>(ta, tb, tc, tact, nullptr, M, N, K, colsum, sm_count, stream);
 }
 
 namespace {
 template <int EPI>
 bool launch_pair(const CUtensorMap& ta, const CUtensorMap& tb, const void* bias, void* C,
                  int64_t ldc, int M, int N, int K, int sm_count, cudaStream_t stream) {
-  constexpr int BN = 256, ST = 4;
-  using L = SmemLayout<BN, ST>;
+  using L = PairSmemLayout;
   const size_t smem = L::kTotal + 1024;
-  const int tiles = ((N + BN - 1) / BN) * ((M + 2 * BLOCK_M - 1) / (2 * BLOCK_M));
+  const int tiles = ((N + kPairN - 1) / kPairN) * ((M + 2 * BLOCK_M - 1) / (2 * BLOCK_M));
   int pairs = sm_count / 2;
   if (tiles < pairs) pairs = tiles;
   if (pairs < 1) return false;
-  cudaFuncSetAttribute(gemm_tn_pair_kernel<BN, ST, EPI>,
-                       cudaFuncAttributeMaxDynamicSharedMemorySize, static_cast<int>(smem));
-  gemm_tn_pair_kernel<BN, ST, EPI><<<dim3(2 * pairs), kGemmThreads, smem, stream>>>(
+  cudaFuncSetAttribute(gemm_tn_pair_kernel<EPI>, cudaFuncAttributeMaxDynamicSharedMemorySize,
+                       static_cast<int>(smem));
+  gemm_tn_pair_kernel<EPI><<<dim3(2 * pairs), kGemmThreads, smem, stream>>>(
       ta, tb, reinterpret_cast<const bf16*>(bias), reinterpret_cast<bf16*>(C), ldc, M, N, K);
   return cudaGetLastError() == cudaSuccess;
 }
@@ -653,7 +677,7 @@
   if (block_n == 512)
     return launch_gemm_tn_pair(A, lda, B, ldb, bias, C, ldc, M, N, K, relu, sm_count, stream);
   return launch_gemm_tn_fused(A, lda, B, ldb, bias, C, ldc, M, N, K, relu ? 1 : 0, nullptr, 0,
-                              nullptr, block_n, sm_count, stream);
-}
-
-}
+                              nullptr, sm_count, stream);
+}
+
+}
```

Result: faster. 19.43 million (median of 6 runs) (+2.2%).
